# Tencent/FeatherCNN

Hardware: AMD Instinct MI355X
Metric: images/sec fp32 forward @224x224 (higher is better)
Workload: dtype f32; 1 GPU; vgg16 whole net (40 layers in the model file, 20 after fusion level 3), batch 32 per GPU, 224x224x3, fp32, synthetic ...; net=vgg16, mode=net, per_gpu_batch=32, global_batch=32, parallelism=batch-shard x1, launch=hipGraph replay per step, conv_routing=fhip_conv_select_algo_tuned

## Files before the change

### __graft_entry__.py

```python
from __future__ import annotations

import os
import subprocess
import sys

ROOT = os.path.dirname(os.path.abspath(__file__))
if ROOT not in sys.path:
    sys.path.insert(0, ROOT)


def build() -> None:
    jobs = str(min(8, os.cpu_count() or 1))
    subprocess.run(["make", "-s", "-j", jobs, "-C", os.path.join(ROOT, "feathercnn_amd", "csrc")], check=True)
    subprocess.run(["make", "-s", "-C", os.path.join(ROOT, "oracle"), "port"], check=True)
    subprocess.run(["make", "-s", "-C", os.path.join(ROOT, "oracle"), "ref"], check=True)
    import feathercnn_amd
    from feathercnn_amd import _lib
    for name in (*_lib.LIBRARIES, *_lib.MORE_LIBRARIES):
        _lib.load(name)
    from feathercnn_amd import provenance
    provenance.write_stamp()


def smoke() -> None:
    import numpy as np
    import torch

    import oracle
    from feathercnn_amd import ConvLayer, ConvParam
    from oracle import conv_geom, nerr, synth

    if not torch.cuda.is_available():
        raise RuntimeError("smoke() needs a GPU")
    if not os.path.exists(os.path.join(ROOT, "feathercnn_amd", "libfeather_hip.so")):
        build()
    dev = torch.device("cuda:0")
    chk = oracle.best()
    cases = [("winograd_f63", conv_geom(16, 32, 20, 3, 1, 1)), ("im2col_1x1", conv_geom(32, 24, 14, 1, 1, 0)),
             ("im2col_7x7s2", conv_geom(3, 16, 32, 7, 2, 3)), ("depthwise_s1", conv_geom(16, 16, 28, 3, 1, 1, group=16)),
             ("depthwise_s2", conv_geom(16, 16, 28, 3, 2, 1, group=16)), ("depthwise_flat_14px", conv_geom(24, 24, 14, 3, 1, 1, group=24)),
             ("depthwise_flat_7px", conv_geom(40, 40, 7, 3, 1, 1, group=40)), ("depthwise_band_56px", conv_geom(8, 8, 56, 3, 1, 1, group=8)),
             ("depthwise_flat_20px_s2", conv_geom(12, 12, 20, 3, 2, 1, group=12)), ("depthwise_flat_5px", conv_geom(44, 44, 5, 3, 1, 1, group=44))]
    for name, g in cases:
        x, w, b = synth(g, 2)
        p = ConvParam(output_channels=g.oc, input_channels=g.ic, input_h=g.ih, input_w=g.iw, kernel_h=g.kh, kernel_w=g.kw,
                      stride_h=g.sh, stride_w=g.sw, pad_left=g.pl, pad_right=g.pr, pad_top=g.pt, pad_bottom=g.pb,
                      group=g.group, bias_term=True, activation=1, batch=2)
        layer = ConvLayer(p, torch.from_numpy(w).to(dev), torch.from_numpy(b).to(dev))
        y = layer.Forward(torch.from_numpy(x).to(dev))
        torch.cuda.synchronize()
        e = nerr(y.cpu().numpy(), chk.forward(g, x, w, b))
        print(f"smoke {name}: algo={layer.booster.algo} normalised error vs {type(chk).__name__} = {e:.2e}")
        if not (e <= 1e-4) or not np.isfinite(e):
            raise AssertionError(f"smoke {name}: parity failed ({e})")
    from feathercnn_amd.booster import WINOGRADF63, forward_chained
    g1, g2 = conv_geom(16, 24, 28, 3, 1, 1), conv_geom(24, 8, 28, 3, 1, 1)
    (x, w1, b1), (_, w2, b2) = synth(g1, 2, seed=3), synth(g2, 2, seed=4)
    run = []
    for g, w, b in ((g1, w1, b1), (g2, w2, b2)):
        p = ConvParam(output_channels=g.oc, input_channels=g.ic, input_h=g.ih, input_w=g.iw, kernel_h=3, kernel_w=3, stride_h=1, stride_w=1,
                      pad_left=1, pad_right=1, pad_top=1, pad_bottom=1, group=1, bias_term=True, activation=1, batch=2)
        run.append(ConvLayer(p, torch.from_numpy(w).to(dev), torch.from_numpy(b).to(dev), algo=WINOGRADF63))
    y = forward_chained(run, torch.from_numpy(x).to(dev))
    torch.cuda.synchronize()
    e = nerr(y.cpu().numpy(), chk.forward(g2, chk.forward(g1, x, w1, b1), w2, b2))
    print(f"smoke chained winograd pair: normalised error = {e:.2e}")
    if not (e <= 1e-4):
        raise AssertionError(f"smoke chained pair: parity failed ({e})")
    g0, g1 = conv_geom(3, 16, 28, 3, 1, 1), conv_geom(16, 8, 28, 3, 1, 1)
    (x, w0, b0), (_, w1, b1) = synth(g0, 2, seed=6), synth(g1, 2, seed=7)
    p0 = ConvParam(output_channels=16, input_channels=3, input_h=28, input_w=28, kernel_h=3, kernel_w=3, stride_h=1, stride_w=1, pad_left=1,
                   pad_right=1, pad_top=1, pad_bottom=1, group=1, bias_term=True, activation=1, batch=2)
    p0.AssignOutputDim()
    p1 = ConvParam(output_channels=8, input_channels=16, input_h=28, input_w=28, kernel_h=3, kernel_w=3, stride_h=1, stride_w=1, pad_left=1,
                   pad_right=1, pad_top=1, pad_bottom=1, group=1, bias_term=True, activation=1, batch=2)
    l1 = ConvLayer(p1, torch.from_numpy(w1).to(dev), torch.from_numpy(b1).to(dev), algo=WINOGRADF63)
    y = forward_chained([l1], torch.from_numpy(x).to(dev), first=(p0, torch.from_numpy(w0).to(dev), torch.from_numpy(b0).to(dev)))
    torch.cuda.synchronize()
    e = nerr(y.cpu().numpy(), chk.forward(g1, chk.forward(g0, x, w0, b0), w1, b1))
    print(f"smoke first layer inside the Winograd input transform: normalised error = {e:.2e}")
    if not (e <= 1e-4):
        raise AssertionError(f"smoke first-layer fusion: parity failed ({e})")
    from feathercnn_amd import model_zoo
    from feathercnn_amd.net import Net
    from oracle import netcheck
    p, b, i, o = model_zoo.tiny_allsorts()
    x = np.random.default_rng(5).uniform(-1, 1, (2, 3, 20, 20)).astype(np.float32)
    want = (netcheck.RefNet(p, b) if netcheck.have_ref_net() else netcheck.PortNet(p, b)).run(i, x, o)
    for level in (1, 3):
        net = Net(fusion=level, tuned=(level == 3), graph=(level == 3))
        net.LoadParam(p)
        net.LoadWeights(b)
        net.FeedInput(i, x)
        net.Forward()
        e = nerr(net.Extract(o), want)
        print(f"smoke tiny net, fusion level {level} ({len(net.layers())} layers after fusion): normalised error = {e:.2e}")
        if not (e <= 1e-4):
            raise AssertionError(f"smoke net: parity failed ({e})")
    sys.path.insert(0, os.path.join(ROOT, "tests"))
    import gconv_ref
    p, b, i, o = model_zoo.tiny_grouped()
    x = np.random.default_rng(6).uniform(-1, 1, (2, 3, 21, 21)).astype(np.float32)
    net = Net(fusion=2)
    net.LoadParam(p)
    net.LoadWeights(b)
    net.FeedInput(i, x)
    net.Forward()
    e = gconv_ref.nerr(net.Extract(o), gconv_ref.Net(p, b).run(i, x, o))
    print(f"smoke grouped net ({sum(a == 'GCONV' for _, _, a in net.layers())} grouped layers): normalised error = {e:.2e}")
    if not (e <= 1e-4):
        raise AssertionError(f"smoke grouped net: parity failed ({e})")
    import deconv_ref
    p, b, i, o = model_zoo.tiny_deconv()
    x = np.random.default_rng(7).uniform(-1, 1, (2, 3, 16, 16)).astype(np.float32)
    net = Net(fusion=2)
    net.LoadParam(p)
    net.LoadWeights(b)
    net.FeedInput(i, x)
    net.Forward()
    e = deconv_ref.nerr(net.Extract(o), deconv_ref.Net(p, b).run(i, x, o))
    print(f"smoke tiny_deconv ({sum(a == 'DECONV' for _, _, a in net.layers())} deconvolution layers): normalised error = {e:.2e}")
    if not (e <= 1e-4):
        raise AssertionError(f"smoke tiny_deconv: parity failed ({e})")
    import inorm_ref
    p, b, i, o = model_zoo.tiny_generative()
    x = np.random.default_rng(8).uniform(-1, 1, (2, 3, 24, 24)).astype(np.float32)
    net = Net(fusion=2)
    net.LoadParam(p)
    net.LoadWeights(b)
    net.FeedInput(i, x)
    net.Forward()
    e = inorm_ref.nerr(net.Extract(o), inorm_ref.Net(p, b).run(i, x, o))
    print(f"smoke tiny_generative ({sum(a == 'INORM' for _, _, a in net.layers())} InstanceNorm layers): normalised error = {e:.2e}")
    if not (e <= 1e-4):
        raise AssertionError(f"smoke tiny_generative: parity failed ({e})")
    import shuffle_ref
    p, b, i, o = model_zoo.tiny_shuffle()
    x = np.random.default_rng(9).uniform(-1, 1, (2, 3, 28, 28)).astype(np.float32)
    net = Net(fusion=2)
    net.LoadParam(p)
    net.LoadWeights(b)
    net.FeedInput(i, x)
    net.Forward()
    e = shuffle_ref.nerr(net.Extract(o), shuffle_ref.Net(p, b).run(i, x, o))
    print(f"smoke tiny_shuffle ({sum(a == 'SHUFFLE' for _, _, a in net.layers())} channel-map launches): normalised error = {e:.2e}")
    if not (e <= 1e-4):
        raise AssertionError(f"smoke tiny_shuffle: parity failed ({e})")
    import atrous_ref
    p, b, i, o = model_zoo.tiny_dilated()
    x = np.random.default_rng(10).uniform(-1, 1, (2, 3, 16, 16)).astype(np.float32)
    net = Net(fusion=2)
    net.SetDilated(True)
    net.LoadParam(p)
    net.LoadWeights(b)
    net.FeedInput(i, x)
    net.Forward()
    e = atrous_ref.nerr(net.Extract(o), atrous_ref.Net(p, b).run(i, x, o))
    print(f"smoke tiny_dilated ({sum(a == 'ATROUS' for _, _, a in net.layers())} dilated layers): normalised error = {e:.2e}")
    if not (e <= 1e-4):
        raise AssertionError(f"smoke tiny_dilated: parity failed ({e})")
    import gate_ref
    p, b, i, o = model_zoo.tiny_se()
    x = np.random.default_rng(11).uniform(-1, 1, (2, 3, 24, 24)).astype(np.float32)
    net = Net(fusion=2)
    net.LoadParam(p)
    net.LoadWeights(b)
    net.FeedInput(i, x)
    net.Forward()
    e = gate_ref.nerr(net.Extract(o), gate_ref.Net(p, b).run(i, x, o))
    print(f"smoke tiny_se ({sum(a == 'GATE' and t == 'Pooling' for t, _, a in net.layers())} collapsed SE blocks): normalised error = {e:.2e}")
    if not (e <= 1e-4):
# ... 87 lines not shown
```

### feathercnn_amd/_lib.py

```python
from __future__ import annotations

import collections
import ctypes
import functools
import os

_HERE = os.path.dirname(os.path.abspath(__file__))
_LOADED = {}

STAGE_NAMES = ("wino_input", "wino_gemm", "wino_output", "igemm", "depthwise", "init", "wino_chain")


class fhip_conv_param(ctypes.Structure):
    _fields_ = [(n, ctypes.c_int) for n in (
        "output_channels", "input_channels", "input_h", "input_w", "kernel_h", "kernel_w", "output_h", "output_w",
        "stride_h", "stride_w", "pad_left", "pad_bottom", "pad_right", "pad_top", "group", "bias_term", "activation")]


class fhip_winograd_plan(ctypes.Structure):
    _fields_ = [("tiles_x", ctypes.c_int), ("tiles_y", ctypes.c_int), ("tiles_per_image", ctypes.c_int),
                ("columns", ctypes.c_int), ("columns_padded", ctypes.c_int), ("column_block", ctypes.c_int), ("frequency_points", ctypes.c_int), ("tile_outputs", ctypes.c_int),
                ("in_channels_padded", ctypes.c_int),
                ("out_channels_padded", ctypes.c_int), ("v_offset_bytes", ctypes.c_size_t), ("v_bytes", ctypes.c_size_t),
                ("m_offset_bytes", ctypes.c_size_t), ("m_bytes", ctypes.c_size_t), ("u_bytes", ctypes.c_size_t)]


class fhip_pool_param(ctypes.Structure):
    _fields_ = [(n, ctypes.c_int) for n in (
        "channels", "input_h", "input_w", "kernel_h", "kernel_w", "stride_h", "stride_w", "pad_left", "pad_right",
        "pad_top", "pad_bottom", "pooling_type", "global_pooling")]


class fhip_pixel_image(ctypes.Structure):
    _fields_ = [("data", ctypes.c_void_p)] + [(n, ctypes.c_int) for n in ("w", "h", "stride", "roi_x", "roi_y", "roi_w", "roi_h")]


_P = ctypes.POINTER(fhip_conv_param)
_Q = ctypes.POINTER(fhip_pool_param)
_PI = ctypes.POINTER(ctypes.c_int)
_SZ = ctypes.c_size_t
_V = ctypes.c_void_p
_I = ctypes.c_int

SIGNATURES = {
    "fhip_conv_assign_output_dim": (_I, [_P]),
    "fhip_conv_flops": (ctypes.c_double, [_P]),
    "fhip_conv_select_algo": (_I, [_P, ctypes.POINTER(_I)]),
    "fhip_conv_select_algo_tuned": (_I, [_P, ctypes.POINTER(_I)]),
    "fhip_conv_get_buffer_size": (_I, [_P, _I, _I, ctypes.POINTER(ctypes.c_size_t), ctypes.POINTER(ctypes.c_size_t)]),
    "fhip_conv_packed_layout": (_I, [_P, _I, ctypes.POINTER(ctypes.c_int)]),
    "fhip_conv_init": (_I, [_P, _I, _V, _V, _V]),
    "fhip_conv_forward": (_I, [_P, _I, _I, _V, _V, _V, _V, _V, _V]),
    "fhip_winograd_f63_plan": (_I, [_P, _I, ctypes.POINTER(fhip_winograd_plan)]),
    "fhip_winograd_f63_plan_canvas": (_I, [_P, _I, _I, ctypes.POINTER(fhip_winograd_plan)]),
    "fhip_winograd_f63_canvas_param": (_I, [_P, _I, _P]),
    "fhip_winograd_f63_transform_kernel": (_I, [_P, _V, _V, _V]),
    "fhip_winograd_f63_input_transform": (_I, [_P, _I, _V, _V, _V]),
    "fhip_winograd_f63_tile_gemm": (_I, [_P, _I, _V, _V, _V, _V]),
    "fhip_winograd_f63_output_transform": (_I, [_P, _I, _V, _V, _V, _V]),
    "fhip_stage_timing_enable": (_I, [_I]),
    "fhip_stage_timing_collect": (_I, [ctypes.POINTER(ctypes.c_double), ctypes.POINTER(ctypes.c_longlong)]),
    "fhip_last_error": (ctypes.c_char_p, []),
    "fhip_version": (ctypes.c_char_p, []),
    "fhip_device_info": (_I, [ctypes.c_char_p, _I, ctypes.POINTER(_I), ctypes.POINTER(_I)]),
    "fhip_conv_streams_1x1": (_I, [_P, _I, _I]),
    "fhip_calibrate_mfma_f32": (_I, [ctypes.POINTER(ctypes.c_double), ctypes.POINTER(ctypes.c_double), _V]),
    "fhip_relu": (_I, [_V, _V, _SZ, _V]),
    "fhip_add": (_I, [_V, _V, _V, _SZ, _I, _V]),
    "fhip_affine": (_I, [_V, _V, _V, _V, _I, _I, _I, _I, _V]),
    "fhip_conv_can_fuse_residual": (_I, [_P, _I]),
    "fhip_conv_forward_residual": (_I, [_P, _I, _I, _V, _V, _V, _V, _V, _V, _V]),
    "fhip_conv_can_fuse_dw_pw": (_I, [_P, _P, _I]),
    "fhip_conv_forward_dw_pw": (_I, [_P, _P, _I, _V, _V, _V, _V, _V, _V, _V]),
    "fhip_conv_can_chain_winograd": (_I, [_P, _I, _P, _I, _I]),
    "fhip_conv_forward_chained": (_I, [_P, _I, _V, _V, _V, _V, _V, _V, _P, _V, _I, _V]),
    "fhip_winograd_f63_output_to_next_input": (_I, [_P, _P, _I, _V, _V, _V, _I, _V]),
    "fhip_conv_can_fuse_siblings": (_I, [_P, _I, _P, _I, _I]),
    "fhip_conv_siblings_geometry": (_I, [_P, _P, _P]),
    "fhip_conv_forward_siblings": (_I, [_P, _P, _I, _V, _V, _V, _V, _V, _V]),
    "fhip_conv_can_fuse_first_winograd": (_I, [_P, _P, _I, _I]),
    "fhip_winograd_f63_input_from_first": (_I, [_P, _P, _I, _V, _V, _V, _V, _V]),
    "fhip_conv_can_fuse_maxpool2": (_I, [_P, _I]),
    "fhip_conv_forward_maxpool2": (_I, [_P, _I, _I, _V, _V, _V, _V, _V, _V]),
    "fhip_pixels_to_float": (_I, [_V, _V, _I, _I, _I, _I, _I, _I, _V, _V, _V]),
    "fhip_yuv420sp_to_float": (_I, [_V, _V, _I, _I, _I, _I, _I, _I, _I, _V, _V, _V]),
    "fhip_pixel_images_plan": (_I, [_V, _I, _I, _I, _I, _V, ctypes.POINTER(_SZ)]),
    "fhip_pixels_to_float_images": (_I, [_V, _V, _V, _V, _V, _V]),
    "fhip_pooling_output_dim": (_I, [_Q, _PI, _PI]),
    "fhip_pooling": (_I, [_Q, _I, _V, _V, _V]),
    "fhip_softmax": (_I, [_V, _V, _I, _I, _V]),
    "fhip_net_create": (_I, [ctypes.POINTER(_V)]),
    "fhip_net_destroy": (_I, [_V]),
    "fhip_net_set_stream": (_I, [_V, _V]),
    "fhip_net_get_stream": (_I, [_V, ctypes.POINTER(_V)]),
    "fhip_net_set_fusion": (_I, [_V, _I]),
    "fhip_net_set_graph": (_I, [_V, _I]),
    "fhip_net_set_tuned_selection": (_I, [_V, _I]),
    "fhip_net_set_dilated": (_I, [_V, _I]),
    "fhip_net_set_quantized": (_I, [_V, _I]),
    "fhip_net_set_requantized": (_I, [_V, _I]),
    "fhip_net_set_extended_layers": (_I, [_V, _I]),
    "fhip_net_set_detection": (_I, [_V, _I]),
    "fhip_net_set_concurrency": (_I, [_V, _I]),
    "fhip_net_set_sub_batches": (_I, [_V, _I]),
    "fhip_net_load_param": (_I, [_V, ctypes.c_char_p]),
    "fhip_net_load_param_mem": (_I, [_V, ctypes.c_char_p, _SZ]),
    "fhip_net_load_weights": (_I, [_V, ctypes.c_char_p]),
    "fhip_net_load_weights_mem": (_I, [_V, _V, _SZ]),
    "fhip_net_load_weights_device": (_I, [_V, _V, _SZ]),
    "fhip_net_feed_input": (_I, [_V, ctypes.c_char_p, _I, _I, _I, _I, _V, _I]),
    "fhip_net_feed_pixels": (_I, [_V, ctypes.c_char_p, _I, _V, _I, _I, _I, _I, _I, _V, _V, _I]),
    "fhip_net_feed_yuv420sp": (_I, [_V, ctypes.c_char_p, _I, _V, _I, _I, _I, _I, _I, _I, _V, _V, _I]),
    "fhip_net_feed_pixel_images": (_I, [_V, ctypes.c_char_p, _I, _V, _I, _I, _I, _V, _V, _I]),
    "fhip_net_forward": (_I, [_V]),
    "fhip_net_extract": (_I, [_V, ctypes.c_char_p, ctypes.POINTER(_V), _PI, _PI, _PI, _PI]),
    "fhip_net_extract_host": (_I, [_V, ctypes.c_char_p, _V, _SZ]),
    "fhip_net_layer_count": (_I, [_V]),
    "fhip_net_layer_info": (_I, [_V, _I, ctypes.c_char_p, ctypes.c_char_p, _I, _PI]),
    "fhip_net_layer_conv_param": (_I, [_V, _I, _P, _PI]),
    "fhip_net_layer_fused_pointwise": (_I, [_V, _I, _P, _PI]),
    "fhip_net_layer_chain": (_I, [_V, _I, _PI, _PI]),
    "fhip_net_layer_canvas": (_I, [_V, _I, _PI]),
    "fhip_net_layer_sibling": (_I, [_V, _I, _PI]),
    "fhip_net_layer_residual": (_I, [_V, _I, _PI]),
    "fhip_net_forward_timed": (_I, [_V, ctypes.POINTER(ctypes.c_float)]),
    "fhip_net_memory": (_I, [_V, ctypes.POINTER(_SZ), ctypes.POINTER(_SZ), ctypes.POINTER(_SZ)]),
}

PIXOUT_SIGNATURES = {
    "fhip_pixout_channels": (_I, [_I]),
    "fhip_float_to_pixels": (_I, [_V, _SZ, _V, _I, _I, _I, _I, _I, _I, _V, _V, _V]),
    "fhip_float_to_pixels_host": (_I, [_V, _SZ, _V, _I, _I, _I, _I, _I, _I, _V, _V, _V]),
    "fhip_pixout_last_error": (ctypes.c_char_p, []),
}

GCONV_SIGNATURES = {
    "fhip_gconv_supported": (_I, [_P]),
    "fhip_gconv_get_buffer_size": (_I, [_P, _I, ctypes.POINTER(_SZ), ctypes.POINTER(_SZ)]),
    "fhip_gconv_init": (_I, [_P, _V, _V, _V]),
    "fhip_gconv_forward": (_I, [_P, _I, _V, _V, _V, _V, _V, _V]),
    "fhip_gconv_route": (_I, [_P, _V, _V, ctypes.c_char_p, _I]),
    "fhip_gconv_last_error": (ctypes.c_char_p, []),
}

class fhip_deconv_param(ctypes.Structure):
    _fields_ = [(n, ctypes.c_int) for n in ("output_channels", "input_channels", "input_h", "input_w", "kernel_h", "kernel_w", "output_h", "output_w",
                                            "stride_h", "stride_w", "pad_left", "pad_bottom", "pad_right", "pad_top", "group", "bias_term",
                                            "activation", "output_pad_right", "output_pad_bottom")]


_DP = ctypes.POINTER(fhip_deconv_param)
DECONV_SIGNATURES = {
    "fhip_deconv_assign_output_dim": (_I, [_DP]),
    "fhip_deconv_supported": (_I, [_DP]),
    "fhip_deconv_get_buffer_size": (_I, [_DP, _I, ctypes.POINTER(_SZ), ctypes.POINTER(_SZ)]),
    "fhip_deconv_init": (_I, [_DP, _V, _V, _V]),
    "fhip_deconv_forward": (_I, [_DP, _I, _V, _V, _V, _V, _V, _V]),
    "fhip_deconv_route": (_I, [_DP, ctypes.c_char_p, _I]),
    "fhip_deconv_last_error": (ctypes.c_char_p, []),
}

_FL = ctypes.c_float
INORM_SIGNATURES = {
    "fhip_instance_norm_get_buffer_size": (_I, [_I, _I, _I, _I, ctypes.POINTER(_SZ)]),
    "fhip_instance_norm_forward": (_I, [_I, _I, _I, _I, _V, _V, _V, _V, _FL, _I, _FL, _V, _V]),
    "fhip_instance_norm_forward_route": (_I, [_I, _I, _I, _I, _I, _V, _V, _V, _V, _FL, _I, _FL, _V, _V]),
    "fhip_instance_norm_route": (_I, [_I, _I, _I, _I, _V, _V, ctypes.c_char_p, _I]),
    "fhip_activation_forward": (_I, [_I, _V, _V, _I, _I, _I, _FL, _FL, _V, _V]),
    "fhip_inorm_last_error": (ctypes.c_char_p, []),
}

_PP = ctypes.POINTER(ctypes.c_void_p)
_IP = ctypes.POINTER(ctypes.c_int)
SHUFFLE_SIGNATURES = {
    "fhip_channel_map_supported": (_I, [_I, _I, _I, _I]),
    "fhip_channel_slice_resolve": (_I, [_I, _IP, _I, _IP]),
    "fhip_channel_shuffle_forward": (_I, [_V, _V, _I, _I, _I, _I, _I, _I, _V]),
    "fhip_channel_slice_forward": (_I, [_PP, _V, _I, _I, _I, _I, _IP, _I, _V]),
    "fhip_channel_map_create": (_I, [_PP, _IP, _I, _IP, _I, _IP]),
    "fhip_channel_map_destroy": (_I, [_V]),
    "fhip_channel_map_forward": (_I, [_V, _PP, _PP, _I, _I, _I, _V]),
    "fhip_channel_map_forward_route": (_I, [_I, _V, _PP, _PP, _I, _I, _I, _V]),
    "fhip_channel_map_route": (_I, [_I, _I, _I, _PP, _I, ctypes.c_char_p, _I]),
    "fhip_shuffle_last_error": (ctypes.c_char_p, []),
}

_PL = ctypes.POINTER(fhip_winograd_plan)
CANVAS_SIGNATURES = {
    "fhip_canvas_output_to_next_input": (_I, [_I, _P, _P, _I, _PL, _PL, _V, _V, _V, _V]),
    "fhip_canvas_output_transform": (_I, [_P, _I, _PL, _V, _V, _V, _I, _V]),
    "fhip_canvas_last_error": (ctypes.c_char_p, []),
}

class fhip_atrous_param(ctypes.Structure):
    _fields_ = [(n, ctypes.c_int) for n in ("output_channels", "input_channels", "input_h", "input_w", "kernel_h", "kernel_w", "output_h", "output_w",
                                            "stride_h", "stride_w", "pad_left", "pad_bottom", "pad_right", "pad_top", "group", "bias_term",
                                            "activation", "dilation_h", "dilation_w")]


_AP = ctypes.POINTER(fhip_atrous_param)
ATROUS_SIGNATURES = {
    "fhip_atrous_assign_output_dim": (_I, [_AP]),
    "fhip_atrous_supported": (_I, [_AP]),
    "fhip_atrous_get_buffer_size": (_I, [_AP, _I, ctypes.POINTER(_SZ), ctypes.POINTER(_SZ)]),
    "fhip_atrous_init": (_I, [_AP, _V, _V, _V]),
    "fhip_atrous_forward": (_I, [_AP, _I, _V, _V, _V, _V, _V, _V]),
    "fhip_atrous_route": (_I, [_AP, ctypes.c_char_p, _I]),
    "fhip_atrous_get_buffer_size_route": (_I, [_AP, _I, ctypes.c_char_p, ctypes.POINTER(_SZ), ctypes.POINTER(_SZ)]),
    "fhip_atrous_init_route": (_I, [_AP, _V, _V, _V, ctypes.c_char_p]),
    "fhip_atrous_forward_route": (_I, [_AP, _I, _V, _V, _V, _V, _V, _V, ctypes.c_char_p]),
    "fhip_atrous_last_error": (ctypes.c_char_p, []),
}

GATE_SIGNATURES = {
    "fhip_channel_gate_forward": (_I, [_I, _I, _I, _I, _V, _V, _V, _V, _I, _V]),
    "fhip_squeeze_get_buffer_size": (_I, [_I, _I, _I, _I, ctypes.POINTER(_SZ)]),
    "fhip_squeeze_forward": (_I, [_I, _I, _I, _I, _V, _V, _V, _V]),
    "fhip_excite_forward": (_I, [_I, _I, _I, _V, _V, _V, _V, _V, _V, _I, _I, _FL, _FL, _V]),
    "fhip_excite_forward_slices": (_I, [_I, _I, _I, _I, _V, _V, _V, _V, _V, _V, _I, _I, _FL, _FL, _V]),
    "fhip_gate_activation_forward": (_I, [_I, _V, _V, _I, _I, _I, _FL, _FL, _V]),
    "fhip_gate_route": (_I, [_I, _I, _I, _I, _I, _V, _V, _V, ctypes.c_char_p, _I]),
    "fhip_gate_last_error": (ctypes.c_char_p, []),
}

RESAMPLE_SIGNATURES = {
    "fhip_interp_output_dim": (_I, [_I, _I, _FL, _FL, _I, _I, _PI, _PI]),
    "fhip_interp_forward": (_I, [_I, _I, _I, _I, _I, _I, _I, _I, _FL, _FL, _V, _V, _V, _I, _V]),
    "fhip_interp_route": (_I, [_I, _I, _I, _I, _I, _I, _I, _FL, _FL, _V, _V, _V, ctypes.c_char_p, _I]),
    "fhip_hardswish_forward": (_I, [_V, _V, _I, _I, _I, _FL, _FL, _V]),
    "fhip_hardswish_route": (_I, [_V, _V, _I, _I, _I, ctypes.c_char_p, _I]),
    "fhip_resample_last_error": (ctypes.c_char_p, []),
}

LRN_SIGNATURES = {
    "fhip_lrn_forward": (_I, [_I, _I, _FL, _FL, _FL, _I, _I, _I, _I, _V, _V, _V]),
    "fhip_lrn_forward_chunked": (_I, [_I, _FL, _FL, _FL, _I, _I, _I, _I, _I, _V, _V, _V]),
    "fhip_lrn_route": (_I, [_I, _I, _I, _I, _I, _I, _V, _V, ctypes.c_char_p, _I]),
    "fhip_lrn_pool_forward": (_I, [_I, _I, _FL, _FL, _FL, _I, _I, _I, _I, _Q, _V, _V, _V]),
    "fhip_lrn_pool_route": (_I, [_I, _I, _I, _I, _I, _I, _Q, _V, _V, ctypes.c_char_p, _I]),
    "fhip_lrn_last_error": (ctypes.c_char_p, []),
}

class fhip_qconv_param(ctypes.Structure):
    _fields_ = [(n, ctypes.c_int) for n in ("output_channels", "input_channels", "input_h", "input_w", "kernel_h", "kernel_w", "output_h", "output_w",
                                            "stride_h", "stride_w", "pad_left", "pad_bottom", "pad_right", "pad_top", "group", "bias_term",
                                            "activation", "dilation_h", "dilation_w", "int8_scale_term")]


_QP = ctypes.POINTER(fhip_qconv_param)
QCONV_SIGNATURES = {
    "fhip_qconv_assign_output_dim": (_I, [_QP]),
    "fhip_qconv_supported": (_I, [_QP]),
    "fhip_qconv_get_buffer_size": (_I, [_QP, _I, ctypes.POINTER(_SZ), ctypes.POINTER(_SZ)]),
    "fhip_qconv_init": (_I, [_QP, _V, _V, _V]),
    "fhip_qconv_dequant_scales": (_I, [_V, _V, _I, _FL]),
    "fhip_qconv_forward": (_I, [_QP, _I, _V, _V, _V, _V, _V, _V, _FL, _V]),
    "fhip_quantize_forward": (_I, [_V, _V, _SZ, _FL, _V]),
    "fhip_qconv_route": (_I, [_QP, ctypes.c_char_p, _I]),
    "fhip_qconv_get_buffer_size_route": (_I, [_QP, _I, ctypes.c_char_p, ctypes.POINTER(_SZ), ctypes.POINTER(_SZ)]),
    "fhip_qconv_init_route": (_I, [_QP, _V, _V, _V, ctypes.c_char_p]),
    "fhip_qconv_forward_route": (_I, [_QP, _I, _V, _V, _V, _V, _V, _V, _FL, _V, ctypes.c_char_p]),
    "fhip_qconv_last_error": (ctypes.c_char_p, []),
}


class fhip_q8_param(ctypes.Structure):
    _fields_ = fhip_qconv_param._fields_ + [("input_int8", ctypes.c_int), ("output_int8", ctypes.c_int)]


_8P = ctypes.POINTER(fhip_q8_param)
Q8_SIGNATURES = {
    "fhip_q8_tensor_bytes": (_I, [_I, _I, _I, _I, ctypes.POINTER(_SZ)]),
    "fhip_q8_assign_output_dim": (_I, [_8P]),
    "fhip_q8_supported": (_I, [_8P]),
    "fhip_q8_get_buffer_size": (_I, [_8P, _I, ctypes.POINTER(_SZ), ctypes.POINTER(_SZ)]),
    "fhip_q8_init": (_I, [_8P, _V, _V, _V]),
    "fhip_q8_dequant_scales": (_I, [_V, _V, _I, _FL]),
    "fhip_q8_forward": (_I, [_8P, _I, _V, _V, _V, _V, _V, _V, _FL, _FL, _V]),
    "fhip_q8_route": (_I, [_8P, ctypes.c_char_p, _I]),
    "fhip_q8_get_buffer_size_route": (_I, [_8P, _I, ctypes.c_char_p, ctypes.POINTER(_SZ), ctypes.POINTER(_SZ)]),
    "fhip_q8_init_route": (_I, [_8P, _V, _V, _V, ctypes.c_char_p]),
    "fhip_q8_forward_route": (_I, [_8P, _I, _V, _V, _V, _V, _V, _V, _FL, _FL, _V, ctypes.c_char_p]),
    "fhip_q8_quantize_forward": (_I, [_V, _V, _I, _I, _I, _I, _FL, _V]),
    "fhip_q8_dequantize_forward": (_I, [_V, _V, _I, _I, _I, _I, _FL, _V]),
    "fhip_q8_relu_forward": (_I, [_V, _V, _SZ, _V]),
    "fhip_q8_max_pool_forward": (_I, [_Q, _I, _V, _V, _V]),
    "fhip_q8_last_error": (ctypes.c_char_p, []),
}


_FP = ctypes.POINTER(ctypes.c_float)
DETECT_SIGNATURES = {
    "fhip_permute_output_dim": (_I, [_I, _I, _I, _I, _I, _PI, _PI, _PI]),
    "fhip_permute_forward": (_I, [_I, _I, _I, _I, _I, _I, _V, _V, _V]),
    "fhip_permute_concat_forward": (_I, [_I, _PI, _PI, _I, _V, _PP, _V]),
    "fhip_normalize_forward": (_I, [_I, _I, _I, _I, _I, _FL, _V, _V, _V, _V]),
    "fhip_axis_softmax_forward": (_I, [_I, _I, _I, _V, _V, _V]),
    "fhip_priorbox_fill": (_I, [_I, _I, _I, _I, _FP, _I, _FP, _I, _FP, _I, _FP, _I, _I, _FL, _FL, _FL, _PI, _FP, _SZ]),
    "fhip_detection_output_get_buffer_size": (_I, [_I, _I, _I, _I, _I, ctypes.POINTER(_SZ)]),
    "fhip_detection_output_forward": (_I, [_I, _I, _I, _FL, _I, _I, _FL, _I, _V, _V, _V, _V, _V, _V]),
    "fhip_detect_route": (_I, [_I, _I, _I, _I, _I, _I, _V, _V, ctypes.c_char_p, _I]),
    "fhip_detect_last_error": (ctypes.c_char_p, []),
}


def _load(path, signatures):
    lib = _LOADED.get(path)
    if lib is None:
        import torch
        if not os.path.exists(path):
            raise RuntimeError(f"feathercnn_amd: HIP library {path} is missing -- run `python -c 'import __graft_entry__ as g; "
                               "g.build()'` (or `make -C feathercnn_amd/csrc`). There is no CPU fallback.")
        lib = ctypes.CDLL(path)
        for name, (res, args) in signatures.items():
            fn = getattr(lib, name)
            fn.restype = res
            fn.argtypes = args
        _LOADED[path] = lib
    return lib


def checker(load, last_error: str):
    def _check(rc: int, what: str):
        if rc != 0:
            from .booster import FeatherHipError
            msg = getattr(load(), last_error)().decode(errors="replace")
            raise FeatherHipError(f"{what} failed with code {rc}: {msg}")
    return _check


Library = collections.namedtuple("Library", "file headers macro signatures last_error structs route")

LIBRARIES = {
    "hip": Library("libfeather_hip.so", ("feather_hip.h", "feather_net.h"), "FHIP_API", SIGNATURES, "fhip_last_error",
                   (fhip_conv_param, fhip_winograd_plan, fhip_pool_param, fhip_pixel_image), None),
    "pixout": Library("libfeather_pixout.so", ("feather_pixout.h",), "FHIP_PIXOUT_API", PIXOUT_SIGNATURES, "fhip_pixout_last_error", (), None),
    "gconv": Library("libfeather_gconv.so", ("feather_gconv.h",), "FHIP_GCONV_API", GCONV_SIGNATURES, "fhip_gconv_last_error", (), "ROUTE_GCONV"),
    "deconv": Library("libfeather_deconv.so", ("feather_deconv.h",), "FHIP_DECONV_API", DECONV_SIGNATURES, "fhip_deconv_last_error",
                      (fhip_deconv_param,), "ROUTE_DECONV"),
    "inorm": Library("libfeather_inorm.so", ("feather_inorm.h",), "FHIP_INORM_API", INORM_SIGNATURES, "fhip_inorm_last_error", (), "ROUTE_INORM"),
    "shuffle": Library("libfeather_shuffle.so", ("feather_shuffle.h",), "FHIP_SHUFFLE_API", SHUFFLE_SIGNATURES, "fhip_shuffle_last_error", (),
                       "ROUTE_SHUFFLE"),
    "canvas": Library("libfeather_canvas.so", ("feather_canvas.h",), "FHIP_CANVAS_API", CANVAS_SIGNATURES, "fhip_canvas_last_error", (), None),
    "atrous": Library("libfeather_atrous.so", ("feather_atrous.h",), "FHIP_ATROUS_API", ATROUS_SIGNATURES, "fhip_atrous_last_error",
                      (fhip_atrous_param,), "ROUTE_ATROUS"),
    "gate": Library("libfeather_gate.so", ("feather_gate.h",), "FHIP_GATE_API", GATE_SIGNATURES, "fhip_gate_last_error", (), "ROUTE_GATE"),
    "resample": Library("libfeather_resample.so", ("feather_resample.h",), "FHIP_RESAMPLE_API", RESAMPLE_SIGNATURES, "fhip_resample_last_error", (),
                        "ROUTE_RESAMPLE"),
    "lrn": Library("libfeather_lrn.so", ("feather_lrn.h",), "FHIP_LRN_API", LRN_SIGNATURES, "fhip_lrn_last_error", (), "ROUTE_LRN"),
    "qconv": Library("libfeather_qconv.so", ("feather_qconv.h",), "FHIP_QCONV_API", QCONV_SIGNATURES, "fhip_qconv_last_error",
                     (fhip_qconv_param,), "ROUTE_QCONV"),
}
MAIN = "hip"
MORE_LIBRARIES = {
    "q8": Library("libfeather_q8.so", ("feather_q8.h",), "FHIP_Q8_API", Q8_SIGNATURES, "fhip_q8_last_error", (fhip_q8_param,), None),
    "detect": Library("libfeather_detect.so", ("feather_detect.h",), "FHIP_DETECT_API", DETECT_SIGNATURES, "fhip_detect_last_error", (), None),
}


def row(name: str) -> Library:
    return LIBRARIES[name] if name in LIBRARIES else MORE_LIBRARIES[name]


def path(name: str) -> str:
    default = os.path.join(_HERE, row(name).file)
    return os.environ.get("FEATHER_HIP_LIB", default) if name == MAIN else default


def load(name: str):
    return _load(path(name), row(name).signatures)


def lib_path() -> str:
    return path(MAIN)


def load_library():
    return load(MAIN)


for _name in (*LIBRARIES, *MORE_LIBRARIES):
    if _name != MAIN:
        globals()[f"{_name}_path"] = functools.partial(path, _name)
        globals()[f"load_{_name}_library"] = functools.partial(load, _name)
del _name
```

### feathercnn_amd/csrc/net.hip

```cpp
#include "net_side.h"
#include "net_model.h"
#include "net_core.h"
#include "net_conv.h"
#include "net_layers.h"
#include "net_detect.h"
#include "net_plan.h"

namespace fhip::net
{

static Layer* create_extended_layer(const std::string& type)
{
    if (type == "Interp") return new InterpLayer;
    if (type == "HardSwish") return new HardSwishLayer;
    if (type == "LRN") return new LRNLayer;
    return nullptr;
}

static Layer* create_layer(const std::string& type)
{
    if (type == "Input") return new InputLayer;
    if (type == "Convolution" || type == "ConvolutionDepthWise") return new ConvLayer;
    if (type == "Deconvolution" || type == "DeconvolutionDepthWise") return new DeconvLayer;
    if (type == "ReLU") return new ReluLayer;
// ... 128 lines not shown
}

}

using namespace fhip;
using namespace fhip::net;

struct fhip_net
{
    Net impl;
    std::vector<std::unique_ptr<fhip_net>> more;
    std::vector<hipStream_t> more_streams;
    hipEvent_t fork = nullptr;
    std::vector<hipEvent_t> joins;
    std::vector<int> share;
    std::map<std::string, DeviceVec> gathered;
    unsigned char* staging = nullptr;
    size_t staging_bytes = 0;
    std::vector<unsigned char> plans;
    hipEvent_t plans_read = nullptr;
    ~fhip_net()
    {
        if (staging) (void)hipFree(staging);
        if (plans_read) (void)hipEventDestroy(plans_read);
        more.clear();
        for (hipStream_t st : more_streams) (void)hipStreamDestroy(st);
        if (fork) (void)hipEventDestroy(fork);
        for (hipEvent_t e : joins) (void)hipEventDestroy(e);
    }
};

static void deal(int num, int parts, std::vector<int>& share)
{
    share.assign(parts, num / parts);
    for (int r = 0; r < num % parts; ++r) ++share[r];
}

static int reserve_staging(fhip_net* n, size_t bytes)
{
    if (bytes <= n->staging_bytes) return FHIP_OK;
    FHIP_CHECK_HIP(hipStreamSynchronize(n->impl.stream));
    if (n->staging) FHIP_CHECK_HIP(hipFree(n->staging));
    n->staging = nullptr;
    n->staging_bytes = 0;
    FHIP_CHECK_HIP(hipMalloc((void**)&n->staging, bytes));
    n->staging_bytes = bytes;
    return FHIP_OK;
}

template <class Convert>
static int feed_shares(fhip_net* n, const char* blob_name, int num, int cout, int target_w, int target_h, const Convert& convert)
{
    const auto into_blob = [&](fhip_net* m, int first, int cnt) -> int {
        Blob* b = m->impl.find(blob_name);
        if (!b) return failf(NET_E_IO, "Invalid input blob %s, not found in map.", blob_name);
        if (b->n != cnt || b->c != cout || b->h != target_h || b->w != target_w)
        {
            const float* old = b->data;
            const int rc = b->reshape(cnt, cout, target_h, target_w);
            if (rc) return rc;
            m->impl.shapes_dirty = true;
            if (old != b->data) m->impl.drop_graph();
        }
        return convert(b->data, first, cnt, m->impl.stream);
    };
    if (!n->more.empty())
    {
        deal(num, (int)n->more.size() + 1, n->share);
        FHIP_CHECK_HIP(hipEventRecord(n->fork, n->impl.stream));
        int first = n->share[0];
        for (size_t r = 0; r < n->more.size(); ++r)
        {
            const int cnt = n->share[r + 1];
            if (cnt > 0)
            {
                FHIP_CHECK_HIP(hipStreamWaitEvent(n->more[r]->impl.stream, n->fork, 0));
                const int rc = into_blob(n->more[r].get(), first, cnt);
                if (rc) return rc;
                FHIP_CHECK_HIP(hipEventRecord(n->joins[r], n->more[r]->impl.stream));
                FHIP_CHECK_HIP(hipStreamWaitEvent(n->impl.stream, n->joins[r], 0));
            }
            first += cnt;
        }
        num = n->share[0];
    }
    return into_blob(n, 0, num);
}

template <class Convert>
static int feed_bytes(fhip_net* n, const char* blob_name, int num, const unsigned char* bytes_in, size_t image, int cout, int target_w,
                      int target_h, int on_device, const Convert& convert)
{
    if (!n->impl.find(blob_name)) return failf(NET_E_IO, "Invalid input blob %s, not found in map.", blob_name);
    const unsigned char* pixels = bytes_in;
    if (!on_device)
    {
        const int rc = reserve_staging(n, image * num);
        if (rc) return rc;
        FHIP_CHECK_HIP(hipMemcpyAsync(n->staging, pixels, image * num, hipMemcpyHostToDevice, n->impl.stream));
        pixels = n->staging;
    }
    return feed_shares(n, blob_name, num, cout, target_w, target_h, [&](float* out, int first, int cnt, hipStream_t s) {
        return convert(out, pixels + first * image, cnt, s);
    });
}

#define NET_GUARD(n) \
    if (!(n)) return fail(FHIP_E_BADARG, "null net")

extern "C"
{

int fhip_net_create(fhip_net** out)
{
    if (!out) return fail(FHIP_E_BADARG, "null argument");
    *out = new fhip_net;
    return FHIP_OK;
}

int fhip_net_destroy(fhip_net* n)
{
    NET_GUARD(n);
    for (auto& m : n->more)
        if (m->impl.stream) (void)hipStreamSynchronize(m->impl.stream);
    if (n->impl.stream || n->impl.initialized) (void)hipStreamSynchronize(n->impl.stream);
    delete n;
    return FHIP_OK;
}

int fhip_net_set_sub_batches(fhip_net* n, int replicas)
{
    NET_GUARD(n);
    if (replicas < 1 || replicas > 16) return fail(FHIP_E_BADARG, "1 .. 16 sub-batches");
    if (n->impl.param_loaded || !n->more.empty()) return fail(FHIP_E_BADARG, "set the number of sub-batches once, before LoadParam");
    for (int r = 1; r < replicas; ++r)
    {
        hipStream_t st = nullptr;
        FHIP_CHECK_HIP(hipStreamCreateWithFlags(&st, hipStreamNonBlocking));
        n->more_streams.push_back(st);
        hipEvent_t e = nullptr;
        FHIP_CHECK_HIP(hipEventCreateWithFlags(&e, hipEventDisableTiming));
        n->joins.push_back(e);
        std::unique_ptr<fhip_net> m(new fhip_net);
        m->impl.stream = st;
        m->impl.fusion = n->impl.fusion;
        m->impl.use_graph = n->impl.use_graph;
        m->impl.tuned_selection = n->impl.tuned_selection;
        m->impl.dilated = n->impl.dilated;
        m->impl.extended = n->impl.extended;
        m->impl.detection = n->impl.detection;
        m->impl.quantized = n->impl.quantized;
        m->impl.requantized = n->impl.requantized;
        m->impl.concurrency = n->impl.concurrency;
        n->more.push_back(std::move(m));
    }
    if (replicas > 1 && !n->fork) FHIP_CHECK_HIP(hipEventCreateWithFlags(&n->fork, hipEventDisableTiming));
    return FHIP_OK;
}

int fhip_net_set_stream(fhip_net* n, void* stream)
{
    NET_GUARD(n);
    n->impl.stream = (hipStream_t)stream;
    n->impl.drop_graph();
    return FHIP_OK;
}

int fhip_net_get_stream(fhip_net* n, void** stream)
{
    NET_GUARD(n);
    if (!stream) return fail(FHIP_E_BADARG, "null argument");
    *stream = (void*)n->impl.stream;
    return FHIP_OK;
}

int fhip_net_set_fusion(fhip_net* n, int on)
{
    NET_GUARD(n);
    if (n->impl.fused) return fail(FHIP_E_BADARG, "fusion already ran; set it before the first Forward");
    n->impl.fusion = on;
    for (auto& m : n->more) m->impl.fusion = on;
    return FHIP_OK;
}

int fhip_net_set_tuned_selection(fhip_net* n, int on)
{
    NET_GUARD(n);
    n->impl.tuned_selection = on != 0;
    n->impl.shapes_dirty = true;
    for (auto& m : n->more) (void)fhip_net_set_tuned_selection(m.get(), on);
    return FHIP_OK;
}

int fhip_net_set_dilated(fhip_net* n, int on)
{
    NET_GUARD(n);
    if (n->impl.param_loaded) return fail(FHIP_E_BADARG, "set the dilated-convolution switch before LoadParam");
    n->impl.dilated = on != 0;
    for (auto& m : n->more) m->impl.dilated = on != 0;
    return FHIP_OK;
}

int fhip_net_set_extended_layers(fhip_net* n, int on)
{
    NET_GUARD(n);
    if (n->impl.param_loaded) return fail(FHIP_E_BADARG, "set the extended-layers switch before LoadParam");
    n->impl.extended = on != 0;
    for (auto& m : n->more) m->impl.extended = on != 0;
    return FHIP_OK;
}

int fhip_net_set_detection(fhip_net* n, int on)
{
    NET_GUARD(n);
    if (n->impl.param_loaded) return fail(FHIP_E_BADARG, "set the detection-layers switch before LoadParam");
    n->impl.detection = on != 0;
    for (auto& m : n->more) m->impl.detection = on != 0;
    return FHIP_OK;
}

int fhip_net_set_quantized(fhip_net* n, int on)
{
    NET_GUARD(n);
    if (n->impl.param_loaded) return fail(FHIP_E_BADARG, "set the quantized-layers switch before LoadParam");
    n->impl.quantized = on != 0;
    for (auto& m : n->more) m->impl.quantized = on != 0;
    return FHIP_OK;
}

int fhip_net_set_requantized(fhip_net* n, int on)
{
    NET_GUARD(n);
    if (n->impl.param_loaded) return fail(FHIP_E_BADARG, "set the requantized-layers switch before LoadParam");
    n->impl.requantized = on != 0;
    for (auto& m : n->more) m->impl.requantized = on != 0;
    return FHIP_OK;
}

int fhip_net_set_concurrency(fhip_net* n, int on)
{
    NET_GUARD(n);
    n->impl.concurrency = on != 0;
    n->impl.shapes_dirty = true;
    for (auto& m : n->more) (void)fhip_net_set_concurrency(m.get(), on);
    return FHIP_OK;
}

int fhip_net_set_graph(fhip_net* n, int on)
{
    NET_GUARD(n);
    n->impl.use_graph = on != 0;
    if (!on) n->impl.drop_graph();
    if (on && !n->impl.stream)
    {
        if (!n->impl.owned_stream) FHIP_CHECK_HIP(hipStreamCreateWithFlags(&n->impl.owned_stream, hipStreamNonBlocking));
        n->impl.stream = n->impl.owned_stream;
    }
    for (auto& m : n->more) (void)fhip_net_set_graph(m.get(), on);
    return FHIP_OK;
}

int fhip_net_load_param_mem(fhip_net* n, const char* text, size_t len)
{
    NET_GUARD(n);
    if (!text) return fail(FHIP_E_BADARG, "null text");
    for (auto& m : n->more)
    {
        const int rc = load_param_text(m->impl, text, len);
        if (rc) return rc;
    }
    return load_param_text(n->impl, text, len);
}

int fhip_net_load_param(fhip_net* n, const char* path)
{
    NET_GUARD(n);
    if (!path) return fail(FHIP_E_BADARG, "null path");
    std::vector<char> buf;
    const int rc = read_file(path, buf);
    if (rc) return rc;
    return fhip_net_load_param_mem(n, buf.data(), buf.size());
}

int fhip_net_load_weights_mem(fhip_net* n, const void* data, size_t len)
{
    NET_GUARD(n);
    if (!data && len) return fail(FHIP_E_BADARG, "null data");
    for (auto& m : n->more)
    {
        const int rc = load_weights_mem(m->impl, data, len);
        if (rc) return rc;
    }
    return load_weights_mem(n->impl, data, len);
}

int fhip_net_load_weights_device(fhip_net* n, const void* device_data, size_t len)
{
    NET_GUARD(n);
    if (!device_data && len) return fail(FHIP_E_BADARG, "null data");
    std::vector<char> host(len);
    if (len) FHIP_CHECK_HIP(hipMemcpy(host.data(), device_data, len, hipMemcpyDeviceToHost));
    return fhip_net_load_weights_mem(n, host.data(), len);
}

int fhip_net_load_weights(fhip_net* n, const char* path)
{
    NET_GUARD(n);
    if (!path) return fail(FHIP_E_BADARG, "null path");
    std::vector<char> buf;
    const int rc = read_file(path, buf);
    if (rc) return rc;
    return fhip_net_load_weights_mem(n, buf.data(), buf.size());
}

int fhip_net_feed_input(fhip_net* n, const char* blob_name, int num, int c, int h, int w, const float* data, int on_device)
{
    NET_GUARD(n);
    if (!blob_name || !data || num < 1 || c < 1 || h < 1 || w < 1) return fail(FHIP_E_BADARG, "bad argument");
    if (!n->more.empty())
    {
        deal(num, (int)n->more.size() + 1, n->share);
        if (on_device) FHIP_CHECK_HIP(hipEventRecord(n->fork, n->impl.stream));
        const size_t chw = (size_t)c * h * w;
        size_t first = n->share[0];
        for (size_t r = 0; r < n->more.size(); ++r)
        {
            const int cnt = n->share[r + 1];
            if (cnt > 0)
            {
                if (on_device) FHIP_CHECK_HIP(hipStreamWaitEvent(n->more[r]->impl.stream, n->fork, 0));
                const int rc = fhip_net_feed_input(n->more[r].get(), blob_name, cnt, c, h, w, data + first * chw, on_device);
                if (rc) return rc;
                FHIP_CHECK_HIP(hipEventRecord(n->joins[r], n->more[r]->impl.stream));
                FHIP_CHECK_HIP(hipStreamWaitEvent(n->impl.stream, n->joins[r], 0));
            }
            first += cnt;
        }
        num = n->share[0];
    }
    Blob* b = n->impl.find(blob_name);
    if (!b) return failf(NET_E_IO, "Invalid input blob %s, not found in map.", blob_name);
    if (b->n != num || b->c != c || b->h != h || b->w != w)
    {
        const float* old = b->data;
        const int rc = b->reshape(num, c, h, w);
        if (rc) return rc;
        n->impl.shapes_dirty = true;
        if (old != b->data) n->impl.drop_graph();
    }
    FHIP_CHECK_HIP(hipMemcpyAsync(b->data, data, b->count() * sizeof(float), on_device ? hipMemcpyDeviceToDevice : hipMemcpyHostToDevice, n->impl.stream));
    return FHIP_OK;
}

int fhip_net_feed_pixels(fhip_net* n, const char* blob_name, int num, const unsigned char* pixels, int type, int w, int h, int target_w,
                         int target_h, const float* mean, const float* norm, int on_device)
{
    NET_GUARD(n);
    int cin, cout;
    if (pixel_channels(type, &cin, &cout)) return fail(FHIP_E_BADARG, "unknown pixel type");
    if (!blob_name || !pixels || num < 1 || w < 1 || h < 1 || target_w < 1 || target_h < 1) return fail(FHIP_E_BADARG, "bad argument");
    if ((w != target_w || h != target_h) && (w < 2 || h < 2)) return fail(FHIP_E_BADARG, "a source 1 pixel wide or high cannot be resized");
    return feed_bytes(n, blob_name, num, pixels, (size_t)h * w * cin, cout, target_w, target_h, on_device,
                      [&](float* out, const unsigned char* px, int cnt, hipStream_t s) {
                          return fhip_pixels_to_float(out, px, cnt, type, w, h, target_w, target_h, mean, norm, s);
                      });
}

int fhip_net_feed_yuv420sp(fhip_net* n, const char* blob_name, int num, const unsigned char* yuv, int w, int h, int target_w, int target_h,
                           int type, int resize_first, const float* mean, const float* norm, int on_device)
{
    NET_GUARD(n);
    int cout;
    if (yuv420sp_check(type, w, h, target_w, target_h, resize_first, &cout)) return FHIP_E_BADARG;
    if (!blob_name || !yuv || num < 1) return fail(FHIP_E_BADARG, "bad argument");
    return feed_bytes(n, blob_name, num, yuv, (size_t)h * w * 3 / 2, cout, target_w, target_h, on_device,
                      [&](float* out, const unsigned char* px, int cnt, hipStream_t s) {
                          return fhip_yuv420sp_to_float(out, px, cnt, type, w, h, target_w, target_h, resize_first, mean, norm, s);
                      });
}

int fhip_net_feed_pixel_images(fhip_net* n, const char* blob_name, int num, const fhip_pixel_image* images, int type, int target_w,
                               int target_h, const float* mean, const float* norm, int on_device)
{
    NET_GUARD(n);
    if (!blob_name) return fail(FHIP_E_BADARG, "bad argument");
    size_t bytes = 0;
    int rc = fhip_pixel_images_plan(images, num, type, target_w, target_h, nullptr, &bytes);
    if (rc) return rc;
    if (!n->impl.find(blob_name)) return failf(NET_E_IO, "Invalid input blob %s, not found in map.", blob_name);
    int cin, cout;
    pixel_channels(type, &cin, &cout);
    std::vector<int> share;
    deal(num, (int)n->more.size() + 1, share);
    std::vector<size_t> plan_at(share.size(), 0);
    size_t plans = 0;
    for (size_t r = 0, first = 0; r < share.size(); first += share[r++])
    {
// ... 54 lines not shown
    FHIP_CHECK_HIP(hipEventRecord(n->fork, n->impl.stream));
    for (size_t r = 0; r < n->more.size(); ++r)
    {
        if (n->share[r + 1] < 1) continue;
        Net& m = n->more[r]->impl;
        FHIP_CHECK_HIP(hipStreamWaitEvent(m.stream, n->fork, 0));
        const int rc = forward(m);
        if (rc) return rc;
        FHIP_CHECK_HIP(hipEventRecord(n->joins[r], m.stream));
    }
    const int rc = forward(n->impl);
    if (rc) return rc;
    for (size_t r = 0; r < n->more.size(); ++r)
        if (n->share[r + 1] > 0) FHIP_CHECK_HIP(hipStreamWaitEvent(n->impl.stream, n->joins[r], 0));
    return FHIP_OK;
}

int fhip_net_extract(fhip_net* n, const char* blob_name, float** ptr, int* num, int* c, int* h, int* w)
{
    NET_GUARD(n);
    if (!blob_name || !ptr) return fail(FHIP_E_BADARG, "null argument");
    Blob* b = n->impl.find(blob_name);
    if (!b) return failf(NET_E_IO, "Cannot find output blob %s", blob_name);
    if (b->fused_away) return failf(NET_E_IO, "blob %s was fused into its consumer; disable fusion to extract it", blob_name);
    if (b->chained)
        return failf(NET_E_IO, "blob %s exists only as the next layer's transformed input at fusion level 3; use level 2 to extract it", blob_name);
    if (b->q8) return failf(NET_E_TOPOLOGY, "blob %s holds the int8 output of a requantised layer: it has no fp32 values to extract", blob_name);
    if (b->alias) b->data = b->alias->data;
    *ptr = b->data;
    if (num) *num = b->n;
    if (c) *c = b->c;
    if (h) *h = b->h;
    if (w) *w = b->w;
    if (n->more.empty() || n->share.size() < 2 || n->share[1] < 1) return FHIP_OK;
    size_t total = b->count();
    int images = b->n;
    std::vector<std::pair<float*, size_t>> pieces(1, std::make_pair(b->data, b->count()));
    for (size_t r = 0; r < n->more.size(); ++r)
    {
        if (n->share[r + 1] < 1) continue;
        float* d = nullptr;
        int pn, pc, ph, pw;
        const int rc = fhip_net_extract(n->more[r].get(), blob_name, &d, &pn, &pc, &ph, &pw);
        if (rc) return rc;
        if (pc != b->c || ph != b->h || pw != b->w) return failf(NET_E_SHAPE, "blob %s has different shapes in the sub-batch replicas", blob_name);
        pieces.push_back(std::make_pair(d, (size_t)pn * pc * ph * pw));
        total += pieces.back().second;
        images += pn;
    }
    DeviceVec& g = n->gathered[blob_name];
    if (g.bytes < total * sizeof(float))
    {
        FHIP_CHECK_HIP(hipStreamSynchronize(n->impl.stream));
        const int rc = g.resize(total * sizeof(float));
        if (rc) return rc;
    }
    size_t at = 0;
    for (auto& pc_ : pieces)
    {
        if (pc_.first && pc_.second)
            FHIP_CHECK_HIP(hipMemcpyAsync(g.d + at, pc_.first, pc_.second * sizeof(float), hipMemcpyDeviceToDevice, n->impl.stream));
        at += pc_.second;
    }
    *ptr = g.d;
    if (num) *num = images;
    return FHIP_OK;
}

int fhip_net_extract_host(fhip_net* n, const char* blob_name, float* host, size_t capacity)
{
    float* d = nullptr;
    int num, c, h, w;
    const int rc = fhip_net_extract(n, blob_name, &d, &num, &c, &h, &w);
    if (rc) return rc;
    const size_t count = (size_t)num * c * h * w;
    if (!host || capacity < count) return fail(FHIP_E_BADARG, "host buffer too small");
    if (!d) return fail(FHIP_E_BADARG, "blob has no data yet (run Forward first)");
    FHIP_CHECK_HIP(hipMemcpyAsync(host, d, count * sizeof(float), hipMemcpyDeviceToHost, n->impl.stream));
    FHIP_CHECK_HIP(hipStreamSynchronize(n->impl.stream));
    return FHIP_OK;
}

int fhip_net_layer_count(fhip_net* n)
{
    NET_GUARD(n);
    return (int)n->impl.layers.size();
}

int fhip_net_layer_info(fhip_net* n, int index, char* type, char* name, int len, int* algo)
{
    NET_GUARD(n);
    if (index < 0 || index >= (int)n->impl.layers.size()) return fail(FHIP_E_BADARG, "layer index out of range");
    Layer* l = n->impl.layers[index].get();
    if (type && len > 0) snprintf(type, len, "%s", l->type.c_str());
    if (name && len > 0) snprintf(name, len, "%s", l->name.c_str());
    if (algo) *algo = l->algo();
    return FHIP_OK;
}

int fhip_net_layer_conv_param(fhip_net* n, int index, fhip_conv_param* param, int* batch)
{
    NET_GUARD(n);
    if (index < 0 || index >= (int)n->impl.layers.size() || !param) return fail(FHIP_E_BADARG, "layer index out of range");
    Layer* l = n->impl.layers[index].get();
    const fhip_conv_param* cp = l->conv_param();
    if (!cp) return fail(FHIP_E_BADARG, "not a convolution layer");
    *param = *cp;
    if (batch) *batch = l->bottoms.empty() ? 0 : l->bottoms[0]->n;
    return FHIP_OK;
}

int fhip_net_layer_fused_pointwise(fhip_net* n, int index, fhip_conv_param* param, int* one_kernel)
{
    NET_GUARD(n);
    if (index < 0 || index >= (int)n->impl.layers.size() || !param) return fail(FHIP_E_BADARG, "layer index out of range");
    const fhip_conv_param* cp = n->impl.layers[index]->fused_pointwise(one_kernel);
    if (!cp) return fail(FHIP_E_BADARG, "no pointwise convolution was absorbed into this layer");
    *param = *cp;
    return FHIP_OK;
}

int fhip_net_layer_sibling(fhip_net* n, int index, int* state)
{
    NET_GUARD(n);
    if (index < 0 || index >= (int)n->impl.layers.size() || !state) return fail(FHIP_E_BADARG, "layer index out of range");
    *state = n->impl.layers[index]->sibling_state();
    return FHIP_OK;
}

int fhip_net_layer_residual(fhip_net* n, int index, int* state)
{
    NET_GUARD(n);
    if (index < 0 || index >= (int)n->impl.layers.size() || !state) return fail(FHIP_E_BADARG, "layer index out of range");
    *state = n->impl.layers[index]->residual_state();
    return FHIP_OK;
}

int fhip_net_layer_chain(fhip_net* n, int index, int* v_from_previous, int* writes_next_v)
{
    NET_GUARD(n);
    if (index < 0 || index >= (int)n->impl.layers.size() || !v_from_previous || !writes_next_v) return fail(FHIP_E_BADARG, "layer index out of range");
    n->impl.layers[index]->chain_state(v_from_previous, writes_next_v);
    return FHIP_OK;
}

int fhip_net_layer_canvas(fhip_net* n, int index, int* canvas)
{
    NET_GUARD(n);
    if (index < 0 || index >= (int)n->impl.layers.size() || !canvas) return fail(FHIP_E_BADARG, "layer index out of range");
    *canvas = n->impl.layers[index]->canvas_state();
    return FHIP_OK;
}

int fhip_net_forward_timed(fhip_net* n, float* ms)
{
    NET_GUARD(n);
    if (!ms) return fail(FHIP_E_BADARG, "null argument");
    if (!n->more.empty())
        return fail(FHIP_E_UNSUPPORTED, "per-layer timing of a net with sub-batch replicas: kernels of concurrent replicas share the chip, "
                                        "so their durations are not layer times -- time a net created without fhip_net_set_sub_batches");
    Net& net = n->impl;
    int rc = prepare(net);
    if (rc) return rc;
    const size_t L = net.layers.size();
    std::vector<hipEvent_t> ev(L + 1);
    for (auto& e : ev) FHIP_CHECK_HIP(hipEventCreate(&e));
    FHIP_CHECK_HIP(hipEventRecord(ev[0], net.stream));
    for (size_t i = 0; i < L && rc == 0; ++i)
    {
        rc = net.layers[i]->Forward(net.stream);
        (void)hipEventRecord(ev[i + 1], net.stream);
    }
    (void)hipStreamSynchronize(net.stream);
    if (rc == 0)
        for (size_t i = 0; i < L; ++i) (void)hipEventElapsedTime(&ms[i], ev[i], ev[i + 1]);
    for (auto& e : ev) (void)hipEventDestroy(e);
    return rc;
}

int fhip_net_memory(fhip_net* n, size_t* blob_bytes, size_t* weight_bytes, size_t* arena_bytes)
{
    NET_GUARD(n);
    size_t bb = 0, wb = 0;
    for (auto& kv : n->impl.blobs) bb += kv.second->capacity * sizeof(float);
    for (auto& b : n->impl.shadowed) bb += b->capacity * sizeof(float);
    for (auto& l : n->impl.layers) wb += l->weight_bytes();
    size_t ab = n->impl.arena.bytes;
    for (auto& m : n->more)
    {
        size_t b2 = 0, w2 = 0, a2 = 0;
        (void)fhip_net_memory(m.get(), &b2, &w2, &a2);
        bb += b2;
        wb += w2;
        ab += a2;
    }
    for (auto& kv : n->gathered) bb += kv.second.bytes;
    if (blob_bytes) *blob_bytes = bb;
    if (weight_bytes) *weight_bytes = wb;
    if (arena_bytes) *arena_bytes = ab;
    return FHIP_OK;
}

}
```

### feathercnn_amd/csrc/net_conv.h

```cpp
#pragma once
#include "net_core.h"

namespace fhip::net
{

struct AffineFold
{
    std::vector<float> mul, add;
    bool empty() const { return mul.empty(); }
    bool absorb(const AffineLayer& nx, int K);
    void apply(std::vector<float>& w, std::vector<float>& b, int K) const
    {
        if (mul.empty()) return;
        const size_t per = w.size() / K;
        if (b.empty()) b.assign(K, 0.f);
        for (int k = 0; k < K; ++k)
        {
            for (size_t i = 0; i < per; ++i) w[k * per + i] *= mul[k];
            b[k] = b[k] * mul[k] + add[k];
        }
    }
};

struct BuiltFor
// ... 32 lines not shown
    a.group = p.group, a.bias_term = p.bias_term, a.activation = p.activation;
}

template <class Api, class Param>
struct SideConv
{
    template <bool Assign>
    static int reshape(Layer* l, const Api* api, Param& p, const char* refusal, size_t* buffer_bytes, size_t* packed_bytes)
    {
        if (!api) return FHIP_E_UNSUPPORTED;
        const Blob* b = l->bottoms[0];
        int rc;
        if constexpr (Assign)
            if ((rc = l->side(api, [&](const Api* a) { return a->assign_output_dim(&p); }, NET_E_SHAPE))) return rc;
        if ((rc = l->side(api, [&](const Api* a) { return a->supported(&p) != 1; }, FHIP_E_UNSUPPORTED, refusal))) return rc;
        if ((rc = l->tops[0]->reshape(b->n, p.output_channels, p.output_h, p.output_w))) return rc;
        return l->side(api, [&](const Api* a) { return a->get_buffer_size(&p, b->n, buffer_bytes, packed_bytes); });
    }
    static int init(Layer* l, const Api* api, const Param& p, const std::vector<float>& w, const std::vector<float>& b, DeviceVec& packed,
                    size_t packed_bytes, DeviceVec& bias, hipStream_t s)
    {
        if (!api) return FHIP_E_UNSUPPORTED;
        return stage_weights(w, packed, packed_bytes, p.bias_term ? &b : nullptr, bias, s,
                             [&](const float* raw) { return l->side(api, [&](const Api* a) { return a->init(&p, packed.d, raw, s); }); });
    }
    static int forward(const Layer* l, const Api* api, const Param& p, const DeviceVec& packed, const DeviceVec& bias, hipStream_t s)
    {
        return l->side(api, [&](const Api* a) {
            return a->forward(&p, l->bottoms[0]->n, l->tops[0]->data, l->bottoms[0]->data, packed.d, nullptr, p.bias_term ? bias.d : nullptr, s);
        });
    }
};

struct QuantRoute
{
    fhip_qconv_param q = {};
    fhip_q8_param q8 = {};
    bool on_q8 = false;
    int scale_term = 0;
    std::vector<signed char> w;
    std::vector<float> s_w, b;
    float s_in = 0.f, s_out = 0.f;
    DeviceVec packed, d, bias;
    size_t packed_bytes = 0;
    BuiltFor built;

    int read_scale_term(const ParamDict& pd) { return scale_term = pd.get(8, 0); }
    bool requant() const { return scale_term > 100; }
    int load(const Layer* l, ModelBin& mb, size_t wsize, int K, bool bias_term)
    {
        built = BuiltFor();
        int rc = mb.load_int8(wsize, w);
        if (rc) return rc;
        if (bias_term && (rc = mb.load(K, 1, b))) return rc;
        if ((rc = mb.load(K, 1, s_w))) return rc;
        std::vector<float> one;
        if ((rc = mb.load(1, 1, one))) return rc;
        s_in = one[0];
        if (!std::isfinite(s_in) || !(s_in > 0.f)) return failf(NET_E_SHAPE, "layer %s: the int8 input scale must be finite and > 0", l->name.c_str());
        for (float v : s_w)
            if (!std::isfinite(v) || v < 0.f) return failf(NET_E_SHAPE, "layer %s: an int8 weight scale is not finite or is negative", l->name.c_str());
        if (!requant()) return 0;
        if ((rc = mb.load(1, 1, one))) return rc;
        s_out = one[0];
        if (!std::isfinite(s_out) || !(s_out > 0.f)) return failf(NET_E_SHAPE, "layer %s: the int8 output scale must be finite and > 0", l->name.c_str());
        return 0;
    }
    int reshape(Layer* l)
    {
        q.dilation_h = q.dilation_w = 1;
        q.int8_scale_term = scale_term;
        size_t scratch = 0;
        on_q8 = requant() || l->bottoms[0]->q8;
        if (!on_q8) return SideConv<QconvApi, fhip_qconv_param>::reshape<true>(l, qconv_api(), q, "int8 convolution refused: ", &scratch, &packed_bytes);
        static_assert(sizeof(fhip_q8_param) == sizeof(fhip_qconv_param) + 2 * sizeof(int), "fhip_q8_param is fhip_qconv_param and the two forms");
        memcpy(&q8, &q, sizeof(q));
        q8.input_int8 = l->bottoms[0]->q8 ? 1 : 0;
        q8.output_int8 = requant() ? 1 : 0;
        const int rc = SideConv<Q8Api, fhip_q8_param>::reshape<true>(l, q8_api(), q8, "int8 convolution refused: ", &scratch, &packed_bytes);
        q.output_h = q8.output_h, q.output_w = q8.output_w;
        return rc;
    }
    int layout() const { return on_q8 ? 1 + q8.input_int8 + 2 * q8.output_int8 : 0; }
    int init(Layer* l, const AffineFold& fold, hipStream_t s)
    {
        const BuiltFor want{FHIP_NET_ROUTE_QCONV, layout(), packed_bytes};
        if (built == want) return 0;
        const QconvApi* api = on_q8 ? nullptr : qconv_api();
        const Q8Api* api8 = on_q8 ? q8_api() : nullptr;
        if (!api && !api8) return FHIP_E_UNSUPPORTED;
        const int K = q.output_channels;
        std::vector<float> dq(K), bq = b;
        int rc = on_q8 ? l->side(api8, [&](const Q8Api* a) { return a->dequant_scales(dq.data(), s_w.data(), K, s_in); })
                       : l->side(api, [&](const QconvApi* a) { return a->dequant_scales(dq.data(), s_w.data(), K, s_in); });
        if (rc) return rc;
        if (!fold.empty())
        {
            if (bq.empty()) bq.assign(K, 0.f);
            for (int k = 0; k < K; ++k)
            {
                dq[k] = dq[k] * fold.mul[k];
                const float scaled = bq[k] * fold.mul[k];
                bq[k] = scaled + fold.add[k];
            }
            q.bias_term = q8.bias_term = 1;
        }
        rc = stage_weights(w, packed, packed_bytes, q.bias_term ? &bq : nullptr, bias, s, [&](const signed char* raw) {
            const int e = on_q8 ? l->side(api8, [&](const Q8Api* a) { return a->init(&q8, packed.d, raw, s); })
                                : l->side(api, [&](const QconvApi* a) { return a->init(&q, packed.d, raw, s); });
            return e ? e : d.upload(dq.data(), dq.size(), s);
        });
        if (!rc) built = want;
        return rc;
    }
    int forward(const Layer* l, hipStream_t s) const
    {
        if (on_q8)
            return l->side(q8_api(), [&](const Q8Api* a) {
                return a->forward(&q8, l->bottoms[0]->n, l->tops[0]->data, l->bottoms[0]->data, packed.d, nullptr, d.d, q8.bias_term ? bias.d : nullptr, s_in, s_out, s);
            });
        return l->side(qconv_api(), [&](const QconvApi* a) {
            return a->forward(&q, l->bottoms[0]->n, l->tops[0]->data, l->bottoms[0]->data, packed.d, nullptr, d.d, q.bias_term ? bias.d : nullptr, s_in, s);
        });
    }
    size_t bytes() const { return packed.bytes + d.bytes + bias.bytes; }
};

enum ConvRoute { ROUTE_MAIN, ROUTE_GROUPED, ROUTE_DILATED, ROUTE_INT8 };
static const int ROUTE_CODE[] = {-1, FHIP_NET_ROUTE_GCONV, FHIP_NET_ROUTE_ATROUS, FHIP_NET_ROUTE_QCONV};

enum ConvClaim { CLAIM_POOL = 1, CLAIM_RESIDUAL = 2, CLAIM_PAIR = 4, CLAIM_CHAIN = 8, CLAIM_HEAD = 16, CLAIM_SIBLING = 32 };

struct ConvEpilogues
{
    bool fuse_pool = false, pool_fast = false;
    fhip_pool_param poolq = {};
    DeviceVec pre_pool;
    Blob* residual = nullptr;
    bool res_fast = false;
    std::unique_ptr<ConvLayer> pw;
    bool pair_fast = false;
    DeviceVec mid;
};

struct ChainPlan
{
    ConvLayer* next = nullptr;
    bool in = false;
    int pos = 0;
    size_t bytes = 0;
    bool canvas = false;
    fhip_conv_param canvas_p = {};
    fhip_winograd_plan run_plan = {};
    ConvLayer* head_of = nullptr;
    ConvLayer* head = nullptr;

    void reset() { *this = ChainPlan(); }
    bool runs() const { return in || next || head; }
    static void link(ConvLayer* a, ConvLayer* b);
    static void absorb_first(ConvLayer* first, ConvLayer* consumer);
    void to_canvas(const fhip_conv_param& p, int n) { canvas = fhip_winograd_f63_canvas_param(&p, n, &canvas_p) == FHIP_OK; }
    int plan_run(const fhip_conv_param& p, int n) { return fhip_winograd_f63_plan_canvas(&p, n, canvas ? 2 : 1, &run_plan); }
    void arena(size_t run_bytes) { bytes = run_bytes; }
};

struct SiblingPlan
{
    ConvLayer *sib = nullptr, *sib_of = nullptr;
    ConvLayer* packed_for = nullptr;
    DeviceVec packed, bias;
    bool has_bias = false;

    void reset() { sib = sib_of = nullptr; }
    static void pair(ConvLayer* a, ConvLayer* b);
    void unpaired()
    {
        if (!packed.bytes) return;
        packed.release();
        bias.release();
        packed_for = nullptr;
    }
};

struct ConvLayer : Layer
{
    typedef SideConv<GconvApi, fhip_conv_param> Grouped;
    typedef SideConv<AtrousApi, fhip_atrous_param> Dilated;
    fhip_conv_param p = {};
    ConvRoute route = ROUTE_MAIN;
    int algo_ = -1, layout = 0;
    int dilation_h = 1, dilation_w = 1;
    fhip_atrous_param dilated = {};
    QuantRoute qr;
    std::vector<float> w_host, b_host;
    AffineFold fold;
    DeviceVec packed, bias;
    DeviceVec first_raw;
    BuiltFor built;
    size_t buffer_bytes = 0, packed_bytes = 0;
    ConvEpilogues ep;
    ChainPlan chain;
    SiblingPlan sibs;

    bool needs_weights() const override { return true; }
    ConvLayer* as_conv() override { return this; }
    bool reads_q8() const override { return route == ROUTE_INT8; }
    bool writes_q8() const override { return route == ROUTE_INT8 && qr.requant(); }
    bool first_candidate() const
    {
        return p.kernel_h == 3 && p.kernel_w == 3 && p.stride_h == 1 && p.stride_w == 1 && p.group == 1 && p.input_channels >= 2 && p.input_channels <= 4 && p.pad_left == 1 &&
               p.pad_right == 1 && p.pad_top == 1 && p.pad_bottom == 1;
    }
    bool whole_k() const { return route != ROUTE_MAIN; }
    bool side_epilogues_only() const { return route != ROUTE_MAIN; }
    int bias_channels() const { return !whole_k() && p.group == p.input_channels ? p.input_channels : p.output_channels; }
    int claims() const
    {
        return (ep.fuse_pool ? CLAIM_POOL : 0) | (ep.residual ? CLAIM_RESIDUAL : 0) | (ep.pw ? CLAIM_PAIR : 0) | (chain.in || chain.next ? CLAIM_CHAIN : 0) |
               (chain.head || chain.head_of ? CLAIM_HEAD : 0) | (sibs.sib || sibs.sib_of ? CLAIM_SIBLING : 0);
    }
    bool unclaimed(int but = 0) const { return !(claims() & ~but); }

    int LoadParam(const ParamDict& pd) override
    {
        dilation_w = pd.get(2, 1);
        dilation_h = pd.get(12, dilation_w);
        const bool atrous = dilation_w > 1 || dilation_h > 1;
        if (atrous && !(net && net->dilated))
            return failf(NET_E_UNKNOWN_LAYER, "layer %s: dilated convolution is not supported (fhip_net_set_dilated lifts this)", name.c_str());
        if (dilation_w < 1 || dilation_h < 1) return failf(NET_E_SHAPE, "layer %s: dilation must be >= 1", name.c_str());
        qr.scale_term = pd.get(8, 0);
        const bool quant = qr.scale_term != 0 && net && net->quantized;
        if (qr.scale_term && !quant) return failf(NET_E_UNKNOWN_LAYER, "layer %s: int8 convolution is not supported", name.c_str());
        if (quant && (qr.scale_term < 0 || (qr.scale_term > 100 && !net->requantized)))
            return failf(NET_E_UNKNOWN_LAYER, "layer %s: int8_scale_term %d (requantised int8 output) is not supported", name.c_str(), qr.scale_term);
        if (quant && qr.scale_term > 200) return failf(NET_E_UNKNOWN_LAYER, "layer %s: int8_scale_term %d is not one of 0 .. 200", name.c_str(), qr.scale_term);
        if (quant && atrous) return failf(NET_E_UNKNOWN_LAYER, "layer %s: a dilated int8 convolution is not supported", name.c_str());
        p.kernel_w = pd.get(1, 0);
        p.kernel_h = pd.get(11, p.kernel_w);
        p.stride_w = pd.get(3, 1);
        p.stride_h = pd.get(13, p.stride_w);
        p.pad_left = pd.get(4, 0);
        p.pad_bottom = pd.get(14, p.pad_left);
        p.pad_right = pd.get(4, 0);
        p.pad_top = pd.get(14, p.pad_left);
        p.group = pd.get(7, 1);
        p.output_channels = pd.get(0, 0);
        p.bias_term = pd.get(5, 0);
        p.activation = FHIP_ACT_NONE;
        const int weight_data_size = pd.get(6, 0);
        if (p.group < 1 || p.output_channels % p.group) return failf(NET_E_SHAPE, "layer %s: output_channels is not divisible by its group", name.c_str());
        p.output_channels /= p.group;
        if (p.output_channels <= 0 || p.kernel_h <= 0 || p.kernel_w <= 0) return failf(NET_E_SHAPE, "layer %s: bad convolution geometry", name.c_str());
        long long per_channel = (long long)p.output_channels * p.kernel_h;
        if (per_channel <= INT_MAX) per_channel *= p.kernel_w;
        if (weight_data_size < 0 || per_channel > INT_MAX || weight_data_size % per_channel)
            return failf(NET_E_SHAPE, "layer %s: weight_data_size does not fit the convolution geometry", name.c_str());
        p.input_channels = (int)(weight_data_size / per_channel);
        route = quant ? ROUTE_INT8 : atrous ? ROUTE_DILATED : p.group > 1 && p.group < p.input_channels ? ROUTE_GROUPED : ROUTE_MAIN;
        if (whole_k()) p.output_channels *= p.group;
        if ((route == ROUTE_INT8 || route == ROUTE_DILATED) && (p.pad_left < 0 || p.pad_top < 0))
            return failf(NET_E_UNKNOWN_LAYER, "layer %s: automatic padding is not supported", name.c_str());
        if (route == ROUTE_INT8)
        {
            if (p.input_channels < 1) return failf(NET_E_SHAPE, "layer %s: weight_data_size does not fit the convolution geometry", name.c_str());
            if (p.group != 1 && (p.group != p.input_channels || p.group != p.output_channels))
                return failf(NET_E_UNKNOWN_LAYER, "layer %s: an int8 convolution with a partial group (1 < group < channels) is not supported", name.c_str());
        }
        if (route == ROUTE_DILATED && (p.input_channels < 1 || p.input_channels % p.group))
            return failf(NET_E_SHAPE, "layer %s: weight_data_size does not fit the convolution geometry", name.c_str());
        return 0;
    }
    int LoadWeights(ModelBin& mb) override
    {
        const size_t wsize = (size_t)p.input_channels * p.output_channels * p.kernel_h * p.kernel_w / (whole_k() ? p.group : 1);
        built = BuiltFor();
        sibs.packed_for = nullptr;
        if (route == ROUTE_INT8) return qr.load(this, mb, wsize, p.output_channels, p.bias_term != 0);
        int rc = mb.load(wsize, 0, w_host);
        if (rc) return rc;
        if (p.bias_term) rc = mb.load(bias_channels(), 1, b_host);
        return rc;
    }

    int Reshape() override
    {
        const Blob* b = bottoms[0];
        p.input_w = b->w;
        p.input_h = b->h;
        if (p.input_channels != b->c)
            return failf(NET_E_TOPOLOGY, "convolution layer %s has %d input channels while bottom blob has %d channels", name.c_str(), p.input_channels, b->c);
        if (route == ROUTE_INT8 || route == ROUTE_DILATED) return reshape_own_output();
        fhip_conv_assign_output_dim(&p);
        if (p.output_h < 1 || p.output_w < 1) return failf(NET_E_SHAPE, "layer %s: empty output", name.c_str());
        if (route == ROUTE_GROUPED) return Grouped::reshape<false>(this, gconv_api(), p, "grouped convolution refused: ", &buffer_bytes, &packed_bytes);
        int rc = net->tuned_selection ? fhip_conv_select_algo_tuned(&p, &algo_) : fhip_conv_select_algo(&p, &algo_);
        if (rc) return rc;
        if ((rc = ep.pw ? reshape_pair() : reshape_epilogues())) return rc;
        return fhip_conv_packed_layout(&p, algo_, &layout);
    }
    int reshape_own_output()
    {
        int rc;
        if (route == ROUTE_INT8)
        {
            copy_geometry(qr.q, p);
// ... 6 lines not shown
        dilated.dilation_h = dilation_h, dilated.dilation_w = dilation_w;
        rc = Dilated::reshape<true>(this, atrous_api(), dilated, "dilated convolution refused: ", &buffer_bytes, &packed_bytes);
        p.output_h = dilated.output_h, p.output_w = dilated.output_w;
        return rc;
    }
    size_t output_bytes() const { return (size_t)bottoms[0]->n * p.output_channels * p.output_h * p.output_w * sizeof(float); }
    template <class Step>
    int with_pair_input(float* data, const Step& step)
    {
        Blob dwout;
        dwout.n = bottoms[0]->n, dwout.c = p.output_channels, dwout.h = p.output_h, dwout.w = p.output_w;
        dwout.data = data;
        ep.pw->bottoms.assign(1, &dwout);
        ep.pw->tops = tops;
        ep.pw->net = net;
        const int rc = step();
        ep.pw->bottoms.clear();
        return rc;
    }
    int reshape_pair()
    {
        ConvLayer* pw = ep.pw.get();
        int rc = with_pair_input(nullptr, [&] { return pw->Reshape(); });
        if (rc) return rc;
        ep.pair_fast = fhip_conv_can_fuse_dw_pw(&p, &pw->p, bottoms[0]->n) != 0 && pw->unclaimed() && pw->algo_ == FHIP_IM2COL;
        if (!ep.pair_fast && (rc = ep.mid.resize(output_bytes()))) return rc;
        size_t bb = 0;
        if ((rc = fhip_conv_get_buffer_size(&p, algo_, bottoms[0]->n, &bb, &packed_bytes))) return rc;
        buffer_bytes = std::max(bb, pw->buffer_bytes);
        return 0;
    }
    int reshape_epilogues()
    {
        const Blob* b = bottoms[0];
        const Blob* r = ep.residual;
        int rc, oh = p.output_h, ow = p.output_w;
        ep.res_fast = r && fhip_conv_can_fuse_residual(&p, algo_) != 0;
        if (r && (r->n != b->n || r->c != p.output_channels || r->h != p.output_h || r->w != p.output_w))
            return failf(NET_E_SHAPE, "Shape mismatch among bottoms of layer %s.", name.c_str());
        if (ep.fuse_pool)
        {
            ep.poolq.channels = p.output_channels, ep.poolq.input_h = p.output_h, ep.poolq.input_w = p.output_w;
            if ((rc = fhip_pooling_output_dim(&ep.poolq, &oh, &ow))) return rc;
            ep.pool_fast = fhip_conv_can_fuse_maxpool2(&p, algo_) != 0;
            if (!ep.pool_fast && (rc = ep.pre_pool.resize(output_bytes()))) return rc;
        }
        if ((rc = tops[0]->reshape(b->n, p.output_channels, oh, ow))) return rc;
        return fhip_conv_get_buffer_size(&p, algo_, b->n, &buffer_bytes, &packed_bytes);
    }

    void folded(std::vector<float>& w, std::vector<float>& b) const
    {
        w = w_host;
        b = b_host;
        fold.apply(w, b, p.output_channels);
    }
    int init_siblings(hipStream_t s)
    {
        ConvLayer* o = sibs.sib;
        std::vector<float> wa, ba, wb, bb;
        folded(wa, ba);
        o->folded(wb, bb);
        fhip_conv_param pa = p, pb = o->p, both;
        pa.bias_term = ba.empty() ? 0 : 1;
        pb.bias_term = bb.empty() ? 0 : 1;
        int rc = fhip_conv_siblings_geometry(&pa, &pb, &both);
        if (rc) return rc;
        wa.insert(wa.end(), wb.begin(), wb.end());
        sibs.has_bias = both.bias_term != 0;
        if (sibs.has_bias)
        {
            if (ba.empty()) ba.assign(p.output_channels, 0.f);
            if (bb.empty()) bb.assign(o->p.output_channels, 0.f);
            ba.insert(ba.end(), bb.begin(), bb.end());
        }
        size_t bytes = 0, pk = 0;
        if ((rc = fhip_conv_get_buffer_size(&both, FHIP_IM2COL, bottoms[0]->n, &bytes, &pk))) return rc;
        if ((rc = init_main(both, FHIP_IM2COL, wa, ba, sibs.packed, pk, sibs.bias, s))) return rc;
        sibs.packed_for = o;
        return 0;
    }
    int Init(hipStream_t s) override
    {
        int rc;
        if (ep.pw && (rc = ep.pw->Init(s))) return rc;
        if (sibs.sib && sibs.packed_for != sibs.sib && (rc = init_siblings(s))) return rc;
        if (route == ROUTE_INT8)
        {
            rc = qr.init(this, fold, s);
            if (!rc && !fold.empty()) p.bias_term = 1;
            return rc;
        }
        const BuiltFor want{algo(), layout, packed_bytes};
        if (built == want) return 0;
        std::vector<float> w, b;
        folded(w, b);
        if (!fold.empty()) p.bias_term = dilated.bias_term = 1;
        if (first_candidate() && (rc = first_raw.upload(w.data(), w.size(), s))) return rc;
        if ((rc = route == ROUTE_DILATED   ? Dilated::init(this, atrous_api(), dilated, w, b, packed, packed_bytes, bias, s)
                  : route == ROUTE_GROUPED ? Grouped::init(this, gconv_api(), p, w, b, packed, packed_bytes, bias, s)
                                           : init_main(p, algo_, w, b, packed, packed_bytes, bias, s)))
            return rc;
        built = want;
        return 0;
    }

    int Forward(hipStream_t s) override
    {
        if (route != ROUTE_MAIN) return forward_side(s);
        if (chain.head_of) return 0;
        if (sibs.sib_of) return 0;
        if (sibs.sib) return forward_siblings(s);
        if (ep.pw) return forward_pair(s);
        if (chain.runs()) return forward_chained(s);
        return forward_plain(s);
    }
    const float* bias_d() const { return p.bias_term ? bias.d : nullptr; }
    float* arena() const { return (float*)net->arena.d; }
    int pool_tail(int rc, hipStream_t s) { return rc ? rc : fhip_pooling(&ep.poolq, bottoms[0]->n, tops[0]->data, ep.pre_pool.d, s); }
    int forward_side(hipStream_t s)
    {
        if (route == ROUTE_INT8) return qr.forward(this, s);
        if (route == ROUTE_DILATED) return Dilated::forward(this, atrous_api(), dilated, packed, bias, s);
        return Grouped::forward(this, gconv_api(), p, packed, bias, s);
    }
    int forward_siblings(hipStream_t s)
    {
        return fhip_conv_forward_siblings(&p, &sibs.sib->p, bottoms[0]->n, tops[0]->data, sibs.sib->tops[0]->data, bottoms[0]->data, sibs.packed.d,
                                          sibs.has_bias ? sibs.bias.d : nullptr, s);
    }
    int forward_pair(hipStream_t s)
    {
        ConvLayer* pw = ep.pw.get();
        if (ep.pair_fast)
            return fhip_conv_forward_dw_pw(&p, &pw->p, bottoms[0]->n, tops[0]->data, bottoms[0]->data, packed.d, bias_d(), pw->packed.d, pw->bias_d(), s);
        const int rc = fhip_conv_forward(&p, algo_, bottoms[0]->n, ep.mid.d, bottoms[0]->data, packed.d, arena(), bias_d(), s);
        return rc ? rc : with_pair_input(ep.mid.d, [&] { return pw->Forward(s); });
    }
    int forward_chained(hipStream_t s)
    {
        char* base = reinterpret_cast<char*>(net->arena.d);
        float* v = reinterpret_cast<float*>(base + net->chain_slot[chain.pos & 1]);
        float* vn = reinterpret_cast<float*>(base + net->chain_slot[(chain.pos + 1) & 1]);
        float* m = reinterpret_cast<float*>(base + net->chain_m);
        const float* in = chain.in || chain.head ? nullptr : bottoms[0]->data;
        const float* b = bias_d();
        const int n = bottoms[0]->n, pool = ep.fuse_pool ? 1 : 0;
        if (const ConvLayer* h = chain.head)
        {
            const int rc = fhip_winograd_f63_input_from_first(&h->p, &p, n, v, h->bottoms[0]->data, h->first_raw.d, h->bias_d(), s);
            if (rc) return rc;
        }
        if (chain.canvas || (chain.next && chain.next->chain.canvas)) return forward_canvas(n, in, v, m, vn, b, s);
        if (chain.next) return fhip_conv_forward_chained(&p, n, nullptr, in, packed.d, v, m, b, &chain.next->p, vn, pool, s);
        if (!ep.fuse_pool || ep.pool_fast) return fhip_conv_forward_chained(&p, n, tops[0]->data, in, packed.d, v, m, b, nullptr, nullptr, pool, s);
        return pool_tail(fhip_conv_forward_chained(&p, n, ep.pre_pool.d, in, packed.d, v, m, b, nullptr, nullptr, 0, s), s);
    }
    int forward_canvas(int n, const float* in, float* v, float* m, float* vn, const float* b, hipStream_t s)
    {
        const CanvasApi* api = canvas_api();
        if (!api) return FHIP_E_UNSUPPORTED;
        int rc;
        if (in)
        {
            if (chain.canvas) return failf(FHIP_E_UNSUPPORTED, "layer %s: a canvas layer takes its input from the chained transform before it", name.c_str());
            if ((rc = fhip_winograd_f63_input_transform(&p, n, v, in, s))) return rc;
        }
        rc = chain.canvas ? fhip_winograd_f63_tile_gemm(&chain.canvas_p, n / 4, m, packed.d, v, s) : fhip_winograd_f63_tile_gemm(&p, n, m, packed.d, v, s);
        if (rc) return rc;
        if (const ConvLayer* nx = chain.next)
        {
            const int form = !chain.canvas ? FHIP_CANVAS_ENTRY : nx->chain.canvas ? FHIP_CANVAS_INSIDE : FHIP_CANVAS_EXIT;
            rc = api->chain(form, &p, &nx->p, n, &chain.run_plan, &nx->chain.run_plan, vn, m, b, s);
        }
        else
            rc = api->output(&p, n, &chain.run_plan, tops[0]->data, m, b, ep.fuse_pool ? 1 : 0, s);
        return rc ? failf(rc, "layer %s: %s", name.c_str(), api->last_error()) : 0;
    }
    int forward_plain(hipStream_t s)
    {
        const int n = bottoms[0]->n;
        const float *in = bottoms[0]->data, *b = bias_d();
        if (Blob* r = ep.residual)
        {
            if (r->alias) r->data = r->alias->data;
            if (ep.res_fast) return fhip_conv_forward_residual(&p, algo_, n, tops[0]->data, in, packed.d, arena(), b, r->data, s);
            fhip_conv_param q = p;
            q.activation = FHIP_ACT_NONE;
            const int rc = fhip_conv_forward(&q, algo_, n, tops[0]->data, in, packed.d, arena(), b, s);
            return rc ? rc : fhip_add(tops[0]->data, tops[0]->data, r->data, tops[0]->count(), p.activation == FHIP_ACT_RELU, s);
        }
        if (!ep.fuse_pool) return fhip_conv_forward(&p, algo_, n, tops[0]->data, in, packed.d, arena(), b, s);
        if (ep.pool_fast) return fhip_conv_forward_maxpool2(&p, algo_, n, tops[0]->data, in, packed.d, arena(), b, s);
        return pool_tail(fhip_conv_forward(&p, algo_, n, ep.pre_pool.d, in, packed.d, arena(), b, s), s);
    }

    int Fuse(Layer* next, int level) override;
    bool FuseResidual(Blob* other)
    {
        if (ep.pw)
        {
            if (!unclaimed(CLAIM_PAIR) || !ep.pw->FuseResidual(other)) return false;
            ep.pw->bottoms.pop_back();
            bottoms.push_back(other);
            return true;
        }
        if (side_epilogues_only() || !unclaimed() || p.activation != FHIP_ACT_NONE) return false;
        ep.residual = other;
        bottoms.push_back(other);
        return true;
    }
    size_t weight_bytes() const override
    {
        return packed.bytes + bias.bytes + ep.pre_pool.bytes + ep.mid.bytes + first_raw.bytes + sibs.packed.bytes + sibs.bias.bytes + qr.bytes() +
               (ep.pw ? ep.pw->weight_bytes() : 0);
    }
    const fhip_conv_param* fused_pointwise(int* one_kernel) const override
    {
        if (one_kernel) *one_kernel = ep.pair_fast ? 1 : 0;
        return ep.pw ? &ep.pw->p : nullptr;
    }
    size_t arena_bytes() const override { return std::max(buffer_bytes, chain.bytes); }
    const fhip_conv_param* conv_param() const override { return &p; }
    int algo() const override { return route == ROUTE_MAIN ? algo_ : ROUTE_CODE[route]; }
    int sibling_state() const override { return sibs.sib ? 1 : sibs.sib_of ? 2 : 0; }
    int residual_state() const override { return !ep.residual ? 0 : ep.res_fast ? 1 : 2; }
    void chain_state(int* v_from_previous, int* writes_next_v) const override
    {
        *v_from_previous = chain.head ? 2 : chain.in ? 1 : 0;
        *writes_next_v = chain.head_of ? 2 : chain.next ? 1 : 0;
    }
    int canvas_state() const override { return chain.canvas ? 1 : 0; }
};

inline void ChainPlan::link(ConvLayer* a, ConvLayer* b) { a->chain.next = b, b->chain.in = true, b->chain.pos = a->chain.pos + 1; }
inline void ChainPlan::absorb_first(ConvLayer* first, ConvLayer* consumer) { first->chain.head_of = consumer, consumer->chain.head = first; }
inline void SiblingPlan::pair(ConvLayer* a, ConvLayer* b) { a->sibs.sib = b, b->sibs.sib_of = a; }

}
```

### feathercnn_amd/csrc/net_core.h

```cpp
#pragma once
#include "net_model.h"

namespace fhip::net
{

struct Blob
{
    std::string name;
    int n = 0, c = 0, h = 0, w = 0;
    int dims = 3;
    float* data = nullptr;
    size_t capacity = 0;
    Blob* alias = nullptr;
    bool fused_away = false;
    bool chained = false;
    bool q8 = false;

    size_t count() const { return (size_t)n * c * h * w; }
    size_t q8_bytes() const { return (size_t)n * ((c + 15) / 16) * h * w * 16; }
    size_t floats() const { return q8 ? q8_bytes() / 4 : count(); }
    int reshape(int n_, int c_, int h_, int w_)
    {
        n = n_;
        c = c_;
        h = h_;
        w = w_;
        dims = 3;
        alias = nullptr;
        if (chained && !data) return 0;
        if (floats() > capacity)
        {
            if (data && capacity) (void)hipFree(data);
            data = nullptr;
            capacity = 0;
            FHIP_CHECK_HIP(hipMalloc((void**)&data, floats() * sizeof(float)));
            capacity = floats();
        }
        return 0;
    }
    void drop_storage()
    {
        if (data && capacity) (void)hipFree(data);
        data = nullptr;
        capacity = 0;
    }
    void share(Blob* src)
    {
        n = src->n;
        c = src->c;
        h = src->h;
        w = src->w;
        dims = src->dims;
        if (data && capacity) (void)hipFree(data);
        capacity = 0;
        alias = src;
        data = src->data;
    }
    ~Blob()
    {
        if (data && capacity) (void)hipFree(data);
    }
};

struct DeviceVec
{
    float* d = nullptr;
    size_t bytes = 0;
    int upload(const float* h, size_t count, hipStream_t s)
    {
        if (bytes != count * 4)
        {
            release();
            FHIP_CHECK_HIP(hipMalloc((void**)&d, std::max<size_t>(count, 1) * 4));
            bytes = count * 4;
        }
        if (count) FHIP_CHECK_HIP(hipMemcpyAsync(d, h, count * 4, hipMemcpyHostToDevice, s));
        return 0;
    }
    int resize(size_t nbytes)
    {
        if (bytes != nbytes)
        {
            release();
            FHIP_CHECK_HIP(hipMalloc((void**)&d, std::max<size_t>(nbytes, 4)));
            bytes = nbytes;
        }
        return 0;
    }
    void release()
    {
        if (d) (void)hipFree(d);
        d = nullptr;
        bytes = 0;
    }
    ~DeviceVec() { release(); }
};

struct Net;
struct ConvLayer;
struct PoolingLayer;
struct AffineLayer;
struct EltwiseLayer;
struct InterpLayer;

struct Layer
{
    std::string type, name;
    std::vector<Blob*> bottoms, tops;
    Net* net = nullptr;

    virtual ~Layer() {}
    virtual bool needs_weights() const { return false; }
    virtual ConvLayer* as_conv() { return nullptr; }
    virtual PoolingLayer* as_pooling() { return nullptr; }
    virtual AffineLayer* as_affine() { return nullptr; }
    virtual EltwiseLayer* as_eltwise() { return nullptr; }
    virtual InterpLayer* as_interp() { return nullptr; }
    virtual const float* relu_slope() const { return nullptr; }
    virtual bool reads_q8() const { return false; }
    virtual bool writes_q8() const { return false; }
    template <class Api, class Call>
    int side(const Api* api, const Call& call, int code = 0, const char* prefix = "") const
    {
        if (!api) return FHIP_E_UNSUPPORTED;
        const int rc = call(api);
        return rc ? failf(code ? code : rc, "layer %s: %s%s", name.c_str(), prefix, api->last_error()) : 0;
    }
    virtual int LoadParam(const ParamDict&) { return 0; }
    virtual int LoadWeights(ModelBin&) { return 0; }
    virtual int Reshape()
    {
        if (tops.size() != 1 || bottoms.size() != 1) return failf(NET_E_BASE_RESHAPE, "layer %s: base Reshape needs 1 bottom and 1 top", name.c_str());
        return tops[0]->reshape(bottoms[0]->n, bottoms[0]->c, bottoms[0]->h, bottoms[0]->w);
    }
    int reshape_with(const void* side_library) { return side_library ? Layer::Reshape() : FHIP_E_UNSUPPORTED; }
    virtual int Init(hipStream_t) { return 0; }
    virtual int Forward(hipStream_t) = 0;
    virtual int Fuse(Layer*, int ) { return 0; }
    virtual size_t weight_bytes() const { return 0; }
    virtual size_t arena_bytes() const { return 0; }
    virtual int algo() const { return -1; }
    virtual const fhip_conv_param* conv_param() const { return nullptr; }
    virtual const fhip_conv_param* fused_pointwise(int*) const { return nullptr; }
    virtual void chain_state(int* v_from_previous, int* writes_next_v) const { *v_from_previous = *writes_next_v = 0; }
    virtual int canvas_state() const { return 0; }
    virtual int sibling_state() const { return 0; }
    virtual int residual_state() const { return 0; }
};

static bool is_plain_relu(const Layer* l)
{
    const float* slope = l->relu_slope();
    return slope && *slope == 0.f;
}

struct Net
{
    std::vector<std::unique_ptr<Layer>> layers;
    std::map<std::string, std::unique_ptr<Blob>> blobs;
    std::vector<std::unique_ptr<Blob>> shadowed;
    hipStream_t stream = nullptr;
    int fusion = 1;
    bool use_graph = false;
    bool tuned_selection = false;
    bool dilated = false;
    bool extended = false;
    bool quantized = false;
    bool detection = false;
    bool requantized = false;
    bool param_loaded = false, weights_loaded = false, fused = false, initialized = false, shapes_dirty = true;
    DeviceVec arena;
    size_t chain_slot[2] = {0, 0}, chain_m = 0;
    hipGraphExec_t graph_exec = nullptr;
    hipStream_t owned_stream = nullptr;
    bool concurrency = false;
    hipStream_t side_stream = nullptr;
    std::vector<hipEvent_t> events;
    std::vector<int> side;
    std::vector<std::vector<int>> waits;

    ~Net()
    {
        drop_graph();
        for (hipEvent_t e : events) (void)hipEventDestroy(e);
        if (side_stream) (void)hipStreamDestroy(side_stream);
        if (owned_stream) (void)hipStreamDestroy(owned_stream);
    }
    void drop_graph()
    {
        if (graph_exec) (void)hipGraphExecDestroy(graph_exec);
        graph_exec = nullptr;
    }
    Blob* find(const std::string& n)
    {
        auto it = blobs.find(n);
        return it == blobs.end() ? nullptr : it->second.get();
    }
};

struct Readers
{
    int count = 0, last = -1;
    int sole() const { return count == 1 ? last : -1; }
};

static Readers readers(const Net& net, const Blob* b, size_t from_layer = 0, bool through_alias = false)
{
    Readers r;
    for (size_t j = from_layer; j < net.layers.size(); ++j)
        for (const Blob* x : net.layers[j]->bottoms)
            if (x == b || (through_alias && x->alias == b))
            {
                ++r.count;
                r.last = (int)j;
            }
    return r;
}

struct SumTail
{
    Blob *other = nullptr, *sum_top = nullptr, *top = nullptr;
    std::vector<Blob*> inner;
    int sum = -1, relu_layer = -1, last = -1;
    bool relu = false;
};

static bool sum_tail(const Net& net, Blob* b, int sum, SumTail& t);

}
```

### feathercnn_amd/csrc/net_plan.h

```cpp
#pragma once
#include "net_detect.h"

namespace fhip::net
{

static bool is_channel_map_type(const Layer* l)
{
    const ConcatLayer* cat = l->type == "Concat" ? dynamic_cast<const ConcatLayer*>(l) : nullptr;
    return l->type == "ShuffleChannel" || l->type == "Slice" || (cat && cat->axis == 0);
}

static void collapse_channel_maps(Net& net)
{
    auto holds = [](const std::vector<Blob*>& v, const Blob* b) { return std::find(v.begin(), v.end(), b) != v.end(); };
    for (size_t i = 0; i < net.layers.size(); ++i)
    {
        if (!is_channel_map_type(net.layers[i].get())) continue;
        std::vector<Blob*> made = net.layers[i]->tops;
        size_t end = i + 1;
        for (; end < net.layers.size(); ++end)
        {
            const Layer* l = net.layers[end].get();
            if (!is_channel_map_type(l)) break;
            bool reads = false, sole = true;
            for (const Blob* b : l->bottoms)
                if (holds(made, b))
                {
                    reads = true;
                    sole = sole && readers(net, b).count == 1;
                }
            if (!reads || !sole) break;
            made.insert(made.end(), l->tops.begin(), l->tops.end());
        }
        std::vector<Blob*> sources, inner, finals;
        for (; end - i >= 2; --end)
        {
            sources.clear();
            inner.clear();
            finals.clear();
            bool moves = false;
            for (size_t k = i; k < end; ++k)
            {
                moves = moves || net.layers[k]->type != "Concat";
                for (Blob* b : net.layers[k]->bottoms)
                {
                    if (holds(made, b))
                        inner.push_back(b);
                    else if (!holds(sources, b))
                        sources.push_back(b);
                }
            }
            for (size_t k = i; k < end; ++k)
                for (Blob* t : net.layers[k]->tops)
                    if (!holds(inner, t)) finals.push_back(t);
            if (moves && sources.size() <= FHIP_CHANNEL_MAP_MAX_BLOBS && finals.size() <= FHIP_CHANNEL_MAP_MAX_BLOBS) break;
        }
        if (end - i < 2) continue;
        std::unique_ptr<ChannelMapLayer> run(new ChannelMapLayer);
        run->type = net.layers[i]->type;
        run->name = net.layers[i]->name;
        run->net = &net;
        run->bottoms = sources;
        run->tops = finals;
        for (size_t k = i; k < end; ++k)
        {
            Layer* l = net.layers[k].get();
            if (l->type == "Concat")
            {
                MapStep st;
                st.kind = MapStep::CONCAT;
                st.name = l->name;
                st.bottoms = l->bottoms;
                st.tops = l->tops;
                run->steps.push_back(st);
            }
            else
                run->steps.push_back(static_cast<ChannelMapLayer*>(l)->steps[0]);
        }
        for (Blob* b : inner) b->fused_away = true;
        net.layers[i] = std::move(run);
        net.layers.erase(net.layers.begin() + i + 1, net.layers.begin() + end);
    }
}

static bool sum_tail(const Net& net, Blob* b, int sum, SumTail& t)
{
    if (sum < 0) return false;
    const Layer* l = net.layers[sum].get();
    const EltwiseLayer* elt = net.layers[sum]->as_eltwise();
    if (!elt || l->bottoms.size() != 2 || l->tops.size() != 1 || l->bottoms[0] == l->bottoms[1]) return false;
    t = SumTail();
    t.other = l->bottoms[0] == b ? l->bottoms[1] : l->bottoms[0];
    t.sum = t.last = sum;
    t.sum_top = t.top = l->tops[0];
    t.inner.assign(1, b);
    t.relu = elt->relu;
    if (t.relu) return true;
    const int j = readers(net, t.top).sole();
    if (j > sum && net.layers[j]->bottoms.size() == 1 && net.layers[j]->tops.size() == 1 && is_plain_relu(net.layers[j].get()))
    {
        t.relu = true;
        t.relu_layer = t.last = j;
        t.inner.push_back(t.top);
        t.top = net.layers[j]->tops[0];
    }
    return true;
}

static void collapse_gate_blocks(Net& net)
{
    auto one_to_one = [](const Layer* l) { return l->bottoms.size() == 1 && l->tops.size() == 1; };
    auto dense = [&](Layer* l, int& in, int& out, std::vector<float>& w, std::vector<float>& b, bool& has_b) {
        if (!one_to_one(l)) return false;
        if (l->type == "InnerProduct")
        {
            InnerProductLayer* ip = static_cast<InnerProductLayer*>(l);
            if (ip->quant || ip->p.activation != FHIP_ACT_NONE || ip->w_host.size() != ip->input_size * ip->output_size) return false;
            in = (int)ip->input_size, out = (int)ip->output_size, w = ip->w_host, b = ip->b_host, has_b = ip->p.bias_term != 0;
            return true;
        }
        if (l->type != "Convolution") return false;
        ConvLayer* cv = l->as_conv();
        const fhip_conv_param& p = cv->p;
        if (cv->route != ROUTE_MAIN || p.group != 1 || p.kernel_h != 1 || p.kernel_w != 1 || p.stride_h != 1 || p.stride_w != 1 || p.pad_left || p.pad_right ||
            p.pad_top || p.pad_bottom || p.activation != FHIP_ACT_NONE || !cv->fold.empty() || cv->w_host.size() != (size_t)p.input_channels * p.output_channels)
            return false;
        in = p.input_channels, out = p.output_channels, w = cv->w_host, b = cv->b_host, has_b = p.bias_term != 0;
        return true;
    };
    for (size_t i = 0; i < net.layers.size(); ++i)
    {
        Layer* pool = net.layers[i].get();
        if (!pool->as_pooling() || !one_to_one(pool)) continue;
        const fhip_pool_param& q = pool->as_pooling()->q;
        if (!q.global_pooling || q.pooling_type == 0) continue;
        std::vector<int> gone(1, (int)i);
        std::vector<Blob*> inner;
        std::unique_ptr<GateBlockLayer> blk(new GateBlockLayer);
        auto step = [&](Blob* top) -> Layer* {
            const int j = readers(net, top).sole();
            if (j < 0) return nullptr;
            gone.push_back(j);
            inner.push_back(top);
            return net.layers[j].get();
        };
        Layer* l = step(pool->tops[0]);
        int in2 = 0, out2 = 0;
        if (!l || !dense(l, blk->C, blk->R, blk->w1, blk->b1, blk->has_b1)) continue;
        if (!(l = step(l->tops[0]))) continue;
        if (one_to_one(l) && (is_plain_relu(l) || l->type == "Swish"))
        {
            blk->mact = l->type == "Swish" ? FHIP_EXCITE_MACT_SWISH : FHIP_EXCITE_MACT_RELU;
            if (!(l = step(l->tops[0]))) continue;
        }
// ... 85 lines not shown
    if (net.fusion >= 2) collapse_gate_blocks(net);
    if (net.fusion >= 2) collapse_upsample_adds(net);
    for (size_t i = 0; i < net.layers.size(); ++i)
    {
        for (;;)
        {
            Layer* cur = net.layers[i].get();
            if (cur->tops.size() != 1) break;
            Blob* top = cur->tops[0];
            const int consumer = readers(net, top, i + 1).sole();
            if (consumer < 0) break;
            Layer* nx = net.layers[consumer].get();
            SumTail tail;
            if (net.fusion >= 2 && cur->as_conv() && sum_tail(net, top, consumer, tail))
            {
                bool earlier = false;
                for (size_t j = 0; j < i; ++j)
                    for (Blob* t : net.layers[j]->tops) earlier = earlier || t == tail.other;
                if (!earlier || !cur->as_conv()->FuseResidual(tail.other)) break;
                top->fused_away = true;
                cur->tops[0] = tail.sum_top;
                net.layers.erase(net.layers.begin() + consumer);
                continue;
            }
            if (nx->bottoms.size() != 1 || nx->tops.size() != 1) break;
            const int fr = cur->Fuse(nx, net.fusion);
            if (fr != 1 && fr != 2) break;
            if (fr == 2) cur->as_conv()->ep.pw.reset(net.layers[consumer].release()->as_conv());
            top->fused_away = true;
            cur->tops[0] = nx->tops[0];
            net.layers.erase(net.layers.begin() + consumer);
        }
    }
}

static int plan_concurrency(Net& net)
{
    const size_t L = net.layers.size();
    net.side.assign(L, -1);
    net.waits.assign(L, std::vector<int>());
    if (!net.concurrency) return 0;
    int pairs = 0;
    for (size_t i = 0; i < L; ++i)
    {
        Layer* l = net.layers[i].get();
        if (!l->as_conv() || l->arena_bytes() != 0 || l->tops.size() != 1) continue;
        if (l->sibling_state()) continue;
        const int sole = readers(net, l->tops[0], i + 1, true).sole();
        if (sole <= (int)i + 1) continue;
        const size_t consumer = (size_t)sole;
        bool work_between = false;
        for (size_t j = i + 1; j < consumer; ++j) work_between = work_between || net.layers[j]->algo() >= 0;
        if (!work_between) continue;
        net.side[i] = pairs;
        net.waits[consumer].push_back(pairs);
        ++pairs;
    }
    if (pairs && !net.side_stream) FHIP_CHECK_HIP(hipStreamCreateWithFlags(&net.side_stream, hipStreamNonBlocking));
    while (net.events.size() < (size_t)2 * pairs)
    {
        hipEvent_t e;
        FHIP_CHECK_HIP(hipEventCreateWithFlags(&e, hipEventDisableTiming));
        net.events.push_back(e);
    }
    return 0;
}

static int plan_chains(Net& net)
{
    const size_t L = net.layers.size();
    std::vector<ConvLayer*> conv(L, nullptr);
    for (size_t i = 0; i < L; ++i)
        if ((conv[i] = net.layers[i]->as_conv())) conv[i]->chain.reset();
    for (auto& kv : net.blobs) kv.second->chained = false;
    for (auto& b : net.shadowed) b->chained = false;
    net.chain_slot[0] = net.chain_slot[1] = net.chain_m = 0;
    if (net.fusion < 3) return 0;
    auto plain = [](const ConvLayer* c) {
        return c && c->unclaimed(CLAIM_POOL | CLAIM_CHAIN | CLAIM_HEAD | CLAIM_SIBLING) && c->algo_ == FHIP_WINOGRADF63 && c->tops.size() == 1 && c->bottoms.size() == 1;
    };
    auto chain_away = [](Blob* b) {
        b->chained = true;
        b->drop_storage();
    };
    for (size_t i = 0; i + 1 < L; ++i)
    {
        ConvLayer *a = conv[i], *b = conv[i + 1];
        if (!plain(a) || !plain(b) || b->bottoms[0] != a->tops[0]) continue;
        if (a->ep.fuse_pool && !a->ep.pool_fast) continue;
        if (readers(net, a->tops[0], 0, true).count != 1) continue;
        if (!fhip_conv_can_chain_winograd(&a->p, a->algo_, &b->p, b->algo_, a->ep.fuse_pool ? 1 : 0)) continue;
        ChainPlan::link(a, b);
        chain_away(a->tops[0]);
    }
    for (size_t i = 0; i < L; ++i)
    {
        ConvLayer* c = conv[i];
        if (!c || !c->chain.in || c->chain.canvas) continue;
        ConvLayer* prev = nullptr;
        for (size_t j = 0; j < i; ++j)
            if (conv[j] && conv[j]->chain.next == c) prev = conv[j];
        if (!prev || prev->chain.canvas || !prev->ep.fuse_pool || prev->chain.head) continue;
        const int n = c->bottoms[0]->n;
        fhip_conv_param q;
        if (fhip_winograd_f63_canvas_param(&prev->p, n, &q) == FHIP_OK) continue;
        if (prev->p.kernel_h != 3 || prev->p.pad_left != 1 || prev->p.pad_right != 1 || prev->p.pad_top != 1 || prev->p.pad_bottom != 1 ||
            prev->p.output_h != prev->p.output_w || prev->p.output_h != prev->p.input_h)
            continue;
        std::vector<ConvLayer*> run;
        for (ConvLayer* x = c; x; x = x->chain.next)
        {
            if (x->p.input_h != c->p.input_h || x->p.input_w != c->p.input_w || fhip_winograd_f63_canvas_param(&x->p, n, &q) != FHIP_OK) break;
            if (x->p.activation != FHIP_ACT_NONE && x->p.activation != FHIP_ACT_RELU) break;
            run.push_back(x);
            if (x->ep.fuse_pool) break;
        }
        if (run.empty()) continue;
        ConvLayer* last = run.back();
        if (last->chain.next && !last->ep.fuse_pool) continue;
        if (!last->chain.next && last->ep.fuse_pool && !last->ep.pool_fast) continue;
        if (!canvas_api()) return FHIP_E_UNSUPPORTED;
        for (ConvLayer* x : run) x->chain.to_canvas(x->p, n);
    }
    for (size_t i = 0; i + 1 < L; ++i)
    {
        ConvLayer *a = conv[i], *b = conv[i + 1];
        if (!a || a->route != ROUTE_MAIN || !a->unclaimed(CLAIM_HEAD | CLAIM_SIBLING) || a->tops.size() != 1 || a->bottoms.size() != 1) continue;
        if (!a->first_candidate() || !plain(b) || b->chain.in || b->bottoms[0] != a->tops[0]) continue;
        if (readers(net, a->tops[0], 0, true).count != 1) continue;
        if (!fhip_conv_can_fuse_first_winograd(&a->p, &b->p, b->algo_, a->bottoms[0]->n)) continue;
        ChainPlan::absorb_first(a, b);
        chain_away(a->tops[0]);
    }
    auto restore = [](Blob* b) -> int {
        if (b->chained || b->data || b->alias || b->fused_away || b->count() == 0) return 0;
        FHIP_CHECK_HIP(hipMalloc((void**)&b->data, b->count() * sizeof(float)));
        b->capacity = b->count();
        return 0;
    };
    for (auto& kv : net.blobs)
        if (const int rc = restore(kv.second.get())) return rc;
    for (auto& b : net.shadowed)
        if (const int rc = restore(b.get())) return rc;
    auto up = [](size_t x) { return (x + 255) / 256 * 256; };
    size_t slot[2] = {0, 0}, msz = 0;
    for (ConvLayer* c : conv)
    {
        if (!c || !c->chain.runs()) continue;
        const int rc = c->chain.plan_run(c->p, c->bottoms[0]->n);
        if (rc) return rc;
        slot[c->chain.pos & 1] = std::max(slot[c->chain.pos & 1], up(c->chain.run_plan.v_bytes));
        msz = std::max(msz, up(c->chain.run_plan.m_bytes));
    }
    net.chain_slot[0] = 0;
    net.chain_slot[1] = slot[0];
    net.chain_m = slot[0] + slot[1];
    for (ConvLayer* c : conv)
        if (c && c->chain.runs()) c->chain.arena(slot[0] + slot[1] + msz);
    return 0;
}

static int plan_siblings(Net& net)
{
    const size_t L = net.layers.size();
    std::vector<ConvLayer*> conv(L, nullptr);
    for (size_t i = 0; i < L; ++i)
        if (net.layers[i]->type != "ConvolutionDepthWise" && (conv[i] = net.layers[i]->as_conv())) conv[i]->sibs.reset();
    if (net.fusion < 2) return 0;
    auto root = [](const Blob* b) { return b->alias ? b->alias : b; };
    auto plain = [](const ConvLayer* c) { return c && c->unclaimed() && c->algo_ == FHIP_IM2COL && c->tops.size() == 1 && c->bottoms.size() == 1; };
    auto pairs = [&](const ConvLayer* a, const ConvLayer* b) {
        if (!plain(a) || !plain(b) || root(a->bottoms[0]) != root(b->bottoms[0]) || a->tops[0] == b->tops[0]) return false;
        if (a->p.output_channels <= 64 || b->p.output_channels <= 64) return false;
        return fhip_conv_can_fuse_siblings(&a->p, a->algo_, &b->p, b->algo_, a->bottoms[0]->n) != 0;
    };
    for (size_t i = 0; i < L; ++i)
    {
        if (i + 1 < L && pairs(conv[i], conv[i + 1]))
            SiblingPlan::pair(conv[i], conv[i + 1]);
        else if (conv[i])
            conv[i]->sibs.unpaired();
    }
    return 0;
}

static const Layer* q8_producer(Net& net, const Blob* b)
{
    Layer* found = nullptr;
    for (size_t hops = 0; hops <= net.layers.size(); ++hops)
    {
        Layer* writer = nullptr;
        for (auto& l : net.layers)
            for (const Blob* t : l->tops)
                if (t == b) writer = l.get();
        if (!writer) break;
        found = writer;
        if (writer->bottoms.empty() || !writer->bottoms[0]->q8 || writer->as_conv()) break;
        b = writer->bottoms[0];
    }
    return found;
}

static int reshape_all(Net& net)
{
    net.drop_graph();
    size_t need = 0;
    for (auto& l : net.layers)
    {
        for (const Blob* b : l->bottoms)
            if (b->q8 && !l->reads_q8())
            {
                const Layer* from = q8_producer(net, b);
                return failf(NET_E_TOPOLOGY, "blob %s holds the int8 output of layer %s, which %s layer %s cannot read", b->name.c_str(),
                             from ? from->name.c_str() : "?", l->type.c_str(), l->name.c_str());
            }
        const bool q8 = !l->bottoms.empty() && l->writes_q8();
        for (Blob* t : l->tops) t->q8 = q8;
        const int rc = l->Reshape();
        if (rc) return rc;
    }
    {
        int rc = plan_chains(net);
        if (rc) return rc;
        if ((rc = plan_siblings(net))) return rc;
    }
    for (auto& l : net.layers) need = std::max(need, l->arena_bytes());
    if (need > net.arena.bytes)
    {
        const int rc = net.arena.resize(need);
        if (rc) return rc;
    }
    net.shapes_dirty = false;
    return plan_concurrency(net);
}

static int prepare(Net& net)
{
    if (!net.param_loaded) return failf(NET_E_IO, "Network has not been loaded. Please load the param file first.");
    if (!net.weights_loaded)
    {
        bool needs = false;
        for (auto& l : net.layers) needs = needs || l->needs_weights();
        if (needs) return failf(NET_E_IO, "weights have not been loaded");
    }
    fuse_layers(net);
    for (auto& kv : net.blobs)
        if (!kv.second->fused_away && kv.second->count() == 0)
        {
            bool is_input = false;
            for (auto& l : net.layers)
                if (l->type == "Input")
                    for (Blob* tb : l->tops) is_input = is_input || tb == kv.second.get();
            if (is_input) return failf(NET_E_SHAPE, "input blob %s has not been fed", kv.first.c_str());
        }
    if (net.shapes_dirty)
    {
        const int rc = reshape_all(net);
        if (rc) return rc;
    }
    for (auto& l : net.layers)
    {
        const int rc = l->Init(net.stream);
        if (rc) return rc;
    }
    net.initialized = true;
    return 0;
}

static int run_layers(Net& net)
{
    for (size_t i = 0; i < net.layers.size(); ++i)
    {
        Layer* l = net.layers[i].get();
        if (i < net.side.size() && net.side[i] >= 0)
        {
            hipEvent_t fork = net.events[2 * net.side[i]], join = net.events[2 * net.side[i] + 1];
            FHIP_CHECK_HIP(hipEventRecord(fork, net.stream));
            FHIP_CHECK_HIP(hipStreamWaitEvent(net.side_stream, fork, 0));
            const int rc = l->Forward(net.side_stream);
            if (rc) return rc;
            FHIP_CHECK_HIP(hipEventRecord(join, net.side_stream));
            continue;
        }
        if (i < net.waits.size())
            for (int pair : net.waits[i]) FHIP_CHECK_HIP(hipStreamWaitEvent(net.stream, net.events[2 * pair + 1], 0));
        const int rc = l->Forward(net.stream);
        if (rc) return rc;
    }
    return 0;
}

static int forward(Net& net)
{
    int rc = prepare(net);
    if (rc) return rc;
    if (!net.use_graph) return run_layers(net);
    if (!net.graph_exec)
    {
        hipGraph_t graph = nullptr;
        FHIP_CHECK_HIP(hipStreamBeginCapture(net.stream, hipStreamCaptureModeThreadLocal));
        rc = run_layers(net);
        const hipError_t e = hipStreamEndCapture(net.stream, &graph);
        if (rc)
        {
            if (graph) (void)hipGraphDestroy(graph);
            return rc;
// ... 12 lines not shown
```

### feathercnn_amd/csrc/net_side.h

```cpp
#pragma once
#include <ctype.h>
#include <dlfcn.h>
#include <errno.h>
#include <float.h>
#include <limits.h>
#include <math.h>
#include <stdarg.h>
#include <stdio.h>
#include <stdlib.h>
#include <string.h>

#include <algorithm>
#include <map>
#include <memory>
#include <mutex>
#include <string>
#include <vector>

#include "common.h"
#include "feather_hip/feather_canvas.h"
#include "feather_hip/feather_atrous.h"
#include "feather_hip/feather_deconv.h"
#include "feather_hip/feather_detect.h"
#include "feather_hip/feather_gate.h"
#include "feather_hip/feather_gconv.h"
#include "feather_hip/feather_inorm.h"
#include "feather_hip/feather_lrn.h"
#include "feather_hip/feather_net.h"
#include "feather_hip/feather_q8.h"
#include "feather_hip/feather_qconv.h"
#include "feather_hip/feather_resample.h"
#include "feather_hip/feather_shuffle.h"

namespace fhip::net
{

static int failf(int code, const char* fmt, ...)
{
    char buf[512];
    va_list ap;
    va_start(ap, fmt);
    vsnprintf(buf, sizeof(buf), fmt, ap);
    va_end(ap);
    return fail(code, buf);
}

enum
{
    NET_E_IO = -1,
    NET_E_SHAPE = -100,
    NET_E_UNKNOWN_LAYER = -200,
    NET_E_TOPOLOGY = -300,
    NET_E_BASE_RESHAPE = -400
};

struct SideSymbol
{
    void* slot;
    const char* name;
};

struct SideLibrary
{
    const char *file, *needs, *header;
    std::vector<SideSymbol> symbols;
};

static bool open_side_library(const SideLibrary& lib)
{
    std::string tried;
    Dl_info self;
    if (dladdr((void*)&open_side_library, &self) && self.dli_fname)
    {
        tried = self.dli_fname;
        const size_t slash = tried.rfind('/');
        tried = (slash == std::string::npos ? std::string() : tried.substr(0, slash + 1)) + lib.file;
    }
    void* h = nullptr;
    for (const char* path : {tried.c_str(), lib.file})
        if (*path && (h = dlopen(path, RTLD_NOW | RTLD_LOCAL))) break;
    if (!h)
    {
        failf(FHIP_E_UNSUPPORTED, "%s needs %s next to libfeather_hip.so (%s): %s", lib.needs, lib.file, tried.c_str(), dlerror());
        return false;
    }
    bool all = true;
    for (const SideSymbol& s : lib.symbols)
    {
        void* f = dlsym(h, s.name);
        memcpy(s.slot, &f, sizeof(f));
        all = all && f;
    }
    if (!all)
    {
        failf(FHIP_E_UNSUPPORTED, "%s (%s) does not export the entry points of %s", lib.file, tried.c_str(), lib.header);
        dlclose(h);
    }
    return all;
}

template <class Api>
static const Api* side_api()
{
    static std::mutex mu;
    static Api api;
    static bool loaded = false;
    std::lock_guard<std::mutex> lk(mu);
    if (loaded) return &api;
    Api a;
    if (!open_side_library(a.library())) return nullptr;
    api = a;
    loaded = true;
    return &api;
}

struct GconvApi
{
    decltype(&fhip_gconv_supported) supported = nullptr;
    decltype(&fhip_gconv_get_buffer_size) get_buffer_size = nullptr;
    decltype(&fhip_gconv_init) init = nullptr;
    decltype(&fhip_gconv_forward) forward = nullptr;
    decltype(&fhip_gconv_last_error) last_error = nullptr;
    SideLibrary library()
    {
        return {"libfeather_gconv.so", "a convolution with 1 < group < input_channels", "feather_gconv.h",
                {{&supported, "fhip_gconv_supported"}, {&get_buffer_size, "fhip_gconv_get_buffer_size"}, {&init, "fhip_gconv_init"},
                 {&forward, "fhip_gconv_forward"}, {&last_error, "fhip_gconv_last_error"}}};
    }
};
static const GconvApi* gconv_api() { return side_api<GconvApi>(); }

struct AtrousApi
{
    decltype(&fhip_atrous_assign_output_dim) assign_output_dim = nullptr;
    decltype(&fhip_atrous_supported) supported = nullptr;
    decltype(&fhip_atrous_get_buffer_size) get_buffer_size = nullptr;
    decltype(&fhip_atrous_init) init = nullptr;
    decltype(&fhip_atrous_forward) forward = nullptr;
    decltype(&fhip_atrous_last_error) last_error = nullptr;
    SideLibrary library()
    {
        return {"libfeather_atrous.so", "a dilated convolution", "feather_atrous.h",
                {{&assign_output_dim, "fhip_atrous_assign_output_dim"}, {&supported, "fhip_atrous_supported"},
                 {&get_buffer_size, "fhip_atrous_get_buffer_size"}, {&init, "fhip_atrous_init"}, {&forward, "fhip_atrous_forward"},
                 {&last_error, "fhip_atrous_last_error"}}};
    }
};
static const AtrousApi* atrous_api() { return side_api<AtrousApi>(); }

struct DeconvApi
{
    decltype(&fhip_deconv_assign_output_dim) assign_output_dim = nullptr;
    decltype(&fhip_deconv_supported) supported = nullptr;
    decltype(&fhip_deconv_get_buffer_size) get_buffer_size = nullptr;
    decltype(&fhip_deconv_init) init = nullptr;
    decltype(&fhip_deconv_forward) forward = nullptr;
    decltype(&fhip_deconv_last_error) last_error = nullptr;
    SideLibrary library()
    {
        return {"libfeather_deconv.so", "a Deconvolution layer", "feather_deconv.h",
                {{&assign_output_dim, "fhip_deconv_assign_output_dim"}, {&supported, "fhip_deconv_supported"},
                 {&get_buffer_size, "fhip_deconv_get_buffer_size"}, {&init, "fhip_deconv_init"}, {&forward, "fhip_deconv_forward"},
                 {&last_error, "fhip_deconv_last_error"}}};
    }
};
static const DeconvApi* deconv_api() { return side_api<DeconvApi>(); }

struct InormApi
{
    decltype(&fhip_instance_norm_get_buffer_size) get_buffer_size = nullptr;
    decltype(&fhip_instance_norm_forward) forward = nullptr;
    decltype(&fhip_activation_forward) activation = nullptr;
    decltype(&fhip_inorm_last_error) last_error = nullptr;
    SideLibrary library()
    {
        return {"libfeather_inorm.so", "an InstanceNorm / activation layer", "feather_inorm.h",
                {{&get_buffer_size, "fhip_instance_norm_get_buffer_size"}, {&forward, "fhip_instance_norm_forward"},
                 {&activation, "fhip_activation_forward"}, {&last_error, "fhip_inorm_last_error"}}};
    }
};
static const InormApi* inorm_api() { return side_api<InormApi>(); }

struct ShuffleApi
{
    decltype(&fhip_channel_slice_resolve) resolve = nullptr;
    decltype(&fhip_channel_map_create) create = nullptr;
    decltype(&fhip_channel_map_destroy) destroy = nullptr;
    decltype(&fhip_channel_map_forward) forward = nullptr;
    decltype(&fhip_shuffle_last_error) last_error = nullptr;
    SideLibrary library()
    {
        return {"libfeather_shuffle.so", "a ShuffleChannel / Slice layer", "feather_shuffle.h",
                {{&resolve, "fhip_channel_slice_resolve"}, {&create, "fhip_channel_map_create"}, {&destroy, "fhip_channel_map_destroy"},
                 {&forward, "fhip_channel_map_forward"}, {&last_error, "fhip_shuffle_last_error"}}};
    }
};
static const ShuffleApi* shuffle_api() { return side_api<ShuffleApi>(); }

struct GateApi
{
    decltype(&fhip_channel_gate_forward) apply = nullptr;
    decltype(&fhip_squeeze_get_buffer_size) squeeze_buffer_size = nullptr;
    decltype(&fhip_squeeze_forward) squeeze = nullptr;
    decltype(&fhip_excite_forward) excite = nullptr;
    decltype(&fhip_gate_activation_forward) activation = nullptr;
    decltype(&fhip_gate_last_error) last_error = nullptr;
    SideLibrary library()
    {
        return {"libfeather_gate.so", "a channel-gate / Swish / HardSigmoid layer", "feather_gate.h",
                {{&apply, "fhip_channel_gate_forward"}, {&squeeze_buffer_size, "fhip_squeeze_get_buffer_size"}, {&squeeze, "fhip_squeeze_forward"},
                 {&excite, "fhip_excite_forward"}, {&activation, "fhip_gate_activation_forward"}, {&last_error, "fhip_gate_last_error"}}};
    }
};
static const GateApi* gate_api() { return side_api<GateApi>(); }

struct ResampleApi
{
    decltype(&fhip_interp_output_dim) output_dim = nullptr;
    decltype(&fhip_interp_forward) interp = nullptr;
    decltype(&fhip_hardswish_forward) hardswish = nullptr;
    decltype(&fhip_resample_last_error) last_error = nullptr;
    SideLibrary library()
    {
        return {"libfeather_resample.so", "an Interp / HardSwish layer", "feather_resample.h",
                {{&output_dim, "fhip_interp_output_dim"}, {&interp, "fhip_interp_forward"}, {&hardswish, "fhip_hardswish_forward"},
                 {&last_error, "fhip_resample_last_error"}}};
    }
};
static const ResampleApi* resample_api() { return side_api<ResampleApi>(); }

struct LrnApi
{
    decltype(&fhip_lrn_forward) forward = nullptr;
    decltype(&fhip_lrn_pool_forward) pool_forward = nullptr;
    decltype(&fhip_lrn_last_error) last_error = nullptr;
    SideLibrary library()
    {
        return {"libfeather_lrn.so", "an LRN layer", "feather_lrn.h",
                {{&forward, "fhip_lrn_forward"}, {&pool_forward, "fhip_lrn_pool_forward"}, {&last_error, "fhip_lrn_last_error"}}};
    }
};
static const LrnApi* lrn_api() { return side_api<LrnApi>(); }

struct QconvApi
{
    decltype(&fhip_qconv_assign_output_dim) assign_output_dim = nullptr;
    decltype(&fhip_qconv_supported) supported = nullptr;
    decltype(&fhip_qconv_get_buffer_size) get_buffer_size = nullptr;
    decltype(&fhip_qconv_init) init = nullptr;
    decltype(&fhip_qconv_dequant_scales) dequant_scales = nullptr;
    decltype(&fhip_qconv_forward) forward = nullptr;
    decltype(&fhip_qconv_last_error) last_error = nullptr;
    SideLibrary library()
    {
        return {"libfeather_qconv.so", "an int8 convolution / InnerProduct layer", "feather_qconv.h",
                {{&assign_output_dim, "fhip_qconv_assign_output_dim"}, {&supported, "fhip_qconv_supported"},
                 {&get_buffer_size, "fhip_qconv_get_buffer_size"}, {&init, "fhip_qconv_init"}, {&dequant_scales, "fhip_qconv_dequant_scales"},
                 {&forward, "fhip_qconv_forward"}, {&last_error, "fhip_qconv_last_error"}}};
    }
};
static const QconvApi* qconv_api() { return side_api<QconvApi>(); }

struct Q8Api
{
    decltype(&fhip_q8_assign_output_dim) assign_output_dim = nullptr;
    decltype(&fhip_q8_supported) supported = nullptr;
    decltype(&fhip_q8_get_buffer_size) get_buffer_size = nullptr;
    decltype(&fhip_q8_init) init = nullptr;
    decltype(&fhip_q8_dequant_scales) dequant_scales = nullptr;
    decltype(&fhip_q8_forward) forward = nullptr;
    decltype(&fhip_q8_relu_forward) relu = nullptr;
    decltype(&fhip_q8_max_pool_forward) max_pool = nullptr;
    decltype(&fhip_q8_last_error) last_error = nullptr;
    SideLibrary library()
    {
        return {"libfeather_q8.so", "an int8 layer with int8 input or output", "feather_q8.h",
                {{&assign_output_dim, "fhip_q8_assign_output_dim"}, {&supported, "fhip_q8_supported"}, {&get_buffer_size, "fhip_q8_get_buffer_size"},
                 {&init, "fhip_q8_init"}, {&dequant_scales, "fhip_q8_dequant_scales"}, {&forward, "fhip_q8_forward"}, {&relu, "fhip_q8_relu_forward"},
                 {&max_pool, "fhip_q8_max_pool_forward"}, {&last_error, "fhip_q8_last_error"}}};
    }
};
static const Q8Api* q8_api() { return side_api<Q8Api>(); }

struct DetectApi
{
    decltype(&fhip_permute_output_dim) permute_output_dim = nullptr;
    decltype(&fhip_permute_forward) permute = nullptr;
    decltype(&fhip_permute_concat_forward) permute_concat = nullptr;
    decltype(&fhip_normalize_forward) normalize = nullptr;
    decltype(&fhip_axis_softmax_forward) axis_softmax = nullptr;
    decltype(&fhip_priorbox_fill) priorbox = nullptr;
    decltype(&fhip_detection_output_get_buffer_size) detection_buffer_size = nullptr;
    decltype(&fhip_detection_output_forward) detection_output = nullptr;
    decltype(&fhip_detect_last_error) last_error = nullptr;
    SideLibrary library()
    {
        return {"libfeather_detect.so", "a detection-head layer (Permute, Normalize, PriorBox, DetectionOutput, Softmax along an axis)", "feather_detect.h",
                {{&permute_output_dim, "fhip_permute_output_dim"}, {&permute, "fhip_permute_forward"}, {&permute_concat, "fhip_permute_concat_forward"},
                 {&normalize, "fhip_normalize_forward"}, {&axis_softmax, "fhip_axis_softmax_forward"}, {&priorbox, "fhip_priorbox_fill"},
                 {&detection_buffer_size, "fhip_detection_output_get_buffer_size"}, {&detection_output, "fhip_detection_output_forward"},
                 {&last_error, "fhip_detect_last_error"}}};
    }
};
static const DetectApi* detect_api() { return side_api<DetectApi>(); }

struct CanvasApi
{
    decltype(&fhip_canvas_output_to_next_input) chain = nullptr;
    decltype(&fhip_canvas_output_transform) output = nullptr;
    decltype(&fhip_canvas_last_error) last_error = nullptr;
    SideLibrary library()
    {
        return {"libfeather_canvas.so", "a chained Winograd run on 2x2 image canvases", "feather_canvas.h",
                {{&chain, "fhip_canvas_output_to_next_input"}, {&output, "fhip_canvas_output_transform"}, {&last_error, "fhip_canvas_last_error"}}};
    }
};
static const CanvasApi* canvas_api() { return side_api<CanvasApi>(); }

}
```

### feathercnn_amd/net.py

```python
from __future__ import annotations

import ctypes

import numpy as np

from . import _lib
from .booster import ALGO_NAMES, FeatherHipError, _check, _stream


ROUTE_GCONV = 100
ROUTE_NAMES = dict(ALGO_NAMES)
ROUTE_NAMES[ROUTE_GCONV] = "GCONV"
ROUTE_DECONV = 101
ROUTE_NAMES[ROUTE_DECONV] = "DECONV"
ROUTE_INORM = 102
ROUTE_NAMES[ROUTE_INORM] = "INORM"
ROUTE_SHUFFLE = 103
ROUTE_NAMES[ROUTE_SHUFFLE] = "SHUFFLE"
ROUTE_ATROUS = 104
ROUTE_NAMES[ROUTE_ATROUS] = "ATROUS"
ROUTE_GATE = 105
ROUTE_NAMES[ROUTE_GATE] = "GATE"
ROUTE_RESAMPLE = 106
ROUTE_NAMES[ROUTE_RESAMPLE] = "RESAMPLE"
ROUTE_LRN = 107
ROUTE_NAMES[ROUTE_LRN] = "LRN"
ROUTE_QCONV = 108
ROUTE_NAMES[ROUTE_QCONV] = "QCONV"
DETECT_ROUTE = 109
ROUTE_NAMES[DETECT_ROUTE] = "DETECT"

class Net:
    def __init__(self, fusion: int = 1, graph: bool = False, stream=None, tuned: bool = False, concurrency: bool = False,
                 sub_batches: int = 1):
        self._lib = _lib.load_library()
        h = ctypes.c_void_p()
        _check(self._lib.fhip_net_create(ctypes.byref(h)), "fhip_net_create")
        self._h = h
        _check(self._lib.fhip_net_set_fusion(h, int(fusion)), "fhip_net_set_fusion")
        _check(self._lib.fhip_net_set_graph(h, int(bool(graph))), "fhip_net_set_graph")
        _check(self._lib.fhip_net_set_tuned_selection(h, int(bool(tuned))), "fhip_net_set_tuned_selection")
        _check(self._lib.fhip_net_set_concurrency(h, int(bool(concurrency))), "fhip_net_set_concurrency")
        if stream is not None:
            _check(self._lib.fhip_net_set_stream(h, ctypes.c_void_p(stream)), "fhip_net_set_stream")
        if sub_batches != 1:
            _check(self._lib.fhip_net_set_sub_batches(h, int(sub_batches)), "fhip_net_set_sub_batches")

    def close(self):
        if getattr(self, "_h", None):
            self._lib.fhip_net_destroy(self._h)
            self._h = None

    __del__ = close

    def SetDilated(self, on: bool = True):
        _check(self._lib.fhip_net_set_dilated(self._h, int(bool(on))), "fhip_net_set_dilated")

    def SetQuantized(self, on: bool = True):
        _check(self._lib.fhip_net_set_quantized(self._h, int(bool(on))), "fhip_net_set_quantized")

    def SetRequantized(self, on: bool = True):
        _check(self._lib.fhip_net_set_requantized(self._h, int(bool(on))), "fhip_net_set_requantized")

    def SetExtendedLayers(self, on: bool = True):
        _check(self._lib.fhip_net_set_extended_layers(self._h, int(bool(on))), "fhip_net_set_extended_layers")

    def SetDetection(self, on: bool = True):
        _check(self._lib.fhip_net_set_detection(self._h, int(bool(on))), "fhip_net_set_detection")

    def set_graph(self, on: bool):
        _check(self._lib.fhip_net_set_graph(self._h, int(bool(on))), "fhip_net_set_graph")

    def set_tuned(self, on: bool):
        _check(self._lib.fhip_net_set_tuned_selection(self._h, int(bool(on))), "fhip_net_set_tuned_selection")

    def set_concurrency(self, on: bool):
        _check(self._lib.fhip_net_set_concurrency(self._h, int(bool(on))), "fhip_net_set_concurrency")

    def use_current_stream(self):
        _check(self._lib.fhip_net_set_stream(self._h, _stream()), "fhip_net_set_stream")

    def LoadParam(self, param) -> int:
        if isinstance(param, bytes):
            _check(self._lib.fhip_net_load_param_mem(self._h, param, len(param)), "fhip_net_load_param_mem")
        else:
            _check(self._lib.fhip_net_load_param(self._h, str(param).encode()), "fhip_net_load_param")
        return 0

    def LoadWeights(self, weights) -> int:
        if isinstance(weights, (bytes, bytearray, memoryview)):
            buf = (ctypes.c_char * len(weights)).from_buffer_copy(weights)
            _check(self._lib.fhip_net_load_weights_mem(self._h, buf, len(weights)), "fhip_net_load_weights_mem")
        else:
            _check(self._lib.fhip_net_load_weights(self._h, str(weights).encode()), "fhip_net_load_weights")
        return 0

    def FeedInput(self, input_name: str, data) -> int:
        import torch
        if isinstance(data, torch.Tensor) and data.is_cuda:
            t = data.contiguous().float()
            torch.cuda.current_stream().synchronize()
            shape, ptr, dev = tuple(t.shape), ctypes.c_void_p(t.data_ptr()), 1
            keep = t
        else:
            a = np.ascontiguousarray(np.asarray(data, dtype=np.float32))
            shape, ptr, dev = a.shape, a.ctypes.data_as(ctypes.c_void_p), 0
            keep = a
        if len(shape) == 3:
            shape = (1,) + tuple(shape)
        if len(shape) != 4:
            raise FeatherHipError("FeedInput wants [N][C][H][W] or [C][H][W]")
        n, c, h, w = (int(v) for v in shape)
        _check(self._lib.fhip_net_feed_input(self._h, input_name.encode(), n, c, h, w, ptr, dev), "fhip_net_feed_input")
        self.synchronize()
        del keep
        return 0

    def FeedPixels(self, input_name: str, pixels, ptype: int, target=None, mean=None, norm=None) -> int:
        from .pixels import _images, _per_channel, pixel_channels
        import torch
        n, h, w, ptr, dev, keep = _images(pixels, ptype)
        tw, th = (w, h) if target is None else (int(target[0]), int(target[1]))
        _, cout = pixel_channels(ptype)
        m, mp = _per_channel(mean, cout, "mean")
        s, sp = _per_channel(norm, cout, "norm")
        if dev:
            torch.cuda.current_stream().synchronize()
        _check(self._lib.fhip_net_feed_pixels(self._h, input_name.encode(), n, ptr, int(ptype), w, h, tw, th, mp, sp, dev),
               "fhip_net_feed_pixels")
        self.synchronize()
        del keep, m, s
        return 0

    def FeedPixelImages(self, input_name: str, images, ptype: int, target, rois=None, mean=None, norm=None) -> int:
        from .pixels import _image_descs, _per_channel, pixel_channels
        import torch
        descs, dev, keep = _image_descs(images, ptype, rois)
        tw, th = int(target[0]), int(target[1])
        _, cout = pixel_channels(ptype)
        m, mp = _per_channel(mean, cout, "mean")
        s, sp = _per_channel(norm, cout, "norm")
        if dev:
            torch.cuda.current_stream().synchronize()
        _check(self._lib.fhip_net_feed_pixel_images(self._h, input_name.encode(), len(descs), descs, int(ptype), tw, th, mp, sp, dev),
               "fhip_net_feed_pixel_images")
        self.synchronize()
        del keep, m, s
        return 0

    def FeedYUV420sp(self, input_name: str, frames, ptype: int = 1, target=None, resize_first: bool = True, mean=None, norm=None) -> int:
        from .pixels import _frames, _per_channel
        import torch
        n, w, h, cout, ptr, dev, keep = _frames(frames, ptype)
        tw, th = (w, h) if target is None else (int(target[0]), int(target[1]))
        m, mp = _per_channel(mean, cout, "mean")
        s, sp = _per_channel(norm, cout, "norm")
        if dev:
            torch.cuda.current_stream().synchronize()
        _check(self._lib.fhip_net_feed_yuv420sp(self._h, input_name.encode(), n, ptr, w, h, tw, th, int(ptype), int(bool(resize_first)), mp,
                                                sp, dev), "fhip_net_feed_yuv420sp")
        self.synchronize()
        del keep, m, s
        return 0

    def Forward(self) -> int:
        _check(self._lib.fhip_net_forward(self._h), "fhip_net_forward")
        return 0

    def Extract(self, blob_name: str) -> np.ndarray:
        ptr, shape = self.ExtractDevice(blob_name)
        out = np.empty(shape, dtype=np.float32)
        _check(self._lib.fhip_net_extract_host(self._h, blob_name.encode(), out.ctypes.data_as(ctypes.c_void_p), out.size),
               "fhip_net_extract_host")
        return out

    def ExtractDetections(self, blob_name: str):
        out = self.Extract(blob_name)
        if out.shape[1] != 1 or out.shape[3] != 6:
            raise FeatherHipError(f"blob {blob_name} of shape {out.shape} is not a DetectionOutput top [n][1][keep_top_k][6]")
        return [img[0][:int((img[0][:, 0] > 0).sum())].copy() for img in out]

    def ExtractPixels(self, blob_name: str, ptype: int, target=None, mean=None, norm=None) -> np.ndarray:
        from .pixels import _check_pixout, _per_channel, output_channels
        cn = output_channels(ptype)
        ptr, (n, c, h, w) = self.ExtractDevice(blob_name)
        if c != cn:
            raise FeatherHipError(f"blob {blob_name} has {c} channels, pixel type {ptype:#x} needs {cn}")
        if not ptr:
            raise FeatherHipError(f"blob {blob_name} has no data yet (run Forward first)")
        tw, th = (w, h) if target is None else (int(target[0]), int(target[1]))
        m, mp = _per_channel(mean, cn, "mean")
        s, sp = _per_channel(norm, cn, "norm")
        stream = ctypes.c_void_p()
        _check(self._lib.fhip_net_get_stream(self._h, ctypes.byref(stream)), "fhip_net_get_stream")
        out = np.empty((n, th, tw, cn), dtype=np.uint8)
        _check_pixout(_lib.load_pixout_library().fhip_float_to_pixels_host(out.ctypes.data_as(ctypes.c_void_p), 0, ctypes.c_void_p(ptr), n,
                                                                           int(ptype), w, h, tw, th, mp, sp, stream),
                      "fhip_float_to_pixels_host")
        del m, s
        return out

    def ExtractDevice(self, blob_name: str):
        p = ctypes.c_void_p()
        dims = [ctypes.c_int() for _ in range(4)]
        _check(self._lib.fhip_net_extract(self._h, blob_name.encode(), ctypes.byref(p), *[ctypes.byref(d) for d in dims]),
               "fhip_net_extract")
        return p.value, tuple(d.value for d in dims)

    def synchronize(self):
        import torch
        torch.cuda.synchronize()

    def layers(self):
        out = []
        n = self._lib.fhip_net_layer_count(self._h)
        for i in range(n):
            t, nm, algo = ctypes.create_string_buffer(64), ctypes.create_string_buffer(256), ctypes.c_int()
            _check(self._lib.fhip_net_layer_info(self._h, i, t, nm, 64, ctypes.byref(algo)), "fhip_net_layer_info")
            out.append((t.value.decode(), nm.value.decode(), ROUTE_NAMES.get(algo.value)))
        return out

    def conv_params(self):
        out = {}
        for i in range(self._lib.fhip_net_layer_count(self._h)):
            p, b = _lib.fhip_conv_param(), ctypes.c_int()
            if self._lib.fhip_net_layer_conv_param(self._h, i, ctypes.byref(p), ctypes.byref(b)) == 0:
                out[i] = (p, b.value)
        return out

    def fused_pointwise(self):
        out = {}
        for i in range(self._lib.fhip_net_layer_count(self._h)):
            p, one = _lib.fhip_conv_param(), ctypes.c_int()
            if self._lib.fhip_net_layer_fused_pointwise(self._h, i, ctypes.byref(p), ctypes.byref(one)) == 0:
                out[i] = (p, bool(one.value))
        return out

    def siblings(self):
        out = {}
        for i in range(self._lib.fhip_net_layer_count(self._h)):
            st = ctypes.c_int()
            if self._lib.fhip_net_layer_sibling(self._h, i, ctypes.byref(st)) == 0 and st.value:
                out[i] = st.value
        return out

    def residuals(self):
        out = {}
        for i in range(self._lib.fhip_net_layer_count(self._h)):
            st = ctypes.c_int()
            if self._lib.fhip_net_layer_residual(self._h, i, ctypes.byref(st)) == 0 and st.value:
                out[i] = st.value
        return out

    def chains(self, raw=False):
        out = {}
        for i in range(self._lib.fhip_net_layer_count(self._h)):
            a, b = ctypes.c_int(), ctypes.c_int()
            if self._lib.fhip_net_layer_chain(self._h, i, ctypes.byref(a), ctypes.byref(b)) == 0 and (a.value or b.value):
                if raw:
                    out[i] = (a.value, b.value)
                elif a.value == 1 or b.value == 1:
                    out[i] = (a.value == 1, b.value == 1)
        return out

    def canvases(self):
        out = []
        for i in range(self._lib.fhip_net_layer_count(self._h)):
            c = ctypes.c_int()
            if self._lib.fhip_net_layer_canvas(self._h, i, ctypes.byref(c)) == 0 and c.value:
                out.append(i)
        return out

    def forward_timed(self):
        n = self._lib.fhip_net_layer_count(self._h)
        ms = (ctypes.c_float * max(n, 1))()
        _check(self._lib.fhip_net_forward_timed(self._h, ms), "fhip_net_forward_timed")
        info = self.layers()
        return [(t, nm, a, ms[i]) for i, (t, nm, a) in enumerate(info)]

    def memory(self):
        v = [ctypes.c_size_t() for _ in range(3)]
        _check(self._lib.fhip_net_memory(self._h, *[ctypes.byref(x) for x in v]), "fhip_net_memory")
        return {"blob_bytes": v[0].value, "weight_bytes": v[1].value, "arena_bytes": v[2].value}


def _p(t):
    return ctypes.c_void_p(t.data_ptr()) if t is not None else None


def relu(x):
    import torch
    y = torch.empty_like(x)
    _check(_lib.load_library().fhip_relu(_p(y), _p(x), x.numel(), _stream()), "fhip_relu")
    return y


def add(a, b, relu: bool = False):
    import torch
    y = torch.empty_like(a)
    _check(_lib.load_library().fhip_add(_p(y), _p(a), _p(b), a.numel(), int(relu), _stream()), "fhip_add")
    return y


def affine(x, mul, add_=None, relu: bool = False):
    import torch
    y = torch.empty_like(x)
    n, c, h, w = x.shape
    _check(_lib.load_library().fhip_affine(_p(y), _p(x), _p(mul), _p(add_), n, c, h * w, int(relu), _stream()),
           "fhip_affine")
    return y


def pool_param(c, h, w, kernel, stride=1, pad=(0, 0, 0, 0), pooling_type=0, global_pooling=False):
    kh, kw = (kernel, kernel) if isinstance(kernel, int) else kernel
    sh, sw = (stride, stride) if isinstance(stride, int) else stride
    return _lib.fhip_pool_param(c, h, w, kh, kw, sh, sw, pad[0], pad[1], pad[2], pad[3], pooling_type, int(global_pooling))


def pooling(x, q):
    import torch
    oh, ow = ctypes.c_int(), ctypes.c_int()
    lib = _lib.load_library()
    _check(lib.fhip_pooling_output_dim(ctypes.byref(q), ctypes.byref(oh), ctypes.byref(ow)), "fhip_pooling_output_dim")
    y = torch.empty((x.shape[0], x.shape[1], oh.value, ow.value), device=x.device, dtype=torch.float32)
    _check(lib.fhip_pooling(ctypes.byref(q), x.shape[0], _p(y), _p(x), _stream()), "fhip_pooling")
    return y


def softmax(x):
    import torch
    y = torch.empty_like(x)
    _check(_lib.load_library().fhip_softmax(_p(y), _p(x), x.shape[0], x[0].numel(), _stream()), "fhip_softmax")
    return y
```

### include/feather/net.h

```cpp
#pragma once

#include <stdio.h>
#include <string.h>

#include <string>
#include <vector>

#include "feather_hip/feather_net.h"
#include "feather_hip/feather_pixout.h"
#include "ncnn/mat.h"

namespace feather
{

struct Detection
{
    int label;
    float score, xmin, ymin, xmax, ymax;
};

class Net
{
  public:
    Net() : net_(NULL) { fhip_net_create(&net_); }
    ~Net()
    {
        if (net_) fhip_net_destroy(net_);
    }

    int LoadParam(const char* param_path) { return fhip_net_load_param(net_, param_path); }
    int LoadParam(FILE* fp) { return load_file(fp, true); }
    int LoadWeights(const char* weights_path) { return fhip_net_load_weights(net_, weights_path); }
    int LoadWeights(FILE* fp) { return load_file(fp, false); }
    int LoadParamMem(const char* text, size_t len) { return fhip_net_load_param_mem(net_, text, len); }
    int LoadWeightsMem(const void* data, size_t len) { return fhip_net_load_weights_mem(net_, data, len); }
    int LoadWeightsDevice(const void* device_data, size_t len) { return fhip_net_load_weights_device(net_, device_data, len); }

    int FeedInput(const char* input_name, ncnn::Mat& in)
    {
        if (in.dims != 3 || in.elemsize != 4u || !in.data) return -500;
        const size_t plane = (size_t)in.w * in.h;
        if (in.cstep == plane) return fhip_net_feed_input(net_, input_name, 1, in.c, in.h, in.w, (const float*)in.data, 0);
        std::string dense;
        dense.resize(plane * in.c * sizeof(float));
        for (int q = 0; q < in.c; ++q) memcpy(&dense[(size_t)q * plane * sizeof(float)], (const float*)in.data + in.cstep * q, plane * sizeof(float));
        return fhip_net_feed_input(net_, input_name, 1, in.c, in.h, in.w, (const float*)dense.data(), 0);
    }
    int FeedInput(const char* input_name, int c, int h, int w, const float* data) { return fhip_net_feed_input(net_, input_name, 1, c, h, w, data, 0); }
    int FeedInput(const char* input_name, int n, int c, int h, int w, const float* data) { return fhip_net_feed_input(net_, input_name, n, c, h, w, data, 0); }
    int FeedInputDevice(const char* input_name, int n, int c, int h, int w, const float* device_data)
    {
        return fhip_net_feed_input(net_, input_name, n, c, h, w, device_data, 1);
    }

    int FeedPixels(const char* input_name, const unsigned char* pixels, int type, int w, int h, int target_w, int target_h,
                   const float* mean = NULL, const float* norm = NULL)
    {
        return fhip_net_feed_pixels(net_, input_name, 1, pixels, type, w, h, target_w, target_h, mean, norm, 0);
    }
    int FeedPixels(const char* input_name, int n, const unsigned char* pixels, int type, int w, int h, int target_w, int target_h,
                   const float* mean = NULL, const float* norm = NULL)
    {
        return fhip_net_feed_pixels(net_, input_name, n, pixels, type, w, h, target_w, target_h, mean, norm, 0);
    }
    int FeedPixelsDevice(const char* input_name, int n, const unsigned char* device_pixels, int type, int w, int h, int target_w, int target_h,
                         const float* mean = NULL, const float* norm = NULL)
    {
        return fhip_net_feed_pixels(net_, input_name, n, device_pixels, type, w, h, target_w, target_h, mean, norm, 1);
    }
    int FeedPixelImages(const char* input_name, int n, const fhip_pixel_image* images, int type, int target_w, int target_h,
                        const float* mean = NULL, const float* norm = NULL)
    {
        return fhip_net_feed_pixel_images(net_, input_name, n, images, type, target_w, target_h, mean, norm, 0);
    }
    int FeedPixelImagesDevice(const char* input_name, int n, const fhip_pixel_image* images, int type, int target_w, int target_h,
                              const float* mean = NULL, const float* norm = NULL)
    {
        return fhip_net_feed_pixel_images(net_, input_name, n, images, type, target_w, target_h, mean, norm, 1);
    }
    int FeedYUV420sp(const char* input_name, const unsigned char* yuv, int w, int h, int target_w, int target_h, int type,
                     int resize_first = 1, const float* mean = NULL, const float* norm = NULL)
    {
        return fhip_net_feed_yuv420sp(net_, input_name, 1, yuv, w, h, target_w, target_h, type, resize_first, mean, norm, 0);
    }
    int FeedYUV420sp(const char* input_name, int n, const unsigned char* yuv, int w, int h, int target_w, int target_h, int type,
                     int resize_first = 1, const float* mean = NULL, const float* norm = NULL)
    {
        return fhip_net_feed_yuv420sp(net_, input_name, n, yuv, w, h, target_w, target_h, type, resize_first, mean, norm, 0);
    }
    int FeedYUV420spDevice(const char* input_name, int n, const unsigned char* device_yuv, int w, int h, int target_w, int target_h, int type,
                           int resize_first = 1, const float* mean = NULL, const float* norm = NULL)
    {
        return fhip_net_feed_yuv420sp(net_, input_name, n, device_yuv, w, h, target_w, target_h, type, resize_first, mean, norm, 1);
    }

    int Forward() { return fhip_net_forward(net_); }

    int Extract(std::string blob_name, float** output_ptr, int* n, int* c, int* h, int* w)
    {
        return fhip_net_extract(net_, blob_name.c_str(), output_ptr, n, c, h, w);
    }
    int Extract(std::string blob_name, ncnn::Mat& out)
    {
        float* dev = NULL;
        int n = 0, c = 0, h = 0, w = 0;
        int rc = fhip_net_extract(net_, blob_name.c_str(), &dev, &n, &c, &h, &w);
        if (rc) return rc;
        const size_t plane = (size_t)w * h, count = plane * c * n;
        out.create(w, h, c * n, 4u);
        if (out.empty() && count) return -1;
        if (out.cstep == plane) return fhip_net_extract_host(net_, blob_name.c_str(), (float*)out.data, count);
        std::string dense;
        dense.resize(count * sizeof(float));
        rc = fhip_net_extract_host(net_, blob_name.c_str(), (float*)&dense[0], count);
        if (rc) return rc;
        for (int q = 0; q < c * n; ++q) memcpy((float*)out.data + out.cstep * q, &dense[(size_t)q * plane * sizeof(float)], plane * sizeof(float));
        return 0;
    }
    int ExtractPixels(std::string blob_name, int* n_out, unsigned char* pixels, int type, int target_w, int target_h,
                      const float* mean = NULL, const float* norm = NULL, size_t pitch = 0)
    {
        return extract_pixels(blob_name, n_out, pixels, type, target_w, target_h, mean, norm, pitch, false);
    }
    int ExtractPixelsDevice(std::string blob_name, int* n_out, unsigned char* device_pixels, int type, int target_w, int target_h,
                            const float* mean = NULL, const float* norm = NULL, size_t pitch = 0)
    {
        return extract_pixels(blob_name, n_out, device_pixels, type, target_w, target_h, mean, norm, pitch, true);
    }
    int ExtractHost(std::string blob_name, float* host, size_t capacity_floats) { return fhip_net_extract_host(net_, blob_name.c_str(), host, capacity_floats); }

    int SetStream(void* hip_stream) { return fhip_net_set_stream(net_, hip_stream); }
    int SetFusion(int level) { return fhip_net_set_fusion(net_, level); }
    int SetGraph(bool on) { return fhip_net_set_graph(net_, on ? 1 : 0); }
    int SetTunedSelection(bool on) { return fhip_net_set_tuned_selection(net_, on ? 1 : 0); }
    int SetDilated(bool on) { return fhip_net_set_dilated(net_, on ? 1 : 0); }
    int SetQuantized(bool on) { return fhip_net_set_quantized(net_, on ? 1 : 0); }
    int SetRequantized(bool on) { return fhip_net_set_requantized(net_, on ? 1 : 0); }
    int SetExtendedLayers(bool on) { return fhip_net_set_extended_layers(net_, on ? 1 : 0); }
    int SetDetection(bool on) { return fhip_net_set_detection(net_, on ? 1 : 0); }
    int ExtractDetections(std::string blob_name, std::vector<std::vector<Detection> >& out)
    {
        float* dev = NULL;
        int n = 0, c = 0, h = 0, w = 0;
        int rc = Extract(blob_name, &dev, &n, &c, &h, &w);
        if (rc) return rc;
        if (c != 1 || w != 6) return -100;
        std::vector<float> rows((size_t)n * h * 6);
        if ((rc = ExtractHost(blob_name, rows.data(), rows.size()))) return rc;
        out.assign(n, std::vector<Detection>());
        for (int i = 0; i < n; ++i)
            for (int r = 0; r < h; ++r)
            {
                const float* v = &rows[((size_t)i * h + r) * 6];
                if (!(v[0] > 0.f)) break;
                Detection d = {(int)v[0], v[1], v[2], v[3], v[4], v[5]};
                out[i].push_back(d);
            }
        return 0;
    }
    int SetConcurrency(bool on) { return fhip_net_set_concurrency(net_, on ? 1 : 0); }
    int SetSubBatches(int replicas) { return fhip_net_set_sub_batches(net_, replicas); }
    int LayerCount() { return fhip_net_layer_count(net_); }
    static const char* LastError() { return fhip_last_error(); }
    static const char* LastPixelError() { return fhip_pixout_last_error(); }
    fhip_net* handle() { return net_; }

  private:
    Net(const Net&);
    Net& operator=(const Net&);
    int extract_pixels(const std::string& blob_name, int* n_out, unsigned char* pixels, int type, int target_w, int target_h,
                       const float* mean, const float* norm, size_t pitch, bool on_device)
    {
        float* dev = NULL;
        int n = 0, c = 0, h = 0, w = 0;
        void* stream = NULL;
        int rc = fhip_net_extract(net_, blob_name.c_str(), &dev, &n, &c, &h, &w);
        if (rc) return rc;
        rc = fhip_net_get_stream(net_, &stream);
        if (rc) return rc;
        const int cn = fhip_pixout_channels(type);
        if (cn < 0) return cn;
        if (cn != c) return FHIP_E_BADARG;
        if (n_out) *n_out = n;
        return on_device ? fhip_float_to_pixels(pixels, pitch, dev, n, type, w, h, target_w, target_h, mean, norm, stream)
                         : fhip_float_to_pixels_host(pixels, pitch, dev, n, type, w, h, target_w, target_h, mean, norm, stream);
    }
    int load_file(FILE* fp, bool param)
    {
        if (!fp) return -1;
        std::string buf;
        char chunk[1 << 16];
        size_t got;
        if (param) fseek(fp, 0, SEEK_SET);
        while ((got = fread(chunk, 1, sizeof(chunk), fp)) > 0) buf.append(chunk, got);
        return param ? fhip_net_load_param_mem(net_, buf.data(), buf.size()) : fhip_net_load_weights_mem(net_, buf.data(), buf.size());
    }
    fhip_net* net_;
};

}
```

### include/feather_hip/feather_net.h

```cpp
#ifndef FEATHER_NET_H_
#define FEATHER_NET_H_

#include "feather_hip/feather_hip.h"

#ifdef __cplusplus
extern "C" {
#endif


FHIP_API int fhip_relu(float* y, const float* x, size_t count, void* stream);

FHIP_API int fhip_add(float* y, const float* a, const float* b, size_t count, int relu, void* stream);

FHIP_API int fhip_affine(float* y, const float* x, const float* mul, const float* add, int batch, int channels, int hw,
                         int relu, void* stream);


enum
{
    FHIP_PIXEL_CONVERT_SHIFT = 16,
    FHIP_PIXEL_RGB = 1,
    FHIP_PIXEL_BGR = (1 << 1),
    FHIP_PIXEL_GRAY = (1 << 2),
    FHIP_PIXEL_RGBA = (1 << 3),
    FHIP_PIXEL_RGB2BGR = FHIP_PIXEL_RGB | (FHIP_PIXEL_BGR << FHIP_PIXEL_CONVERT_SHIFT),
    FHIP_PIXEL_RGB2GRAY = FHIP_PIXEL_RGB | (FHIP_PIXEL_GRAY << FHIP_PIXEL_CONVERT_SHIFT),
    FHIP_PIXEL_BGR2RGB = FHIP_PIXEL_BGR | (FHIP_PIXEL_RGB << FHIP_PIXEL_CONVERT_SHIFT),
    FHIP_PIXEL_BGR2GRAY = FHIP_PIXEL_BGR | (FHIP_PIXEL_GRAY << FHIP_PIXEL_CONVERT_SHIFT),
    FHIP_PIXEL_GRAY2RGB = FHIP_PIXEL_GRAY | (FHIP_PIXEL_RGB << FHIP_PIXEL_CONVERT_SHIFT),
    FHIP_PIXEL_GRAY2BGR = FHIP_PIXEL_GRAY | (FHIP_PIXEL_BGR << FHIP_PIXEL_CONVERT_SHIFT),
    FHIP_PIXEL_RGBA2RGB = FHIP_PIXEL_RGBA | (FHIP_PIXEL_RGB << FHIP_PIXEL_CONVERT_SHIFT),
    FHIP_PIXEL_RGBA2BGR = FHIP_PIXEL_RGBA | (FHIP_PIXEL_BGR << FHIP_PIXEL_CONVERT_SHIFT),
    FHIP_PIXEL_RGBA2GRAY = FHIP_PIXEL_RGBA | (FHIP_PIXEL_GRAY << FHIP_PIXEL_CONVERT_SHIFT)
};

FHIP_API int fhip_pixels_to_float(float* output, const unsigned char* pixels, int batch, int type, int w, int h, int target_w, int target_h,
                                  const float* mean, const float* norm, void* stream);

FHIP_API int fhip_yuv420sp_to_float(float* output, const unsigned char* yuv, int batch, int type, int w, int h, int target_w, int target_h,
                                    int resize_first, const float* mean, const float* norm, void* stream);

typedef struct fhip_pixel_image
{
    const unsigned char* data;
    int w, h, stride;
    int roi_x, roi_y, roi_w, roi_h;
} fhip_pixel_image;

FHIP_API int fhip_pixel_images_plan(const fhip_pixel_image* images, int batch, int type, int target_w, int target_h, void* plan,
                                    size_t* plan_bytes);
FHIP_API int fhip_pixels_to_float_images(float* output, const void* plan, const void* plan_device, const float* mean, const float* norm,
                                         void* stream);

FHIP_API int fhip_conv_can_fuse_maxpool2(const fhip_conv_param* param, int algo);
FHIP_API int fhip_conv_forward_maxpool2(const fhip_conv_param* param, int algo, int batch, float* pooled_output, const float* input,
                                        const float* packed, float* buffer, const float* bias, void* stream);

FHIP_API int fhip_conv_can_fuse_residual(const fhip_conv_param* param, int algo);
FHIP_API int fhip_conv_forward_residual(const fhip_conv_param* param, int algo, int batch, float* output, const float* input,
                                        const float* packed, float* buffer, const float* bias, const float* residual, void* stream);

FHIP_API int fhip_conv_can_fuse_dw_pw(const fhip_conv_param* dw, const fhip_conv_param* pw, int batch);
FHIP_API int fhip_conv_forward_dw_pw(const fhip_conv_param* dw, const fhip_conv_param* pw, int batch, float* output, const float* input,
                                     const float* dw_packed, const float* dw_bias, const float* pw_packed, const float* pw_bias, void* stream);

typedef struct fhip_pool_param
{
    int channels, input_h, input_w;
    int kernel_h, kernel_w;
    int stride_h, stride_w;
    int pad_left, pad_right, pad_top, pad_bottom;
    int pooling_type;
    int global_pooling;
} fhip_pool_param;

FHIP_API int fhip_pooling_output_dim(const fhip_pool_param* p, int* out_h, int* out_w);
FHIP_API int fhip_pooling(const fhip_pool_param* p, int batch, float* y, const float* x, void* stream);

FHIP_API int fhip_softmax(float* y, const float* x, int batch, int count_per_image, void* stream);

FHIP_API int fhip_conv_can_chain_winograd(const fhip_conv_param* param, int algo, const fhip_conv_param* next, int next_algo, int pool);
FHIP_API int fhip_conv_forward_chained(const fhip_conv_param* param, int batch, float* output, const float* input, const float* packed, float* v,
                                       float* m, const float* bias, const fhip_conv_param* next, float* v_next, int pool, void* stream);
FHIP_API int fhip_winograd_f63_output_to_next_input(const fhip_conv_param* param, const fhip_conv_param* next, int batch, float* v_next,
                                                    const float* m, const float* bias, int pool, void* stream);

FHIP_API int fhip_conv_can_fuse_siblings(const fhip_conv_param* a, int algo_a, const fhip_conv_param* b, int algo_b, int batch);
FHIP_API int fhip_conv_siblings_geometry(const fhip_conv_param* a, const fhip_conv_param* b, fhip_conv_param* both);
FHIP_API int fhip_conv_forward_siblings(const fhip_conv_param* a, const fhip_conv_param* b, int batch, float* output_a, float* output_b,
                                        const float* input, const float* packed_both, const float* bias_both, void* stream);

FHIP_API int fhip_conv_can_fuse_first_winograd(const fhip_conv_param* first, const fhip_conv_param* next, int next_algo, int batch);
FHIP_API int fhip_winograd_f63_input_from_first(const fhip_conv_param* first, const fhip_conv_param* next, int batch, float* v_next,
                                                const float* input, const float* first_kernel, const float* first_bias, void* stream);


typedef struct fhip_net fhip_net;

FHIP_API int fhip_net_create(fhip_net** net);
FHIP_API int fhip_net_destroy(fhip_net* net);
FHIP_API int fhip_net_set_stream(fhip_net* net, void* stream);
FHIP_API int fhip_net_get_stream(fhip_net* net, void** stream);
FHIP_API int fhip_net_set_fusion(fhip_net* net, int on);
FHIP_API int fhip_net_set_tuned_selection(fhip_net* net, int on);
FHIP_API int fhip_net_set_dilated(fhip_net* net, int on);
FHIP_API int fhip_net_set_extended_layers(fhip_net* net, int on);
FHIP_API int fhip_net_set_detection(fhip_net* net, int on);
FHIP_API int fhip_net_set_quantized(fhip_net* net, int on);
FHIP_API int fhip_net_set_requantized(fhip_net* net, int on);
FHIP_API int fhip_net_set_concurrency(fhip_net* net, int on);
FHIP_API int fhip_net_set_graph(fhip_net* net, int on);

FHIP_API int fhip_net_set_sub_batches(fhip_net* net, int replicas);

FHIP_API int fhip_net_load_param(fhip_net* net, const char* path);
FHIP_API int fhip_net_load_param_mem(fhip_net* net, const char* text, size_t len);
FHIP_API int fhip_net_load_weights(fhip_net* net, const char* path);
FHIP_API int fhip_net_load_weights_mem(fhip_net* net, const void* data, size_t len);
FHIP_API int fhip_net_load_weights_device(fhip_net* net, const void* device_data, size_t len);

FHIP_API int fhip_net_feed_input(fhip_net* net, const char* blob_name, int n, int c, int h, int w, const float* data,
                                 int on_device);
FHIP_API int fhip_net_feed_pixels(fhip_net* net, const char* blob_name, int n, const unsigned char* pixels, int type, int w, int h,
                                  int target_w, int target_h, const float* mean, const float* norm, int on_device);
FHIP_API int fhip_net_feed_yuv420sp(fhip_net* net, const char* blob_name, int n, const unsigned char* yuv, int w, int h, int target_w,
                                    int target_h, int type, int resize_first, const float* mean, const float* norm, int on_device);
FHIP_API int fhip_net_feed_pixel_images(fhip_net* net, const char* blob_name, int n, const fhip_pixel_image* images, int type,
                                        int target_w, int target_h, const float* mean, const float* norm, int on_device);
FHIP_API int fhip_net_forward(fhip_net* net);
FHIP_API int fhip_net_extract(fhip_net* net, const char* blob_name, float** device_ptr, int* n, int* c, int* h, int* w);
FHIP_API int fhip_net_extract_host(fhip_net* net, const char* blob_name, float* host, size_t capacity);

FHIP_API int fhip_net_layer_count(fhip_net* net);
#define FHIP_NET_ROUTE_GCONV 100
#define FHIP_NET_ROUTE_DECONV 101
#define FHIP_NET_ROUTE_INORM 102
#define FHIP_NET_ROUTE_SHUFFLE 103
#define FHIP_NET_ROUTE_ATROUS 104
#define FHIP_NET_ROUTE_GATE 105
#define FHIP_NET_ROUTE_RESAMPLE 106
#define FHIP_NET_ROUTE_LRN 107
#define FHIP_NET_ROUTE_QCONV 108
FHIP_API int fhip_net_layer_info(fhip_net* net, int index, char* type, char* name, int len, int* algo);
FHIP_API int fhip_net_layer_conv_param(fhip_net* net, int index, fhip_conv_param* param, int* batch);
FHIP_API int fhip_net_layer_fused_pointwise(fhip_net* net, int index, fhip_conv_param* param, int* one_kernel);
FHIP_API int fhip_net_layer_chain(fhip_net* net, int index, int* v_from_previous, int* writes_next_v);
FHIP_API int fhip_net_layer_canvas(fhip_net* net, int index, int* canvas);
FHIP_API int fhip_net_layer_sibling(fhip_net* net, int index, int* state);
FHIP_API int fhip_net_layer_residual(fhip_net* net, int index, int* state);
FHIP_API int fhip_net_forward_timed(fhip_net* net, float* ms);
FHIP_API int fhip_net_memory(fhip_net* net, size_t* blob_bytes, size_t* weight_bytes, size_t* arena_bytes);

#ifdef __cplusplus
}
#endif
#endif
```

Baseline: 10170 images/s.

## Add column-pass Winograd tile GEMM with fused output-to-next-input chain for 64-channel layers

```diff
diff --git a/__graft_entry__.py b/__graft_entry__.py
--- a/__graft_entry__.py
+++ b/__graft_entry__.py
@@ -16,7 +16,7 @@
     subprocess.run(["make", "-s", "-C", os.path.join(ROOT, "oracle"), "ref"], check=True)
     import feathercnn_amd
     from feathercnn_amd import _lib
-    for name in (*_lib.LIBRARIES, *_lib.MORE_LIBRARIES):
+    for name in (*_lib.LIBRARIES, *_lib.MORE_LIBRARIES, *_lib.THIRD_LIBRARIES):
         _lib.load(name)
     from feathercnn_amd import provenance
     provenance.write_stamp()
diff --git a/feathercnn_amd/_lib.py b/feathercnn_amd/_lib.py
--- a/feathercnn_amd/_lib.py
+++ b/feathercnn_amd/_lib.py
@@ -101,6 +101,7 @@
     "fhip_net_set_requantized": (_I, [_V, _I]),
     "fhip_net_set_extended_layers": (_I, [_V, _I]),
     "fhip_net_set_detection": (_I, [_V, _I]),
+    "fhip_net_set_colpass": (_I, [_V, _I]),
     "fhip_net_set_concurrency": (_I, [_V, _I]),
     "fhip_net_set_sub_batches": (_I, [_V, _I]),
     "fhip_net_load_param": (_I, [_V, ctypes.c_char_p]),
@@ -121,6 +122,7 @@
     "fhip_net_layer_fused_pointwise": (_I, [_V, _I, _P, _PI]),
     "fhip_net_layer_chain": (_I, [_V, _I, _PI, _PI]),
     "fhip_net_layer_canvas": (_I, [_V, _I, _PI]),
+    "fhip_net_layer_colpass": (_I, [_V, _I, _PI]),
     "fhip_net_layer_sibling": (_I, [_V, _I, _PI]),
     "fhip_net_layer_residual": (_I, [_V, _I, _PI]),
     "fhip_net_forward_timed": (_I, [_V, ctypes.POINTER(ctypes.c_float)]),
@@ -301,6 +303,14 @@
     "fhip_detection_output_forward": (_I, [_I, _I, _I, _FL, _I, _I, _FL, _I, _V, _V, _V, _V, _V, _V]),
     "fhip_detect_route": (_I, [_I, _I, _I, _I, _I, _I, _V, _V, ctypes.c_char_p, _I]),
     "fhip_detect_last_error": (ctypes.c_char_p, []),
+}
+
+
+COLPASS_SIGNATURES = {
+    "fhip_colpass_supported": (_I, [_P, _I]),
+    "fhip_colpass_tile_gemm": (_I, [_P, _I, _PL, _V, _V, _V, _V]),
+    "fhip_colpass_output_to_next_input": (_I, [_P, _P, _I, _PL, _PL, _V, _V, _V, _I, _V]),
+    "fhip_colpass_last_error": (ctypes.c_char_p, []),
 }
 
 
@@ -356,10 +366,16 @@
     "q8": Library("libfeather_q8.so", ("feather_q8.h",), "FHIP_Q8_API", Q8_SIGNATURES, "fhip_q8_last_error", (fhip_q8_param,), None),
     "detect": Library("libfeather_detect.so", ("feather_detect.h",), "FHIP_DETECT_API", DETECT_SIGNATURES, "fhip_detect_last_error", (), None),
 }
+THIRD_LIBRARIES = {
+    "colpass": Library("libfeather_colpass.so", ("feather_colpass.h",), "FHIP_COLPASS_API", COLPASS_SIGNATURES, "fhip_colpass_last_error", (), None),
+}
 
 
 def row(name: str) -> Library:
-    return LIBRARIES[name] if name in LIBRARIES else MORE_LIBRARIES[name]
+    for table in (LIBRARIES, MORE_LIBRARIES, THIRD_LIBRARIES):
+        if name in table:
+            return table[name]
+    raise KeyError(name)
 
 
 def path(name: str) -> str:
@@ -379,7 +395,7 @@
     return load(MAIN)
 
 
-for _name in (*LIBRARIES, *MORE_LIBRARIES):
+for _name in (*LIBRARIES, *MORE_LIBRARIES, *THIRD_LIBRARIES):
     if _name != MAIN:
         globals()[f"{_name}_path"] = functools.partial(path, _name)
         globals()[f"load_{_name}_library"] = functools.partial(load, _name)
diff --git a/feathercnn_amd/csrc/net.hip b/feathercnn_amd/csrc/net.hip
--- a/feathercnn_amd/csrc/net.hip
+++ b/feathercnn_amd/csrc/net.hip
@@ -304,6 +304,7 @@
         m->impl.quantized = n->impl.quantized;
         m->impl.requantized = n->impl.requantized;
         m->impl.concurrency = n->impl.concurrency;
+        m->impl.colpass = n->impl.colpass;
         n->more.push_back(std::move(m));
     }
     if (replicas > 1 && !n->fork) FHIP_CHECK_HIP(hipEventCreateWithFlags(&n->fork, hipEventDisableTiming));
@@ -395,6 +396,16 @@
     n->impl.concurrency = on != 0;
     n->impl.shapes_dirty = true;
     for (auto& m : n->more) (void)fhip_net_set_concurrency(m.get(), on);
+    return FHIP_OK;
+}
+
+int fhip_net_set_colpass(fhip_net* n, int mode)
+{
+    NET_GUARD(n);
+    if (mode < 0 || mode > 2) return fail(FHIP_E_BADARG, "colpass mode: 0 never, 1 where M is HBM-bound, 2 wherever the library accepts the layer");
+    n->impl.colpass = mode;
+    n->impl.shapes_dirty = true;
+    for (auto& m : n->more) (void)fhip_net_set_colpass(m.get(), mode);
     return FHIP_OK;
 }
 
@@ -755,6 +766,14 @@
     return FHIP_OK;
 }
 
+int fhip_net_layer_colpass(fhip_net* n, int index, int* colpass)
+{
+    NET_GUARD(n);
+    if (index < 0 || index >= (int)n->impl.layers.size() || !colpass) return fail(FHIP_E_BADARG, "layer index out of range");
+    *colpass = n->impl.layers[index]->colpass_state();
+    return FHIP_OK;
+}
+
 int fhip_net_forward_timed(fhip_net* n, float* ms)
 {
     NET_GUARD(n);
diff --git a/feathercnn_amd/csrc/net_conv.h b/feathercnn_amd/csrc/net_conv.h
--- a/feathercnn_amd/csrc/net_conv.h
+++ b/feathercnn_amd/csrc/net_conv.h
@@ -208,6 +208,7 @@
     bool canvas = false;
     fhip_conv_param canvas_p = {};
     fhip_winograd_plan run_plan = {};
+    bool colpass = false;
     ConvLayer* head_of = nullptr;
     ConvLayer* head = nullptr;
 
@@ -520,6 +521,7 @@
             if (rc) return rc;
         }
         if (chain.canvas || (chain.next && chain.next->chain.canvas)) return forward_canvas(n, in, v, m, vn, b, s);
+        if (chain.colpass) return forward_colpass(n, in, v, m, vn, b, s);
         if (chain.next) return fhip_conv_forward_chained(&p, n, nullptr, in, packed.d, v, m, b, &chain.next->p, vn, pool, s);
         if (!ep.fuse_pool || ep.pool_fast) return fhip_conv_forward_chained(&p, n, tops[0]->data, in, packed.d, v, m, b, nullptr, nullptr, pool, s);
         return pool_tail(fhip_conv_forward_chained(&p, n, ep.pre_pool.d, in, packed.d, v, m, b, nullptr, nullptr, 0, s), s);
@@ -543,6 +545,17 @@
         }
         else
             rc = api->output(&p, n, &chain.run_plan, tops[0]->data, m, b, ep.fuse_pool ? 1 : 0, s);
+        return rc ? failf(rc, "layer %s: %s", name.c_str(), api->last_error()) : 0;
+    }
+    int forward_colpass(int n, const float* in, float* v, float* m, float* vn, const float* b, hipStream_t s)
+    {
+        const ColpassApi* api = colpass_api();
+        if (!api) return FHIP_E_UNSUPPORTED;
+        int rc;
+        if (in && (rc = fhip_winograd_f63_input_transform(&p, n, v, in, s))) return rc;
+        const ConvLayer* nx = chain.next;
+        rc = api->tile_gemm(&p, n, &chain.run_plan, m, packed.d, v, s);
+        if (!rc) rc = api->chain(&p, &nx->p, n, &chain.run_plan, &nx->chain.run_plan, vn, m, b, ep.fuse_pool ? 1 : 0, s);
         return rc ? failf(rc, "layer %s: %s", name.c_str(), api->last_error()) : 0;
     }
     int forward_plain(hipStream_t s)
@@ -599,6 +612,7 @@
         *writes_next_v = chain.head_of ? 2 : chain.next ? 1 : 0;
     }
     int canvas_state() const override { return chain.canvas ? 1 : 0; }
+    int colpass_state() const override { return chain.colpass ? 1 : 0; }
 };
 
 inline void ChainPlan::link(ConvLayer* a, ConvLayer* b) { a->chain.next = b, b->chain.in = true, b->chain.pos = a->chain.pos + 1; }
diff --git a/feathercnn_amd/csrc/net_core.h b/feathercnn_amd/csrc/net_core.h
--- a/feathercnn_amd/csrc/net_core.h
+++ b/feathercnn_amd/csrc/net_core.h
@@ -144,6 +144,7 @@
     virtual const fhip_conv_param* fused_pointwise(int*) const { return nullptr; }
     virtual void chain_state(int* v_from_previous, int* writes_next_v) const { *v_from_previous = *writes_next_v = 0; }
     virtual int canvas_state() const { return 0; }
+    virtual int colpass_state() const { return 0; }
     virtual int sibling_state() const { return 0; }
     virtual int residual_state() const { return 0; }
 };
@@ -168,6 +169,7 @@
     bool quantized = false;
     bool detection = false;
     bool requantized = false;
+    int colpass = 1;
     bool param_loaded = false, weights_loaded = false, fused = false, initialized = false, shapes_dirty = true;
     DeviceVec arena;
     size_t chain_slot[2] = {0, 0}, chain_m = 0;
diff --git a/feathercnn_amd/csrc/net_plan.h b/feathercnn_amd/csrc/net_plan.h
--- a/feathercnn_amd/csrc/net_plan.h
+++ b/feathercnn_amd/csrc/net_plan.h
@@ -1,5 +1,6 @@
 #pragma once
 #include "net_detect.h"
+#include "wino_gemm_policy.h"
 
 namespace fhip::net
 {
@@ -391,6 +392,19 @@
         slot[c->chain.pos & 1] = std::max(slot[c->chain.pos & 1], up(c->chain.run_plan.v_bytes));
         msz = std::max(msz, up(c->chain.run_plan.m_bytes));
     }
+    if (net.colpass)
+        for (ConvLayer* c : conv)
+        {
+            if (!c || !c->chain.next || c->chain.canvas || c->chain.next->chain.canvas) continue;
+            if (net.colpass == 1 && c->chain.run_plan.m_bytes < (size_t)FHIP_M_NT_BYTES) continue;
+            const fhip_conv_param& q = c->p;
+            if (q.input_channels != 64 || q.output_channels < 64 || (q.output_channels & 63) || c->chain.run_plan.frequency_points != 64) continue;
+            if (q.activation != FHIP_ACT_NONE && q.activation != FHIP_ACT_RELU) continue;
+            const ColpassApi* api = net.colpass == 2 ? colpass_api() : colpass_api_quiet();
+            if (!api && net.colpass == 2) return FHIP_E_UNSUPPORTED;
+            if (!api) break;
+            c->chain.colpass = api->supported(&q, c->bottoms[0]->n) == FHIP_OK;
+        }
     net.chain_slot[0] = 0;
     net.chain_slot[1] = slot[0];
     net.chain_m = slot[0] + slot[1];
diff --git a/feathercnn_amd/csrc/net_side.h b/feathercnn_amd/csrc/net_side.h
--- a/feathercnn_amd/csrc/net_side.h
+++ b/feathercnn_amd/csrc/net_side.h
@@ -19,6 +19,7 @@
 
 #include "common.h"
 #include "feather_hip/feather_canvas.h"
+#include "feather_hip/feather_colpass.h"
 #include "feather_hip/feather_atrous.h"
 #include "feather_hip/feather_deconv.h"
 #include "feather_hip/feather_detect.h"
@@ -317,4 +318,26 @@
 };
 static const CanvasApi* canvas_api() { return side_api<CanvasApi>(); }
 
-}
+struct ColpassApi
+{
+    decltype(&fhip_colpass_supported) supported = nullptr;
+    decltype(&fhip_colpass_tile_gemm) tile_gemm = nullptr;
+    decltype(&fhip_colpass_output_to_next_input) chain = nullptr;
+    decltype(&fhip_colpass_last_error) last_error = nullptr;
+    SideLibrary library()
+    {
+        return {"libfeather_colpass.so", "a chained Winograd layer on the column-passed tile GEMM (fhip_net_set_colpass 2)", "feather_colpass.h",
+                {{&supported, "fhip_colpass_supported"}, {&tile_gemm, "fhip_colpass_tile_gemm"}, {&chain, "fhip_colpass_output_to_next_input"},
+                 {&last_error, "fhip_colpass_last_error"}}};
+    }
+};
+static const ColpassApi* colpass_api() { return side_api<ColpassApi>(); }
+static const ColpassApi* colpass_api_quiet()
+{
+    const std::string kept = fhip_last_error();
+    const ColpassApi* api = colpass_api();
+    if (!api) fail(FHIP_OK, kept.c_str());
+    return api;
+}
+
+}
diff --git a/feathercnn_amd/csrc_colpass/colpass.hip b/feathercnn_amd/csrc_colpass/colpass.hip
--- /dev/null
+++ b/feathercnn_amd/csrc_colpass/colpass.hip
@@ -0,0 +1,463 @@
+#include <hip/hip_runtime.h>
+#include <stdint.h>
+
+#include <algorithm>
+#include <string>
+
+#include "feather_hip/feather_colpass.h"
+#include "side_error.h"
+#include "wino_butterfly.h"
+#include "wino_layout.h"
+
+namespace fhip
+{
+
+typedef __attribute__((address_space(3))) void lds_void;
+
+constexpr size_t kBigM = (size_t)150u << 20;
+
+struct ColGemm
+{
+    const float* U;
+    const float* V;
+    float* M;
+    int Kp, m_tiles, n_tiles;
+    WinoLayout Lv, Lm;
+};
+
+template <int N>
+__device__ __forceinline__ void wait_stage()
+{
+    asm volatile("s_waitcnt vmcnt(%0) lgkmcnt(0)" ::"n"(N) : "memory");
+}
+
+#ifndef COLPASS_WN
+#define COLPASS_WN 2
+#endif
+#ifndef COLPASS_BK
+#define COLPASS_BK 16
+#endif
+#ifndef COLPASS_NBUF
+#define COLPASS_NBUF 6
+#endif
+#ifndef COLPASS_OCC
+#define COLPASS_OCC 3
+#endif
+
+template <int WN, int BK, int NBUF, int NT>
+__global__ __launch_bounds__(128 * WN, COLPASS_OCC * WN / 2) void colpass_gemm_kernel(const ColGemm g)
+{
+    constexpr int C = 64, BM = 64, BN = 32 * WN, NW = 2 * WN, EPI_LD = 36;
+    constexpr int KT = C / BK, S = 8 * KT;
+    constexpr int BUF = BK * (BM + BN);
+    constexpr int A_PIECES = BK / 4 / NW;
+    constexpr int B_LPR = BN / 4, B_RPP = 64 / B_LPR, B_PIECES = BK / B_RPP / NW;
+    constexpr int PPS = A_PIECES + B_PIECES;
+    constexpr int LDSF = NBUF * BUF > NW * 32 * EPI_LD ? NBUF * BUF : NW * 32 * EPI_LD;
+    static_assert(A_PIECES >= 1 && B_PIECES >= 1 && A_PIECES * 4 * NW == BK && B_PIECES * B_RPP * NW == BK, "stage pieces");
+    static_assert(NBUF >= 2 && NBUF <= S, "buffers");
+    __shared__ __attribute__((aligned(16))) float lds[LDSF];
+
+    int vid = xcd_remap(blockIdx.x, 8 * g.m_tiles * g.n_tiles);
+    const int j = vid & 7;
+    vid >>= 3;
+    const int mt = vid % g.m_tiles;
+    const int nt = vid / g.m_tiles;
+    const int m0 = mt * BM, n0 = nt * BN;
+
+    const int tid = threadIdx.x, lane = tid & 63, wave = tid >> 6;
+    const int wm = wave / WN, wn = wave % WN;
+    const int l31 = lane & 31, half = lane >> 5;
+
+    const float* srcA = g.U + (size_t)j * C * g.Kp + (size_t)(wave * A_PIECES * 4 + (lane >> 4)) * g.Kp + m0 + (lane & 15) * 4;
+    const float* srcB = g.V + (size_t)j * g.Lv.xis + g.Lv.col(n0) + (size_t)(wave * B_PIECES * B_RPP + lane / B_LPR) * g.Lv.bp + (lane % B_LPR) * 4;
+    const size_t a_xi = (size_t)8 * C * g.Kp, b_xi = (size_t)8 * g.Lv.xis;
+
+    auto issue = [&](int s, int buf) {
+        const int i = s / KT, kt = s - i * KT;
+        float* base = lds + buf * BUF;
+        const float* a = srcA + (size_t)i * a_xi + (size_t)(kt * BK) * g.Kp;
+        const float* b = srcB + (size_t)i * b_xi + (size_t)(kt * BK) * g.Lv.bp;
+#pragma unroll
+        for (int p = 0; p < A_PIECES; ++p)
+            __builtin_amdgcn_global_load_lds(a + (size_t)(4 * p) * g.Kp, (lds_void*)(base + (wave * A_PIECES + p) * 256), 16, 0, 0);
+#pragma unroll
+        for (int p = 0; p < B_PIECES; ++p)
+            __builtin_amdgcn_global_load_lds(b + (size_t)(B_RPP * p) * g.Lv.bp, (lds_void*)(base + BK * BM + (wave * B_PIECES + p) * 256), 16, 0,
+                                             (NT & 1) ? 2 : 0);
+    };
+
+    f32x16 acc[8];
+#pragma unroll
+    for (int i = 0; i < 8; ++i)
+#pragma unroll
+        for (int r = 0; r < 16; ++r) acc[i][r] = 0.f;
+
+#pragma unroll
+    for (int s = 0; s < NBUF - 1; ++s) issue(s, s);
+    wait_stage<(NBUF - 2) * PPS>();
+    __builtin_amdgcn_s_barrier();
+
+    const int a_off = half * BM + wm * 32 + l31;
+    const int b_off = BK * BM + half * BN + wn * 32 + l31;
+#pragma unroll
+    for (int s = 0; s < S; ++s)
+    {
+        const bool more = s + NBUF - 1 < S;
+        if (more) issue(s + NBUF - 1, (s + NBUF - 1) % NBUF);
+        const float* as = lds + (s % NBUF) * BUF + a_off;
+        const float* bs = lds + (s % NBUF) * BUF + b_off;
+#pragma unroll
+        for (int kp = 0; kp < BK / 2; ++kp) acc[s / KT] = __builtin_amdgcn_mfma_f32_32x32x2f32(as[(2 * kp) * BM], bs[(2 * kp) * BN], acc[s / KT], 0, 0, 0);
+        if (more)
+            wait_stage<(NBUF - 2) * PPS>();
+        else
+            wait_stage<0>();
+        __builtin_amdgcn_s_barrier();
+    }
+
+#pragma unroll
+    for (int r = 0; r < 16; ++r)
+    {
+        float s0, s1, s2, s3, s4, s5;
+        at6(acc[0][r], acc[1][r], acc[2][r], acc[3][r], acc[4][r], acc[5][r], acc[6][r], acc[7][r], s0, s1, s2, s3, s4, s5);
+        acc[0][r] = s0;
+        acc[1][r] = s1;
+        acc[2][r] = s2;
+        acc[3][r] = s3;
+        acc[4][r] = s4;
+        acc[5][r] = s5;
+    }
+
+    float* const scr = lds + wave * (32 * EPI_LD);
+    const int e_row = lane >> 3, e_c4 = (lane & 7) * 4;
+    float* const mbase = g.M + (size_t)j * g.Lm.xis + g.Lm.col(n0 + wn * 32) + e_c4 + (size_t)(m0 + wm * 32 + e_row) * g.Lm.bp;
+#pragma unroll
+    for (int a = 0; a < 6; ++a)
+    {
+#pragma unroll
+        for (int r = 0; r < 16; ++r) scr[((r & 3) + 8 * (r >> 2) + 4 * half) * EPI_LD + l31] = acc[a][r];
+        float* const mp = mbase + (size_t)(8 * a) * g.Lm.xis;
+#pragma unroll
+        for (int q = 0; q < 4; ++q)
+        {
+            const float4 v = *reinterpret_cast<const float4*>(&scr[(q * 8 + e_row) * EPI_LD + e_c4]);
+            if constexpr ((NT & 2) != 0)
+                stg4_nt(mp + (size_t)(q * 8) * g.Lm.bp, v);
+            else
+                *reinterpret_cast<float4*>(mp + (size_t)(q * 8) * g.Lm.bp) = v;
+        }
+    }
+}
+
+struct ColChain
+{
+    int K, N;
+    int TX, T;
+    int AH, AW;
+    int TX2, T2;
+    int planes;
+    int ppb;
+    int LDW, LDH;
+    WinoLayout Lm, Lv2;
+};
+
+template <bool HAS_BIAS, bool RELU, bool POOL, bool MULTI>
+__global__ __launch_bounds__(512, 3) void colpass_chain_kernel(float* __restrict__ Vn, const float* __restrict__ M, const float* __restrict__ bias,
+                                                               const ColChain g, const int units)
+{
+    extern __shared__ __attribute__((aligned(16))) float smem[];
+    const int tid = threadIdx.x, nthreads = blockDim.x;
+    const int plane_floats = g.LDH * g.LDW;
+    for (int i = tid; i < g.ppb * plane_floats; i += nthreads) smem[i] = 0.f;
+    const int n1 = MULTI ? (g.T + nthreads - 1) / nthreads : 1;
+    int pl = MULTI ? 0 : tid / g.T, t = tid - pl * g.T;
+    bool lane_on = MULTI ? t < g.T : pl < g.ppb;
+    int ty = t / g.TX, tx = t - ty * g.TX;
+    const int pl2 = tid / g.T2, t2 = tid - pl2 * g.T2;
+    const bool lane_on2 = pl2 < g.ppb;
+    const int ty2 = t2 / g.TX2, tx2 = t2 - ty2 * g.TX2;
+    const int xcd = blockIdx.x & 7, j = blockIdx.x >> 3, xcd_blocks = (gridDim.x + 7 - xcd) >> 3;
+    const int u_lo = (int)((long long)units * xcd / 8), u_hi = (int)((long long)units * (xcd + 1) / 8);
+    const size_t xi_stride = g.Lm.xis, xi_stride2 = g.Lv2.xis;
+    float* const lp1 = smem + pl * plane_floats;
+
+    float tmp[6][8];
+    auto fetch = [&](int unit, int tile) {
+        const int plane = min(unit * g.ppb + (lane_on ? pl : 0), g.planes - 1);
+        const int k = plane / g.N, n = plane - k * g.N;
+        const float* mp = M + (size_t)k * g.Lm.bp + g.Lm.col(n * g.T + min(tile, g.T - 1));
+#pragma unroll
+        for (int a = 0; a < 6; ++a)
+#pragma unroll
+            for (int jj = 0; jj < 8; ++jj) tmp[a][jj] = mp[(size_t)(a * 8 + jj) * xi_stride];
+    };
+    int unit = u_lo + j;
+    if (unit < u_hi) fetch(unit, t);
+    __syncthreads();
+    for (; unit < u_hi; unit += xcd_blocks)
+    {
+        const int plane = unit * g.ppb + pl;
+        const int k = min(plane, g.planes - 1) / g.N;
+        for (int it = 0; it < n1; ++it)
+        {
+            if (MULTI)
+            {
+                t = tid + it * nthreads;
+                lane_on = t < g.T;
+                ty = t / g.TX;
+                tx = t - ty * g.TX;
+            }
+            if (lane_on && plane < g.planes)
+            {
+                const float b = HAS_BIAS ? bias[k] : 0.f;
+                float prev0 = 0.f, prev1 = 0.f, prev2 = 0.f;
+#pragma unroll
+                for (int a = 0; a < 6; ++a)
+                {
+                    float y[6];
+                    at6(tmp[a][0], tmp[a][1], tmp[a][2], tmp[a][3], tmp[a][4], tmp[a][5], tmp[a][6], tmp[a][7], y[0], y[1], y[2], y[3], y[4], y[5]);
+#pragma unroll
+                    for (int bb = 0; bb < 6; ++bb)
+                    {
+                        float v = y[bb] + b;
+                        if (RELU) v = fmaxf(v, 0.f);
+                        y[bb] = v;
+                    }
+                    if (POOL)
+                    {
+                        const float h0 = fmaxf(y[0], y[1]), h1 = fmaxf(y[2], y[3]), h2 = fmaxf(y[4], y[5]);
+                        if ((a & 1) == 0)
+                        {
+                            prev0 = h0;
+                            prev1 = h1;
+                            prev2 = h2;
+                        }
+                        else
+                        {
+                            const int ay = 3 * ty + (a >> 1);
+                            if (ay < g.AH)
+                            {
+                                float* row = lp1 + (size_t)(ay + 1) * g.LDW + 2 + 3 * tx;
+                                row[0] = (3 * tx < g.AW) ? fmaxf(prev0, h0) : 0.f;
+                                row[1] = (3 * tx + 1 < g.AW) ? fmaxf(prev1, h1) : 0.f;
+                                row[2] = (3 * tx + 2 < g.AW) ? fmaxf(prev2, h2) : 0.f;
+                            }
+                        }
+                        continue;
+                    }
+                    const int ay = 6 * ty + a;
+                    if (ay < g.AH)
+                    {
+                        float* row = lp1 + (size_t)(ay + 1) * g.LDW + 2 + 6 * tx;
+#pragma unroll
+                        for (int bb = 0; bb < 6; bb += 2)
+                        {
+                            const float v0 = (6 * tx + bb < g.AW) ? y[bb] : 0.f, v1 = (6 * tx + bb + 1 < g.AW) ? y[bb + 1] : 0.f;
+                            *reinterpret_cast<float2*>(row + bb) = make_float2(v0, v1);
+                        }
+                    }
+                }
+            }
+            if (MULTI && it + 1 < n1) fetch(unit, tid + (it + 1) * nthreads);
+        }
+        __syncthreads();
+        if (unit + xcd_blocks < u_hi) fetch(unit + xcd_blocks, MULTI ? tid : t);
+        __builtin_amdgcn_sched_barrier(0);
+        const int plane2 = unit * g.ppb + pl2;
+        if (lane_on2 && plane2 < g.planes)
+        {
+            const int k2 = plane2 / g.N, n2 = plane2 - k2 * g.N;
+            const float* lp = smem + pl2 * plane_floats + (size_t)(6 * ty2) * g.LDW + 6 * tx2 + 1;
+            float d[8][8];
+#pragma unroll
+            for (int i = 0; i < 8; ++i)
+#pragma unroll
+                for (int jj = 0; jj < 8; ++jj) d[i][jj] = lp[(size_t)i * g.LDW + jj];
+#pragma unroll
+            for (int jj = 0; jj < 8; ++jj) bt8(d[0][jj], d[1][jj], d[2][jj], d[3][jj], d[4][jj], d[5][jj], d[6][jj], d[7][jj]);
+#pragma unroll
+            for (int i = 0; i < 8; ++i) bt8(d[i][0], d[i][1], d[i][2], d[i][3], d[i][4], d[i][5], d[i][6], d[i][7]);
+            float* vp = Vn + (size_t)k2 * g.Lv2.bp + g.Lv2.col(n2 * g.T2 + t2);
+#pragma unroll
+            for (int i = 0; i < 8; ++i)
+#pragma unroll
+                for (int jj = 0; jj < 8; ++jj) vp[(size_t)(i * 8 + jj) * xi_stride2] = d[i][jj];
+        }
+        __syncthreads();
+    }
+}
+
+static int device_limits(int* cus, size_t* lds)
+{
+    static thread_local int dev_cached = -1, cus_cached = 0;
+    static thread_local size_t lds_cached = 0;
+    int dev = 0;
+    FHIP_CHECK_HIP(hipGetDevice(&dev));
+    if (dev != dev_cached)
+    {
+        hipDeviceProp_t prop;
+        FHIP_CHECK_HIP(hipGetDeviceProperties(&prop, dev));
+        cus_cached = prop.multiProcessorCount;
+        lds_cached = prop.maxSharedMemoryPerMultiProcessor;
+        dev_cached = dev;
+    }
+    *cus = cus_cached;
+    *lds = lds_cached;
+    return FHIP_OK;
+}
+
+static bool k3s1(const fhip_conv_param& c) { return c.kernel_h == 3 && c.kernel_w == 3 && c.stride_h <= 1 && c.stride_w <= 1 && c.group <= 1; }
+
+static bool f43_plane(const fhip_conv_param& p)
+{
+    const int oh = p.input_h + p.pad_top + p.pad_bottom - 2, ow = p.input_w + p.pad_left + p.pad_right - 2;
+    if (oh < 1 || ow < 1 || oh > 8 || ow > 8 || (oh < 7 && ow < 7)) return false;
+    return ((oh + 3) / 4) * ((ow + 3) / 4) * 36 < ((oh + 5) / 6) * ((ow + 5) / 6) * 64;
+}
+
+static int supported(const fhip_conv_param& p, int batch)
+{
+    if (batch < 1) return fail(FHIP_E_BADARG, "batch < 1");
+    if (!k3s1(p)) return fail(FHIP_E_UNSUPPORTED, "the column-passed tile GEMM needs a 3x3 stride-1 group-1 convolution");
+    const int hp = p.input_h + p.pad_top + p.pad_bottom, wp = p.input_w + p.pad_left + p.pad_right;
+    if (hp < 3 || wp < 3) return fail(FHIP_E_BADARG, "input smaller than the kernel");
+    if (f43_plane(p)) return fail(FHIP_E_UNSUPPORTED, "a plane of 7 or 8 pixels runs on F(4x4,3x3), which has no column-passed form");
+    if (p.input_channels != 64) return fail(FHIP_E_UNSUPPORTED, "the column-passed tile GEMM holds the whole depth of a stage on chip: input_channels must be 64");
+    if (p.output_channels < 64 || (p.output_channels & 63)) return fail(FHIP_E_UNSUPPORTED, "output_channels must be a multiple of 64 (the row tile)");
+    const long long P = (long long)((wp + 3) / 6) * ((hp + 3) / 6) * batch;
+    if (P > 0x7fffff00LL) return fail(FHIP_E_BADARG, "too many Winograd tiles for 32-bit column indices: N * tiles per image above 0x7fffff00");
+    return FHIP_OK;
+}
+
+static bool plan_is(const fhip_winograd_plan& pl, const fhip_conv_param& p, int batch)
+{
+    const int tx = (p.input_w + p.pad_left + p.pad_right + 3) / 6, ty = (p.input_h + p.pad_top + p.pad_bottom + 3) / 6;
+    if (pl.frequency_points != 64 || pl.tiles_x != tx || pl.tiles_y != ty || pl.tiles_per_image != tx * ty) return false;
+    if ((long long)pl.columns != (long long)tx * ty * batch || pl.columns_padded < pl.columns || (pl.columns_padded & 127)) return false;
+    const int bp = pl.column_block;
+    return bp == pl.columns_padded || (bp >= 128 && (bp & (bp - 1)) == 0 && pl.columns_padded % bp == 0);
+}
+
+static int tile_gemm(const fhip_conv_param& p, int batch, const fhip_winograd_plan& pl, float* m48, const float* u, const float* v, hipStream_t s)
+{
+    if (const int rc = supported(p, batch)) return rc;
+    if (!plan_is(pl, p, batch) || pl.in_channels_padded != 64 || pl.out_channels_padded < p.output_channels || (pl.out_channels_padded & 63))
+        return fail(FHIP_E_BADARG, "the plan does not belong to this layer and batch (fhip_winograd_f63_plan)");
+    if (!aligned(m48, 16) || !aligned(u, 16) || !aligned(v, 16)) return fail(FHIP_E_BADARG, "m48, u and v must be 16-byte aligned");
+    constexpr int WN = COLPASS_WN, BK = COLPASS_BK, NBUF = COLPASS_NBUF, BN = 32 * WN;
+    ColGemm g;
+    g.U = u;
+    g.V = v;
+    g.M = m48;
+    g.Kp = pl.out_channels_padded;
+    g.m_tiles = p.output_channels / 64;
+    g.n_tiles = (pl.columns + BN - 1) / BN;
+    g.Lv = wino_layout(64, pl.columns_padded, pl.column_block, 64);
+    g.Lm = wino_layout(p.output_channels, pl.columns_padded, pl.column_block, 48);
+    const long long blocks = 8LL * g.m_tiles * g.n_tiles;
+    if (blocks > 0x7fffffffLL) return fail(FHIP_E_BADARG, "2^31 blocks or more");
+    const bool big_m = (size_t)64 * p.output_channels * pl.columns_padded * sizeof(float) >= kBigM;
+    const dim3 grid((unsigned)blocks), threads(128 * WN);
+    if (g.m_tiles == 1 && big_m) hipLaunchKernelGGL((colpass_gemm_kernel<WN, BK, NBUF, 3>), grid, threads, 0, s, g);
+    else if (g.m_tiles == 1) hipLaunchKernelGGL((colpass_gemm_kernel<WN, BK, NBUF, 1>), grid, threads, 0, s, g);
+    else if (big_m) hipLaunchKernelGGL((colpass_gemm_kernel<WN, BK, NBUF, 2>), grid, threads, 0, s, g);
+    else hipLaunchKernelGGL((colpass_gemm_kernel<WN, BK, NBUF, 0>), grid, threads, 0, s, g);
+    FHIP_CHECK_HIP(hipGetLastError());
+    return FHIP_OK;
+}
+
+static int chain(const fhip_conv_param& p, const fhip_conv_param& next, int batch, const fhip_winograd_plan& pl, const fhip_winograd_plan& pn,
+                 float* vn, const float* m48, const float* bias, int pool, hipStream_t s)
+{
+    if (const int rc = supported(p, batch)) return rc;
+    if (!k3s1(next) || next.pad_left != 1 || next.pad_right != 1 || next.pad_top != 1 || next.pad_bottom != 1 ||
+        next.input_channels != p.output_channels || f43_plane(next))
+        return fail(FHIP_E_UNSUPPORTED, "the consumer must be a 3x3 / stride-1 / pad-1 F(6x6,3x3) layer on this layer's output channels");
+    if (pool && ((p.output_h & 1) || (p.output_w & 1))) return fail(FHIP_E_UNSUPPORTED, "fused max pooling needs even output dims");
+    const int ah = pool ? p.output_h / 2 : p.output_h, aw = pool ? p.output_w / 2 : p.output_w;
+    if (next.input_h != ah || next.input_w != aw) return fail(FHIP_E_UNSUPPORTED, "the consumer's input is not this layer's (pooled) output");
+    if (p.activation != FHIP_ACT_NONE && p.activation != FHIP_ACT_RELU) return fail(FHIP_E_UNSUPPORTED, "activation other than none / ReLU");
+    if (!plan_is(pl, p, batch) || !plan_is(pn, next, batch))
+        return fail(FHIP_E_BADARG, "the plans do not belong to these layers and this batch (fhip_winograd_f63_plan)");
+    if (p.output_h != p.input_h + p.pad_top + p.pad_bottom - 2 || p.output_w != p.input_w + p.pad_left + p.pad_right - 2)
+        return fail(FHIP_E_BADARG, "output dims are not those of the geometry (fhip_conv_assign_output_dim)");
+    const bool has_bias = p.bias_term != 0, relu = p.activation == FHIP_ACT_RELU;
+    if (has_bias && !bias) return fail(FHIP_E_BADARG, "bias_term set but bias is NULL");
+    ColChain g;
+    g.K = p.output_channels;
+    g.N = batch;
+    g.TX = pl.tiles_x;
+    g.T = pl.tiles_per_image;
+    g.AH = ah;
+    g.AW = aw;
+    g.TX2 = pn.tiles_x;
+    g.T2 = pn.tiles_per_image;
+    g.Lm = wino_layout(g.K, pl.columns_padded, pl.column_block, 48);
+    g.Lv2 = wino_layout(g.K, pn.columns_padded, pn.column_block, 64);
+    const long long planes = (long long)batch * g.K;
+    if (planes > 0x7fffffffLL) return fail(FHIP_E_BADARG, "N*K too large: 2^31 planes or more");
+    g.planes = (int)planes;
+    g.LDH = 6 * pn.tiles_y + 2;
+    g.LDW = 6 * pn.tiles_x + 4;
+    const size_t plane_bytes = (size_t)g.LDH * g.LDW * sizeof(float);
+    if (plane_bytes > 64 * 1024) return fail(FHIP_E_UNSUPPORTED, "the consumer's plane does not fit a block's LDS");
+    const int work = std::max(g.T, g.T2);
+    int ppb = std::max(1, 256 / work);
+    ppb = (int)std::min<size_t>(ppb, std::max<size_t>(1, (48 * 1024) / plane_bytes));
+    g.ppb = (int)std::min<long long>(ppb, planes);
+    const bool multi = work > 512;
+    if (multi && !pool) return fail(FHIP_E_UNSUPPORTED, "an unpooled plane of more than 512 tiles");
+    const unsigned threads = std::max(256u, (unsigned)((multi ? g.T2 : work) + 63) / 64 * 64);
+    if (threads > 512u) return fail(FHIP_E_UNSUPPORTED, "the consumer's plane has more than 512 tiles");
+    const size_t lds = plane_bytes * g.ppb;
+    const long long units = (planes + g.ppb - 1) / g.ppb;
+    int cus;
+    size_t dev_lds;
+    if (const int rc = device_limits(&cus, &dev_lds)) return rc;
+    const int bpc = std::max(1, std::min((int)(dev_lds / lds), 12 / (int)(threads / 64)));
+    const unsigned grid = ((unsigned)std::min<long long>(units, (long long)cus * bpc) + 7u) & ~7u;
+#define FHIP_COLPASS_CHAIN(P_, M_)                                                                                                              \
+    do                                                                                                                                          \
+    {                                                                                                                                           \
+        if (has_bias && relu) hipLaunchKernelGGL((colpass_chain_kernel<true, true, P_, M_>), dim3(grid), dim3(threads), lds, s, vn, m48, bias, g, (int)units); \
+        else if (has_bias) hipLaunchKernelGGL((colpass_chain_kernel<true, false, P_, M_>), dim3(grid), dim3(threads), lds, s, vn, m48, bias, g, (int)units);   \
+        else if (relu) hipLaunchKernelGGL((colpass_chain_kernel<false, true, P_, M_>), dim3(grid), dim3(threads), lds, s, vn, m48, bias, g, (int)units);       \
+        else hipLaunchKernelGGL((colpass_chain_kernel<false, false, P_, M_>), dim3(grid), dim3(threads), lds, s, vn, m48, bias, g, (int)units);                \
+    } while (0)
+    if (pool && multi) FHIP_COLPASS_CHAIN(true, true);
+    else if (pool) FHIP_COLPASS_CHAIN(true, false);
+    else FHIP_COLPASS_CHAIN(false, false);
+#undef FHIP_COLPASS_CHAIN
+    FHIP_CHECK_HIP(hipGetLastError());
+    return FHIP_OK;
+}
+
+}
+
+extern "C"
+{
+
+int fhip_colpass_supported(const fhip_conv_param* param, int batch)
+{
+    if (!param) return fhip::fail(FHIP_E_BADARG, "bad argument");
+    return fhip::supported(*param, batch);
+}
+
+int fhip_colpass_tile_gemm(const fhip_conv_param* param, int batch, const fhip_winograd_plan* plan, float* m48, const float* u, const float* v,
+                           void* stream)
+{
+    if (!param || !plan || !m48 || !u || !v) return fhip::fail(FHIP_E_BADARG, "bad argument");
+    return fhip::tile_gemm(*param, batch, *plan, m48, u, v, (hipStream_t)stream);
+}
+
+int fhip_colpass_output_to_next_input(const fhip_conv_param* param, const fhip_conv_param* next, int batch, const fhip_winograd_plan* plan,
+                                      const fhip_winograd_plan* plan_next, float* v_next, const float* m48, const float* bias, int pool, void* stream)
+{
+    if (!param || !next || !plan || !plan_next || !v_next || !m48) return fhip::fail(FHIP_E_BADARG, "bad argument");
+    return fhip::chain(*param, *next, batch, *plan, *plan_next, v_next, m48, bias, pool, (hipStream_t)stream);
+}
+
+const char* fhip_colpass_last_error(void) { return fhip::last_error(); }
+
+}
diff --git a/feathercnn_amd/net.py b/feathercnn_amd/net.py
--- a/feathercnn_amd/net.py
+++ b/feathercnn_amd/net.py
@@ -74,6 +74,9 @@
     def set_tuned(self, on: bool):
         _check(self._lib.fhip_net_set_tuned_selection(self._h, int(bool(on))), "fhip_net_set_tuned_selection")
 
+    def SetColpass(self, mode: int = 1):
+        _check(self._lib.fhip_net_set_colpass(self._h, int(mode)), "fhip_net_set_colpass")
+
     def set_concurrency(self, on: bool):
         _check(self._lib.fhip_net_set_concurrency(self._h, int(bool(on))), "fhip_net_set_concurrency")
 
@@ -271,6 +274,14 @@
                 out.append(i)
         return out
 
+    def colpasses(self):
+        out = []
+        for i in range(self._lib.fhip_net_layer_count(self._h)):
+            c = ctypes.c_int()
+            if self._lib.fhip_net_layer_colpass(self._h, i, ctypes.byref(c)) == 0 and c.value:
+                out.append(i)
+        return out
+
     def forward_timed(self):
         n = self._lib.fhip_net_layer_count(self._h)
         ms = (ctypes.c_float * max(n, 1))()
diff --git a/include/feather/net.h b/include/feather/net.h
--- a/include/feather/net.h
+++ b/include/feather/net.h
@@ -159,6 +159,7 @@
         return 0;
     }
     int SetConcurrency(bool on) { return fhip_net_set_concurrency(net_, on ? 1 : 0); }
+    int SetColpass(int mode) { return fhip_net_set_colpass(net_, mode); }
     int SetSubBatches(int replicas) { return fhip_net_set_sub_batches(net_, replicas); }
     int LayerCount() { return fhip_net_layer_count(net_); }
     static const char* LastError() { return fhip_last_error(); }
diff --git a/include/feather_hip/feather_colpass.h b/include/feather_hip/feather_colpass.h
--- /dev/null
+++ b/include/feather_hip/feather_colpass.h
@@ -0,0 +1,30 @@
+#ifndef FEATHER_HIP_FEATHER_COLPASS_H_
+#define FEATHER_HIP_FEATHER_COLPASS_H_
+
+#include <stddef.h>
+
+#include "feather_hip/feather_hip.h"
+
+#ifdef __cplusplus
+extern "C"
+{
+#endif
+
+#define FHIP_COLPASS_API __attribute__((visibility("default")))
+
+FHIP_COLPASS_API int fhip_colpass_supported(const fhip_conv_param* param, int batch);
+
+FHIP_COLPASS_API int fhip_colpass_tile_gemm(const fhip_conv_param* param, int batch, const fhip_winograd_plan* plan, float* m48, const float* u,
+                                            const float* v, void* stream);
+
+FHIP_COLPASS_API int fhip_colpass_output_to_next_input(const fhip_conv_param* param, const fhip_conv_param* next, int batch,
+                                                       const fhip_winograd_plan* plan, const fhip_winograd_plan* plan_next, float* v_next,
+                                                       const float* m48, const float* bias, int pool, void* stream);
+
+FHIP_COLPASS_API const char* fhip_colpass_last_error(void);
+
+#ifdef __cplusplus
+}
+#endif
+
+#endif
diff --git a/include/feather_hip/feather_net.h b/include/feather_hip/feather_net.h
--- a/include/feather_hip/feather_net.h
+++ b/include/feather_hip/feather_net.h
@@ -109,6 +109,7 @@
 FHIP_API int fhip_net_set_quantized(fhip_net* net, int on);
 FHIP_API int fhip_net_set_requantized(fhip_net* net, int on);
 FHIP_API int fhip_net_set_concurrency(fhip_net* net, int on);
+FHIP_API int fhip_net_set_colpass(fhip_net* net, int mode);
 FHIP_API int fhip_net_set_graph(fhip_net* net, int on);
 
 FHIP_API int fhip_net_set_sub_batches(fhip_net* net, int replicas);
@@ -146,6 +147,7 @@
 FHIP_API int fhip_net_layer_fused_pointwise(fhip_net* net, int index, fhip_conv_param* param, int* one_kernel);
 FHIP_API int fhip_net_layer_chain(fhip_net* net, int index, int* v_from_previous, int* writes_next_v);
 FHIP_API int fhip_net_layer_canvas(fhip_net* net, int index, int* canvas);
+FHIP_API int fhip_net_layer_colpass(fhip_net* net, int index, int* colpass);
 FHIP_API int fhip_net_layer_sibling(fhip_net* net, int index, int* state);
 FHIP_API int fhip_net_layer_residual(fhip_net* net, int index, int* state);
 FHIP_API int fhip_net_forward_timed(fhip_net* net, float* ms);
```

New measurement: 10320 images/s, median of 6. 1.01x the previous value.
